# Parskatt/RoMa

Hardware: AMD Instinct MI355X
Metric: image-pairs/sec, roma_outdoor 560->864, batch=8 per GPU (higher is better)
Workload: dtype bf16; 1 GPU; roma_outdoor match() 560->864, symmetric, upsample_preds, 8 pairs/GPU/step, seeded synthetic weights + N(0,1) images; precision policy of the reference's bf16 timing script: bfloat16 DINOv2 + float16 autocast for VGG / decoder / refiners (ROMA_MIXED), f32 accumulate; precision_policy=mixed, global_batch=8, streams_per_gpu=2, parallelism=single GPU, outputs_finite=True

## Files before the change

include/roma_hip.h:

```cpp
#ifndef ROMA_HIP_H
#define ROMA_HIP_H
#include <stdint.h>
#ifdef __cplusplus
extern "C" {
#endif

typedef struct roma_model* roma_handle_t;

enum { ROMA_F32 = 0, ROMA_BF16 = 1, ROMA_F16 = 2,
       ROMA_MIXED = 3 };
int roma_h16_format(void);
enum { ROMA_ERR_ARG = -1, ROMA_ERR_HIP = -2, ROMA_ERR_STATE = -3 };

typedef struct {
  int coarse_h, coarse_w;
  int upsample_h, upsample_w;
  int symmetric;
  int upsample_preds;
  int attenuate_cert;
  int precision;
  int max_batch;
  int device;
} roma_config_t;

const char* roma_last_error(void);
const char* roma_version(void);
#define ROMA_ABI_VERSION 5
int roma_abi_stamp(void);
int roma_self_check(void);

typedef struct {
  const float *ln1_w, *ln1_b, *ln2_w, *ln2_b;
  const float *ls1, *ls2;
  const void *qkv_w, *proj_w, *fc1_w, *fc2_w;
  const float *qkv_b, *proj_b, *fc1_b, *fc2_b;
  int qkv_ldw, proj_ldw, fc1_ldw, fc2_ldw;
} roma_vit_block_t;

typedef struct {
  int B, H, W;
  int act;
  int bf16_residual;
  const float *im_a, *im_b;
  const void* patch_w;
  const float* patch_b;
  int patch_ldw;
  const float *cls_tok, *pos_emb;
  const roma_vit_block_t* blocks;
  int nblocks;
  const float *norm_w, *norm_b;
  void *col, *pt, *x, *xs, *ln, *ao, *hid, *q, *k, *vt;
  void* feat_out;
} roma_vit_args_t;
int roma_vit_forward(const roma_vit_args_t* a, void* stream);
int roma_op_convert_from_bf16(const void* in_bf16, void* out_h16, long n, void* stream);

int roma_create(const roma_config_t* cfg, roma_handle_t* out);
int roma_set_tensor(roma_handle_t h, const char* name, int ndim, const int64_t* shape, const void* data, int is_int64);
int roma_finalize(roma_handle_t h);
int roma_set_option(roma_handle_t h, const char* key, int value);
int roma_set_option_f(roma_handle_t h, const char* key, double value);
int roma_match(roma_handle_t h, int B, const float* im_a, const float* im_b, const float* im_a_hr,
               const float* im_b_hr, float* warp_out, float* cert_out, void* stream);
typedef struct {
  int upsample;
  int symmetric;
  double scale_factor;
  const float* seed_flow;
  const float* seed_cert;
  int seed_h, seed_w;
  float* flow[5];
  float* cert[5];
  void* feat[5];
} roma_forward_args_t;
int roma_forward(roma_handle_t h, int B, const float* im_a, const float* im_b, const roma_forward_args_t* a, void* stream);
long roma_debug_fetch(roma_handle_t h, const char* name, void* dst_host, long nbytes);
int roma_debug_inject(roma_handle_t h, const char* name, const void* src_host, long nbytes);
long roma_debug_trace(roma_handle_t h, int slot, unsigned long long* sums_host, long max_entries, char* names_host,
                      long names_bytes);
int roma_destroy(roma_handle_t h);
int roma_tuning(const char* key, int value);
long roma_tuning_describe(char* buf, long nbytes);
long roma_debug_gemm_trace(unsigned int* dst_host, long nbytes);
int roma_profile_enable(int on);
long roma_profile_report(char* buf, long nbytes);


int roma_op_local_corr(const void* feature0, const void* feature1, const float* warp, void* out, int B, int H, int W,
                       int C, int K, int nearest, int dt_in, int dt_out, void* stream);
int roma_op_local_corr_window(const void* feature0, const void* feature1, const float* warp, void* out, int B, int H,
                              int W, int C, int radius, float scale, long ldo, int dt_in, int dt_out, void* stream);
long roma_op_local_corr_window_workspace(int B, int H, int W, int radius);
int roma_op_local_corr_window_ws(const void* feature0, const void* feature1, const float* warp, void* out, int B, int H,
                                 int W, int C, int radius, float scale, long ldo, int dt_in, int dt_out, void* ws,
                                 long ws_bytes, void* stream);

int roma_op_gemm(const void* A, long lda, const void* W, long ldw, void* C, long ldc, int M, int N, int K, int batch,
                 long sA, long sW, long sC, const float* bias, const float* scale, const float* res, long ldr,
                 int act, float alpha, int dt_in, int dt_out, void* stream);
int roma_op_conv3x3(const void* in, const void* w, const float* bias, void* out, int B, int H, int W, int Cin, int Cout,
                    int relu, int dt, void* stream);
int roma_op_conv3x3_slab(const void* in, const void* w, const float* bias, void* out, int B, int H, int W, int Cin, int Cout,
                         int relu, int dt, void* stream);
int roma_op_attention(const void* q, const void* k, const void* vt, void* out, int B, int heads, int N, int npad, int hd,
                      int dt_in, int dt_out, void* stream);
int roma_op_qkv_scatter_gemm(const void* A, const void* W, const float* bias, void* q, void* k, void* vt, int B, int N,
                             int npad, int heads, int hd, int K, int dt_in, int dt_out, void* stream);
int roma_op_layernorm(const float* x, const float* w, const float* b, void* out, long M, int D, float eps, int dt_out,
                      void* stream);
int roma_op_layernorm_dt(const void* x, int dt_in, const float* w, const float* b, void* out, long M, int D, float eps,
                         int dt_out, void* stream);
int roma_op_gemm_res_bf16(const void* A, long lda, const void* W, long ldw, void* C, long ldc, int M, int N, int K,
                          const float* bias, const float* scale, const void* res, long ldr, void* stream);
int roma_op_cholesky_solve_t(float* A, float* Ft, float* LT, float* Linv, float* LinvT, int n, int d, int batch,
                             void* stream);
int roma_op_gp(const void* x, const void* y, const float* pos_w, const float* pos_b, float* mu, int b, int h, int w, int dt,
               void* stream);
int roma_op_cls_to_flow(const float* logits, long ld, float* flow, float* cert, long M, void* stream);
int roma_op_resize_bilinear(const float* in, float* out, int B, int Hin, int Win, int Hout, int Wout, int nc,
                            void* stream);
int roma_op_refiner_input(const void* feat, long ldf, const float* flow, void* d, long ldd, const float* emb_w,
                          const float* emb_b, int B, int H, int W, int C, int E, int Kcorr, int nimg, int shift,
                          float disp_scale, int dt, void* stream);
int roma_op_dwconv5x5(const void* in, void* out, const float* w, const float* bias, int B, int H, int W, int Cp, int dt,
                      void* stream);
int roma_op_refiner_block(const void* in, void* out, const float* dw_w, const float* dw_b, const void* pw,
                          const float* pw_b, int B, int H, int W, int Cp, int dt, void* stream);
int roma_op_refiner_block_final(const void* in, float* delta, const float* dw_w, const float* dw_b, const void* pw_final,
                                const float* bias_final, int B, int H, int W, int Cp, int dt, void* stream);
int roma_op_refiner_apply_delta(const float* delta, float* flow, float* cert, long M, float sx, float sy, void* stream);
int roma_op_kde(const float* x, long n, int down, float std, int half_inputs, float* density, void* stream);
int roma_op_sample_warp_at(const float* warp, const float* cert, int H, int W, const float* xa, long n, float* xa_to_b,
                           float* cert_a, void* stream);
int roma_op_mutual_nn(const float* a, long na, const float* b, long nb, const float* cert_a, float cert_th, float max_dist,
                      int* match_b, void* ws_a, void* ws_b, void* stream);
int roma_op_mutual_nn_count(const float* a, long na, const float* b, long nb, const float* cert_a, float cert_th, float max_dist,
                            void* ws_a, void* ws_b, long long* offsets, void* stream);
int roma_op_mutual_nn_fill(const float* a, long na, const float* b, long nb, const float* cert_a, float cert_th, float max_dist,
                           const void* ws_a, const void* ws_b, long long* offsets, long long* pairs, void* stream);
long roma_op_multinomial_workspace(long n, long k);
int roma_op_multinomial(const float* weights, long n, long k, unsigned long long seed, long long* out_indices, void* workspace,
                        long workspace_bytes, void* stream);
long roma_op_sample_matches_workspace(int B, long n, long num, int balanced);
int roma_op_sample_matches(const float* matches, const float* certainty, const unsigned long long* seeds, int B, long n, long num,
                           int threshold, float thresh, int balanced, float* out_matches, float* out_certainty, int* out_counts,
                           long long* out_idx, long long* out_first_idx, float* out_density, void* workspace, long workspace_bytes,
                           void* stream);
long roma_op_ransac_workspace(int B, int N);
int roma_op_ransac(int model, const float* kpts_a, const float* kpts_b, const int* counts, const unsigned long long* seeds, int B,
                   int N, float threshold, double confidence, int max_iters, int refine, double* out_model, unsigned char* out_mask,
                   unsigned char* out_ok, int* out_info, void* workspace, long workspace_bytes, void* stream);
long roma_op_magsac_workspace(int B, int N);
int roma_op_magsac(int model, const float* kpts_a, const float* kpts_b, const int* counts, const unsigned long long* seeds, int B,
                   int N, float threshold, double confidence, int max_iters, int lo_iters, double* out_model, unsigned char* out_mask,
                   unsigned char* out_ok, int* out_info, double* out_score, void* workspace, long workspace_bytes, void* stream);
long roma_op_essential_workspace(int B, int N);
int roma_op_essential(const float* kpts_a, const float* kpts_b, const int* counts, const unsigned long long* seeds,
                      const double* camera_matrix, int B, int N, float threshold, double prob, int max_iters, double* out_e,
                      unsigned char* out_mask, unsigned char* out_ok, int* out_info, void* workspace, long workspace_bytes,
                      void* stream);
long roma_op_essential_magsac_workspace(int B, int N);
int roma_op_essential_magsac(const float* kpts_a, const float* kpts_b, const int* counts, const unsigned long long* seeds,
                             const double* camera_matrix, int B, int N, float threshold, double prob, int max_iters, int lo_iters,
                             double* out_e, unsigned char* out_mask, unsigned char* out_ok, int* out_info, double* out_score,
                             void* workspace, long workspace_bytes, void* stream);
int roma_op_essential_minimal(const double* x0, const double* x1, int S, double* out_e, int* out_n, void* stream);
long roma_op_recover_pose_workspace(int B, int N);
int roma_op_recover_pose(const double* E, const float* kpts_a, const float* kpts_b, const unsigned char* mask, const int* counts,
                         const double* camera_matrix, int B, int N, double distance_thresh, int* out_n_good, double* out_r,
                         double* out_t, unsigned char* out_mask, void* workspace, long workspace_bytes, void* stream);
long roma_op_refine_pose_workspace(int B, int N);
int roma_op_refine_pose(const double* R, const double* t, const float* kpts_a, const float* kpts_b, const int* counts,
                        const unsigned char* valid, int B, int N, double thr, int max_steps, double* out_r, double* out_t,
                        unsigned char* out_mask, int* out_info, void* workspace, long workspace_bytes, void* stream);
long roma_op_absolute_pose_workspace(int B, int N);
int roma_op_absolute_pose(const float* points3d, const float* kpts, const int* counts, const unsigned long long* seeds,
                          const double* camera_matrix, int B, int N, float threshold, double conf, int max_iters, double* out_r,
                          double* out_t, unsigned char* out_mask, unsigned char* out_ok, int* out_info, void* workspace,
                          long workspace_bytes, void* stream);
int roma_op_absolute_pose_minimal(const double* X, const double* x, int S, double* out_r, double* out_t, int* out_n, void* stream);
int roma_op_refine_absolute_pose(const double* R, const double* t, const float* points3d, const float* kpts, const int* counts,
                                 const unsigned char* valid, const double* camera_matrix, int B, int N, double thr, int max_steps,
                                 double* out_r, double* out_t, unsigned char* out_mask, int* out_info, void* stream);
int roma_op_lift_matches(const float* matches, const float* depth_a, const double* camera_a, int B, int N, int H, int W, int H_b,
                         int W_b, float* out_points, float* out_kpts_b, void* stream);
long roma_op_bundle_adjust_workspace(int B, int V, int N);
int roma_op_bundle_adjust(const double* points, const float* kpts, const double* camera_matrices, const double* R, const double* t,
                          const unsigned char* hold, const int* counts, const unsigned char* valid, int B, int V, int N,
                          double reproj_thresh, int max_steps, double* out_points, double* out_r, double* out_t, unsigned char* out_mask,
                          int* out_info, double* out_cost, void* workspace, long workspace_bytes, void* stream);
long roma_op_build_tracks_workspace(int B, int V, int K, int P, int M);
int roma_op_build_tracks(const int* inds, const int* pair_views, const int* match_counts, const int* num_kpts, const float* x, int B,
                         int V, int K, int P, int M, int max_tracks, int min_views, int* out_tracks, float* out_kpts, int* out_counts,
                         int* out_total, int* out_info, void* workspace, long workspace_bytes, void* stream);
int roma_op_triangulate_views(const float* kpts, const double* camera_matrices, const double* R, const double* t,
                              const unsigned char* view_valid, const int* counts, const unsigned char* valid, int B, int V, int N,
                              double max_reproj, double min_parallax, double max_depth, int min_views, int gn_steps, int trim,
                              double* out_points, float* out_reproj, unsigned char* out_used, float* out_parallax,
                              unsigned char* out_flags, int* out_stats, void* stream);
long roma_op_refine_model_workspace(int B, int N);
int roma_op_refine_model(int model, const double* M, const float* kpts_a, const float* kpts_b, const int* counts,
                         const unsigned char* valid, int B, int N, double thr, int max_steps, double* out_m, unsigned char* out_mask,
                         int* out_info, double* out_cost, void* workspace, long workspace_bytes, void* stream);
int roma_op_triangulate(const float* matches, const float* certainty, const int* counts, const unsigned char* valid, const double* R,
                        const double* t, const double* K_a, const double* K_b, int B, long n, int coords, int W_a, int H_a, int W_b,
                        int H_b, int sym_w, double max_depth, double max_reproj, double min_parallax, double min_certainty,
                        float* out_points, float* out_depth_other, float* out_reproj, float* out_parallax, unsigned char* out_flags,
                        int* out_stats, void* stream);
int roma_op_depth_consistency(const float* points, const unsigned char* flags, const double* R, const double* t, const double* K_a,
                              const double* K_b, int W_a, int H_a, int W_b, int H_b, int B, int H, int W, double rel_thresh,
                              unsigned char* out_consistent, float* out_err, void* stream);
int roma_op_warp_kpts(const void* kpts, int kpts_f64, int grid_h, int grid_w, const float* depth0, const float* depth1, const double* T,
                      int t_rows, const double* K0, const double* K1, int B, long L, int H0, int W0, int H1, int W1, double rel_thresh,
                      unsigned char* out_valid, float* out_prob, double* out_rel, double* out_warped, void* stream);
long roma_op_dense_metrics_workspace(int B, int h, int w);
int roma_op_dense_metrics(const float* matches, long batch_stride, long row_stride, const float* depth1, const float* depth2,
                          const double* T, int t_rows, const double* K1, const double* K2, int B, int h, int w, int H1, int W1, int H2,
                          int W2, double rel_thresh, double thr0, double thr1, double thr2, long long* out_n_valid,
                          long long* out_n_below, double* out_gd_sum, double* out_epe, double* out_pck, float* out_prob, double* out_gd,
                          void* workspace, long workspace_bytes, void* stream);
int roma_op_pose_error(const double* R, const double* t, const unsigned char* ok, const double* T_gt, int t_rows, int B, double* out_err,
                       double* log, long capacity, long long* state, void* stream);
int roma_op_corner_error(const double* H_pred, const unsigned char* ok, const double* H_gt, const double* sizes, int B, double* out_err,
                         double* log, long capacity, long long* state, void* stream);
int roma_op_error_log_append(const double* values, int B, double* log, long capacity, long long* state, void* stream);
int roma_op_error_summary(const double* errors, long n, const long long* state, long capacity, const double* thresholds, int T,
                          long long* out_n, long long* out_below, double* out_acc, double* out_auc, void* stream);
int roma_op_render_morph_frame_chunk(void);
long roma_op_render_morph_workspace(int B, int im_h, int im_w, long T);
int roma_op_render_morph(const float* warp, long warp_batch_stride, long warp_row_stride, const void* image, int image_u8, const double* ts,
                         const float* certainty, long cert_batch_stride, long cert_row_stride, float background, int B, long T, int H,
                         int W, int im_h, int im_w, void* out, int out_f32, void* workspace, long workspace_bytes, void* stream);
long roma_op_match_keypoints_workspace(int B, long NA, long NB);
int roma_op_match_keypoints(const float* x_a, const float* x_b, const int* counts_a, const int* counts_b, const float* warp,
                            long warp_batch_stride, long warp_row_stride, const float* certainty, long cert_batch_stride,
                            long cert_row_stride, const float* sizes, long sizes_batch_stride, int B, long NA, long NB, int H, int W,
                            float max_dist, float cert_th, long M, int* inds, float* kpts_a, float* kpts_b, int* counts,
                            long long* total, void* workspace, long workspace_bytes, void* stream);
long roma_op_preprocess_workspace(const long long* desc_host, int n_images, const int* targets_hw, int n_targets);
int roma_op_preprocess(const unsigned char* src, long long src_bytes, const long long* desc_host, const long long* desc_dev,
                       int n_images, const int* targets_hw, int n_targets, int normalize, float* out0, float* out1, void* workspace,
                       void* stream);
int roma_op_nchw_to_nhwc(const float* in, float* out, int B, int C, int H, int W, void* stream);
int roma_op_tiny_pos_embed(const float* corr_volume, float* out, int B, int H1, int W1, int H0, int W0, int exact_softmax,
                           void* stream);
int roma_op_gray_instnorm(const float* in, float* out, int B, int H, int W, int C, float eps, void* stream);
int roma_op_conv2d_nhwc(const float* in, const float* w, const float* bias, const float* res, float* out, int B, int H, int W,
                        int Cin, int Cout, int K, int stride, int pad, int relu, void* stream);
int roma_op_avgpool_nhwc(const float* in, float* out, int B, int H, int W, int C, int k, void* stream);
int roma_op_add3(const float* a, const float* b, const float* c, float* out, long n, void* stream);
int roma_op_tiny_matcher_input(const float* f0, const float* f1, const float* warp, int warp_channels, float* d, int B, int H,
                               int W, int H1, int W1, int C, int Cp, void* stream);
int roma_op_tiny_update(const float* base, int base_channels, const float* delta, long ldd, float sx, float sy, float* out,
                        long npix, void* stream);
int roma_op_tiny_final(const float* matches, float* warp, float* certainty, int B, int H, int W, void* stream);
int roma_op_visualize_warp(const float* warp, const float* certainty, const float* im_a, const float* im_b, int H, int W,
                           int symmetric, int im_h, int im_w, float* out, void* stream);
int roma_op_fb_consistency(const float* flow_fwd, const float* flow_bwd, int B, int H, int W, float th_n, float* out,
                           void* stream);
int roma_op_maxpool2x2(const void* in, void* out, int B, int H, int W, int C, int dt, void* stream);
int roma_op_pool_proj(const void* in, void* pooled, void* pf, const void* pw, long ldw, const float* pb, int N, int ldf, int B, int H,
                      int W, int C, int dt, void* stream);
int roma_op_refiner_out(const void* d, long ldd, int dt, const float* w, const float* b, float* flow, float* cert, long M,
                        int Cp, float sx, float sy, void* stream);
int roma_op_conv3x3_c3(const float* img, const float* w, const float* bias, void* out, int B, int H, int W, int dt_out,
                       void* stream);
int roma_op_conv3x3_c3_bf16(const float* img, const void* w, const float* bias, void* out, int B, int H, int W, void* stream);

#ifdef __cplusplus
}
#endif
#endif
```

roma_amd/_lib.py:

```python
from __future__ import annotations

import ctypes as C
import os

_HERE = os.path.dirname(os.path.abspath(__file__))
_HERE = os.environ.get("ROMA_LIB_DIR", _HERE)
LIB_PATH = os.path.join(_HERE, "libroma_hip.so")
LIB_PATHS = {"bf16": LIB_PATH, "f16": os.path.join(_HERE, "libroma_hip_f16.so")}

ROMA_F32, ROMA_BF16, ROMA_F16, ROMA_MIXED = 0, 1, 2, 3
H16_CODE = {"bf16": ROMA_BF16, "f16": ROMA_F16}


class RomaConfig(C.Structure):
    _fields_ = [("coarse_h", C.c_int), ("coarse_w", C.c_int), ("upsample_h", C.c_int), ("upsample_w", C.c_int),
                ("symmetric", C.c_int), ("upsample_preds", C.c_int), ("attenuate_cert", C.c_int),
                ("precision", C.c_int), ("max_batch", C.c_int), ("device", C.c_int)]


class RomaForwardArgs(C.Structure):
    _fields_ = [("upsample", C.c_int), ("symmetric", C.c_int), ("scale_factor", C.c_double),
                ("seed_flow", C.c_void_p), ("seed_cert", C.c_void_p), ("seed_h", C.c_int), ("seed_w", C.c_int),
                ("flow", C.c_void_p * 5), ("cert", C.c_void_p * 5), ("feat", C.c_void_p * 5)]


_vp, _i, _l, _f = C.c_void_p, C.c_int, C.c_long, C.c_float

SIGNATURES = {
    "roma_last_error": (C.c_char_p, []),
    "roma_version": (C.c_char_p, []),
    "roma_h16_format": (_i, []),
    "roma_abi_stamp": (_i, []),
    "roma_self_check": (_i, []),
    "roma_create": (_i, [C.POINTER(RomaConfig), C.POINTER(_vp)]),
    "roma_set_tensor": (_i, [_vp, C.c_char_p, _i, C.POINTER(C.c_int64), _vp, _i]),
    "roma_finalize": (_i, [_vp]),
    "roma_set_option": (_i, [_vp, C.c_char_p, _i]),
    "roma_set_option_f": (_i, [_vp, C.c_char_p, C.c_double]),
    "roma_match": (_i, [_vp, _i, _vp, _vp, _vp, _vp, _vp, _vp, _vp]),
    "roma_forward": (_i, [_vp, _i, _vp, _vp, C.POINTER(RomaForwardArgs), _vp]),
    "roma_debug_fetch": (_l, [_vp, C.c_char_p, _vp, _l]),
    "roma_debug_trace": (_l, [_vp, _i, _vp, _l, C.c_char_p, _l]),
    "roma_debug_inject": (_i, [_vp, C.c_char_p, _vp, _l]),
    "roma_destroy": (_i, [_vp]),
    "roma_tuning": (_i, [C.c_char_p, _i]),
    "roma_tuning_describe": (_l, [C.c_char_p, _l]),
    "roma_debug_gemm_trace": (_l, [_vp, _l]),
    "roma_vit_forward": (_i, [_vp, _vp]),
    "roma_op_convert_from_bf16": (_i, [_vp, _vp, _l, _vp]),
    "roma_profile_enable": (_i, [_i]),
    "roma_profile_report": (_l, [C.c_char_p, _l]),
    "roma_op_local_corr": (_i, [_vp, _vp, _vp, _vp, _i, _i, _i, _i, _i, _i, _i, _i, _vp]),
    "roma_op_local_corr_window": (_i, [_vp, _vp, _vp, _vp, _i, _i, _i, _i, _i, _f, _l, _i, _i, _vp]),
    "roma_op_local_corr_window_workspace": (_l, [_i, _i, _i, _i]),
    "roma_op_local_corr_window_ws": (_i, [_vp, _vp, _vp, _vp, _i, _i, _i, _i, _i, _f, _l, _i, _i, _vp, _l, _vp]),
    "roma_op_gemm": (_i, [_vp, _l, _vp, _l, _vp, _l, _i, _i, _i, _i, _l, _l, _l, _vp, _vp, _vp, _l, _i, _f, _i, _i, _vp]),
    "roma_op_conv3x3": (_i, [_vp, _vp, _vp, _vp, _i, _i, _i, _i, _i, _i, _i, _vp]),
    "roma_op_conv3x3_slab": (_i, [_vp, _vp, _vp, _vp, _i, _i, _i, _i, _i, _i, _i, _vp]),
    "roma_op_attention": (_i, [_vp, _vp, _vp, _vp, _i, _i, _i, _i, _i, _i, _i, _vp]),
    "roma_op_qkv_scatter_gemm": (_i, [_vp, _vp, _vp, _vp, _vp, _vp, _i, _i, _i, _i, _i, _i, _i, _i, _vp]),
    "roma_op_layernorm": (_i, [_vp, _vp, _vp, _vp, _l, _i, _f, _i, _vp]),
    "roma_op_layernorm_dt": (_i, [_vp, _i, _vp, _vp, _vp, _l, _i, _f, _i, _vp]),
    "roma_op_gemm_res_bf16": (_i, [_vp, _l, _vp, _l, _vp, _l, _i, _i, _i, _vp, _vp, _vp, _l, _vp]),
    "roma_op_cholesky_solve_t": (_i, [_vp, _vp, _vp, _vp, _vp, _i, _i, _i, _vp]),
    "roma_op_gp": (_i, [_vp, _vp, _vp, _vp, _vp, _i, _i, _i, _i, _vp]),
    "roma_op_cls_to_flow": (_i, [_vp, _l, _vp, _vp, _l, _vp]),
    "roma_op_resize_bilinear": (_i, [_vp, _vp, _i, _i, _i, _i, _i, _i, _vp]),
    "roma_op_refiner_input": (_i, [_vp, _l, _vp, _vp, _l, _vp, _vp, _i, _i, _i, _i, _i, _i, _i, _i, _f, _i, _vp]),
    "roma_op_dwconv5x5": (_i, [_vp, _vp, _vp, _vp, _i, _i, _i, _i, _i, _vp]),
    "roma_op_refiner_block": (_i, [_vp, _vp, _vp, _vp, _vp, _vp, _i, _i, _i, _i, _i, _vp]),
    "roma_op_refiner_block_final": (_i, [_vp, _vp, _vp, _vp, _vp, _vp, _i, _i, _i, _i, _i, _vp]),
    "roma_op_refiner_apply_delta": (_i, [_vp, _vp, _vp, _l, _f, _f, _vp]),
    "roma_op_kde": (_i, [_vp, _l, _i, _f, _i, _vp, _vp]),
    "roma_op_sample_warp_at": (_i, [_vp, _vp, _i, _i, _vp, _l, _vp, _vp, _vp]),
    "roma_op_mutual_nn": (_i, [_vp, _l, _vp, _l, _vp, _f, _f, _vp, _vp, _vp, _vp]),
    "roma_op_mutual_nn_count": (_i, [_vp, _l, _vp, _l, _vp, _f, _f, _vp, _vp, _vp, _vp]),
    "roma_op_mutual_nn_fill": (_i, [_vp, _l, _vp, _l, _vp, _f, _f, _vp, _vp, _vp, _vp, _vp]),
    "roma_op_fb_consistency": (_i, [_vp, _vp, _i, _i, _i, _f, _vp, _vp]),
    "roma_op_visualize_warp": (_i, [_vp, _vp, _vp, _vp, _i, _i, _i, _i, _i, _vp, _vp]),
    "roma_op_multinomial_workspace": (_l, [_l, _l]),
    "roma_op_multinomial": (_i, [_vp, _l, _l, C.c_ulonglong, _vp, _vp, _l, _vp]),
    "roma_op_sample_matches_workspace": (_l, [_i, _l, _l, _i]),
    "roma_op_sample_matches": (_i, [_vp, _vp, _vp, _i, _l, _l, _i, _f, _i, _vp, _vp, _vp, _vp, _vp, _vp, _vp, _l, _vp]),
    "roma_op_ransac_workspace": (_l, [_i, _i]),
    "roma_op_ransac": (_i, [_i, _vp, _vp, _vp, _vp, _i, _i, _f, C.c_double, _i, _i, _vp, _vp, _vp, _vp, _vp, _l, _vp]),
    "roma_op_magsac_workspace": (_l, [_i, _i]),
    "roma_op_magsac": (_i, [_i, _vp, _vp, _vp, _vp, _i, _i, _f, C.c_double, _i, _i, _vp, _vp, _vp, _vp, _vp, _vp, _l, _vp]),
    "roma_op_essential_workspace": (_l, [_i, _i]),
    "roma_op_essential": (_i, [_vp, _vp, _vp, _vp, _vp, _i, _i, _f, C.c_double, _i, _vp, _vp, _vp, _vp, _vp, _l, _vp]),
    "roma_op_essential_magsac_workspace": (_l, [_i, _i]),
    "roma_op_essential_magsac": (_i, [_vp, _vp, _vp, _vp, _vp, _i, _i, _f, C.c_double, _i, _i, _vp, _vp, _vp, _vp, _vp, _vp, _l, _vp]),
    "roma_op_essential_minimal": (_i, [_vp, _vp, _i, _vp, _vp, _vp]),
    "roma_op_recover_pose_workspace": (_l, [_i, _i]),
    "roma_op_recover_pose": (_i, [_vp, _vp, _vp, _vp, _vp, _vp, _i, _i, C.c_double, _vp, _vp, _vp, _vp, _vp, _l, _vp]),
    "roma_op_refine_pose_workspace": (_l, [_i, _i]),
    "roma_op_refine_pose": (_i, [_vp, _vp, _vp, _vp, _vp, _vp, _i, _i, C.c_double, _i, _vp, _vp, _vp, _vp, _vp, _l, _vp]),
    "roma_op_absolute_pose_workspace": (_l, [_i, _i]),
    "roma_op_absolute_pose": (_i, [_vp, _vp, _vp, _vp, _vp, _i, _i, _f, C.c_double, _i, _vp, _vp, _vp, _vp, _vp, _vp, _l, _vp]),
    "roma_op_absolute_pose_minimal": (_i, [_vp, _vp, _i, _vp, _vp, _vp, _vp]),
    "roma_op_refine_absolute_pose": (_i, [_vp, _vp, _vp, _vp, _vp, _vp, _vp, _i, _i, C.c_double, _i, _vp, _vp, _vp, _vp, _vp]),
    "roma_op_lift_matches": (_i, [_vp, _vp, _vp, _i, _i, _i, _i, _i, _i, _vp, _vp, _vp]),
    "roma_op_bundle_adjust_workspace": (_l, [_i, _i, _i]),
    "roma_op_bundle_adjust": (_i, [_vp, _vp, _vp, _vp, _vp, _vp, _vp, _vp, _i, _i, _i, C.c_double, _i, _vp, _vp, _vp, _vp, _vp, _vp,
                                  _vp, _l, _vp]),
    "roma_op_build_tracks_workspace": (_l, [_i, _i, _i, _i, _i]),
    "roma_op_build_tracks": (_i, [_vp, _vp, _vp, _vp, _vp, _i, _i, _i, _i, _i, _i, _i, _vp, _vp, _vp, _vp, _vp, _vp, _l, _vp]),
    "roma_op_triangulate_views": (_i, [_vp, _vp, _vp, _vp, _vp, _vp, _vp, _i, _i, _i, C.c_double, C.c_double, C.c_double, _i, _i, _i,
                                      _vp, _vp, _vp, _vp, _vp, _vp, _vp]),
    "roma_op_refine_model_workspace": (_l, [_i, _i]),
    "roma_op_refine_model": (_i, [_i, _vp, _vp, _vp, _vp, _vp, _i, _i, C.c_double, _i, _vp, _vp, _vp, _vp, _vp, _l, _vp]),
    "roma_op_triangulate": (_i, [_vp, _vp, _vp, _vp, _vp, _vp, _vp, _vp, _i, _l, _i, _i, _i, _i, _i, _i, C.c_double, C.c_double,
                                C.c_double, C.c_double, _vp, _vp, _vp, _vp, _vp, _vp, _vp]),
    "roma_op_depth_consistency": (_i, [_vp, _vp, _vp, _vp, _vp, _vp, _i, _i, _i, _i, _i, _i, _i, C.c_double, _vp, _vp, _vp]),
    "roma_op_warp_kpts": (_i, [_vp, _i, _i, _i, _vp, _vp, _vp, _i, _vp, _vp, _i, _l, _i, _i, _i, _i, C.c_double, _vp, _vp, _vp, _vp, _vp]),
    "roma_op_dense_metrics_workspace": (_l, [_i, _i, _i]),
    "roma_op_dense_metrics": (_i, [_vp, _l, _l, _vp, _vp, _vp, _i, _vp, _vp, _i, _i, _i, _i, _i, _i, _i, C.c_double, C.c_double, C.c_double,
                                  C.c_double, _vp, _vp, _vp, _vp, _vp, _vp, _vp, _vp, _l, _vp]),
    "roma_op_pose_error": (_i, [_vp, _vp, _vp, _vp, _i, _i, _vp, _vp, _l, _vp, _vp]),
    "roma_op_corner_error": (_i, [_vp, _vp, _vp, _vp, _i, _vp, _vp, _l, _vp, _vp]),
    "roma_op_error_log_append": (_i, [_vp, _i, _vp, _l, _vp, _vp]),
    "roma_op_error_summary": (_i, [_vp, _l, _vp, _l, C.POINTER(C.c_double), _i, _vp, _vp, _vp, _vp, _vp]),
    "roma_op_render_morph_frame_chunk": (_i, []),
    "roma_op_render_morph_workspace": (_l, [_i, _i, _i, _l]),
    "roma_op_render_morph": (_i, [_vp, _l, _l, _vp, _i, _vp, _vp, _l, _l, _f, _i, _l, _i, _i, _i, _i, _vp, _i, _vp, _l, _vp]),
    "roma_op_match_keypoints_workspace": (_l, [_i, _l, _l]),
    "roma_op_match_keypoints": (_i, [_vp, _vp, _vp, _vp, _vp, _l, _l, _vp, _l, _l, _vp, _l, _i, _l, _l, _i, _i, _f, _f, _l, _vp, _vp, _vp,
                                    _vp, _vp, _vp, _l, _vp]),
    "roma_op_preprocess_workspace": (_l, [_vp, _i, _vp, _i]),
    "roma_op_preprocess": (_i, [_vp, C.c_longlong, _vp, _vp, _i, _vp, _i, _i, _vp, _vp, _vp, _vp]),
    "roma_op_nchw_to_nhwc": (_i, [_vp, _vp, _i, _i, _i, _i, _vp]),
    "roma_op_tiny_pos_embed": (_i, [_vp, _vp, _i, _i, _i, _i, _i, _i, _vp]),
    "roma_op_gray_instnorm": (_i, [_vp, _vp, _i, _i, _i, _i, _f, _vp]),
    "roma_op_conv2d_nhwc": (_i, [_vp, _vp, _vp, _vp, _vp, _i, _i, _i, _i, _i, _i, _i, _i, _i, _vp]),
    "roma_op_avgpool_nhwc": (_i, [_vp, _vp, _i, _i, _i, _i, _i, _vp]),
    "roma_op_add3": (_i, [_vp, _vp, _vp, _vp, _l, _vp]),
    "roma_op_tiny_matcher_input": (_i, [_vp, _vp, _vp, _i, _vp, _i, _i, _i, _i, _i, _i, _i, _vp]),
    "roma_op_tiny_update": (_i, [_vp, _i, _vp, _l, _f, _f, _vp, _l, _vp]),
    "roma_op_tiny_final": (_i, [_vp, _vp, _vp, _i, _i, _i, _vp]),
    "roma_op_maxpool2x2": (_i, [_vp, _vp, _i, _i, _i, _i, _i, _vp]),
    "roma_op_pool_proj": (_i, [_vp, _vp, _vp, _vp, _l, _vp, _i, _i, _i, _i, _i, _i, _i, _vp]),
    "roma_op_conv3x3_c3": (_i, [_vp, _vp, _vp, _vp, _i, _i, _i, _i, _vp]),
    "roma_op_conv3x3_c3_bf16": (_i, [_vp, _vp, _vp, _vp, _i, _i, _i, _vp]),
    "roma_op_refiner_out": (_i, [_vp, _l, _i, _vp, _vp, _vp, _vp, _l, _i, _f, _f, _vp]),
}

_libs = {}


class RomaHipError(RuntimeError):
    pass


def load(fmt: str = "bf16"):
    if fmt in _libs:
        return _libs[fmt]
    path = LIB_PATHS[fmt]
    if not os.path.exists(path):
        raise ImportError(f"{path} not found - build it with `python -c 'import __graft_entry__ as g; g.build()'` "
                          "(roma_amd has no CPU fallback)")
    lib = C.CDLL(path)
    for name, (res, args) in SIGNATURES.items():
        fn = getattr(lib, name)
        fn.restype = res
        fn.argtypes = args
    if lib.roma_h16_format() != H16_CODE[fmt]:
        raise ImportError(f"{path} does not store {fmt} (roma_h16_format() = {lib.roma_h16_format()})")
    lib.h16 = fmt
    _libs[fmt] = lib
    return lib


def fmt_of(dtype) -> str:
    return "f16" if str(dtype) == "torch.float16" else "bf16"


def last_error(lib=None) -> str:
    return (lib or load()).roma_last_error().decode("utf-8", "replace")


def check(rc: int, exc=RomaHipError, lib=None):
    if rc != 0:
        raise exc(last_error(lib))
    return rc
```

roma_amd/csrc/api.hip:

```cpp
#include <algorithm>
#include <mutex>
#include <map>
#include <vector>
#include <dlfcn.h>
#include <string.h>

#include "../../include/roma_hip.h"
#include "attention.h"
#include "conv64.h"
#include "conv_patch.h"
#include "elementwise.h"
#include "gemm.h"
#include "local_corr.h"
#include "pool_proj.h"
#include "gp.h"
#include "model.h"
#include "refiner_block.h"
#include "kde.h"
#include "keypoints.h"
#include "keypoints_batched.h"
#include "tiny.h"
#include "tuning.h"
#include "vit.h"
#include "sampling.h"
#include "sample_batched.h"
#include "absolute_pose.h"
#include "bundle.h"
#include "essential.h"
#include "model_refine.h"
#include "pose_refine.h"
#include "geometry.h"
#include "triangulate.h"
#include "tracks.h"
#include "gt_warp.h"
#include "metrics.h"
#include "morph.h"
#include "preprocess.h"

namespace roma {
static thread_local std::string g_err;
void set_error(const std::string& msg) { g_err = msg; }
}

namespace roma {
struct ProfRec { std::string name, unit; double work; hipEvent_t e0, e1; };
static bool g_prof_on = false;
static std::vector<ProfRec> g_prof;
bool prof_enabled() { return g_prof_on; }
void prof_begin(const char* kernel, double work, const char* unit, hipStream_t s) {
  ProfRec r;
  r.name = kernel; r.unit = unit; r.work = work;
  (void)hipEventCreate(&r.e0);
  (void)hipEventCreate(&r.e1);
  (void)hipEventRecord(r.e0, s);
  g_prof.push_back(r);
}
void prof_end(hipStream_t s) { (void)hipEventRecord(g_prof.back().e1, s); }
}

struct roma_model {
  roma::Model m;
};

namespace roma {
void* g_peer_lib = nullptr;
int g_mixed_handles = 0;
template <typename F> static F peer_sym(const char* name) {
  return g_peer_lib ? reinterpret_cast<F>(dlsym(g_peer_lib, name)) : nullptr;
}
}

using namespace roma;

static inline hipStream_t S(void* s) { return static_cast<hipStream_t>(s); }
#ifdef ROMA_H16_F16
static constexpr int ROMA_H16_CODE = ROMA_F16, ROMA_OTHER16_CODE = ROMA_BF16;
#else
static constexpr int ROMA_H16_CODE = ROMA_BF16, ROMA_OTHER16_CODE = ROMA_F16;
#endif
static inline int dt_code(int dt) {
  if (dt == ROMA_F32) return DT_F32;
  if (dt == ROMA_H16_CODE) return DT_BF16;
  set_error(dt == ROMA_OTHER16_CODE
                ? std::string("this library stores ") + ROMA_H16_NAME + ": load " +
                      (ROMA_H16_CODE == ROMA_BF16 ? "libroma_hip_f16.so for ROMA_F16" : "libroma_hip.so for ROMA_BF16")
                : std::string("bad dtype code"));
  return -1;
}
#define DT(dt)                           \
  ({                                     \
    const int _d = dt_code(dt);          \
    if (_d < 0) return ROMA_ERR_ARG;     \
    _d;                                  \
  })

extern "C" {

const char* roma_last_error(void) { return g_err.c_str(); }
const char* roma_version(void) { return "roma_hip 0.3 (gfx950, 16-bit storage = " ROMA_H16_NAME ")"; }
int roma_h16_format(void) { return ROMA_H16_CODE; }
int roma_abi_stamp(void) { return ROMA_ABI_VERSION * 100000 + (int)sizeof(roma_vit_args_t); }
int roma_self_check(void) { return roma::internal_h16_code(); }

int roma_create(const roma_config_t* cfg, roma_handle_t* out) {
  ROMA_REQUIRE(cfg && out, "roma_create: null argument");
  ROMA_REQUIRE(cfg->coarse_h > 0 && cfg->coarse_w > 0 && cfg->coarse_h % 14 == 0 && cfg->coarse_w % 14 == 0,
               "Needs to be multiple of 14 for backbone");
  ROMA_REQUIRE(cfg->coarse_h >= 16 && cfg->coarse_w >= 16, "roma_create: coarse resolution too small for the stride-16 pyramid");
  ROMA_REQUIRE(cfg->upsample_h >= 0 && cfg->upsample_w >= 0 && (cfg->upsample_h == 0 || (cfg->upsample_h >= 16 && cfg->upsample_w >= 16)),
               "roma_create: bad upsample resolution");
  ROMA_REQUIRE(cfg->max_batch >= 1, "roma_create: max_batch must be >= 1");
  if (cfg->precision == ROMA_MIXED) {
    ROMA_REQUIRE(ROMA_H16_CODE == ROMA_F16, "ROMA_MIXED: load libroma_hip_f16.so (it runs DINOv2 through libroma_hip.so)");
  } else if (dt_code(cfg->precision) < 0) {
    return ROMA_ERR_ARG;
  }
  int ndev = 0;
  ROMA_CHECK_HIP(hipGetDeviceCount(&ndev));
  ROMA_REQUIRE(cfg->device >= 0 && cfg->device < ndev, "roma_create: no such HIP device (the HIP path has no CPU fallback)");
  roma_model* h = new roma_model();
  h->m.cfg = *cfg;
  *out = h;
  return 0;
}

int roma_set_tensor(roma_handle_t h, const char* name, int ndim, const int64_t* shape, const void* data, int is_int64) {
  ROMA_REQUIRE(h, "roma_set_tensor: null handle");
  return h->m.set_tensor(name, ndim, shape, data, is_int64);
}

int roma_finalize(roma_handle_t h) {
  ROMA_REQUIRE(h, "roma_finalize: null handle");
  return h->m.finalize();
}

int roma_set_option(roma_handle_t h, const char* key, int value) {
  ROMA_REQUIRE(h && key, "roma_set_option: null argument");
  const std::string k(key);
  if (k == "symmetric") h->m.cfg.symmetric = value ? 1 : 0;
  else if (k == "upsample_preds") {
    ROMA_REQUIRE(!value || h->m.cfg.upsample_h > 0, "roma_set_option: handle was created without an upsample resolution");
    h->m.cfg.upsample_preds = value ? 1 : 0;
  } else if (k == "attenuate_cert") h->m.cfg.attenuate_cert = value ? 1 : 0;
  else if (k == "debug") h->m.debug = value != 0;
  else if (k == "fuse_refiner_blocks") h->m.fuse_refiner_blocks = value != 0;
  else if (k == "compose_out_conv") h->m.compose_out_conv = value != 0;
  else if (k == "vit_bf16_residual") h->m.vit_bf16_residual = value != 0;
  else if (k == "dual_stream") h->m.n_streams = value != 0 ? 2 : 1;
  else if (k == "trace") h->m.trace_on = value != 0;
  else if (k == "streams") {
    ROMA_REQUIRE(value >= 1 && value <= Model::MAX_STREAMS, "roma_set_option: streams must be 1..4");
    h->m.n_streams = value;
  }
  else {
    set_error("roma_set_option: unknown key " + k);
    return ROMA_ERR_ARG;
  }
  return 0;
}

int roma_set_option_f(roma_handle_t h, const char* key, double value) {
  ROMA_REQUIRE(h && key, "roma_set_option_f: null argument");
  const std::string k(key);
  if (k == "coarse_scale_factor") {
    ROMA_REQUIRE(value >= 0.0, "roma_set_option_f: coarse_scale_factor must be >= 0 (0 = derive from the handle's resolution)");
    h->m.coarse_scale_factor = value;
  } else {
    set_error("roma_set_option_f: unknown key " + k);
    return ROMA_ERR_ARG;
  }
  return 0;
}

int roma_match(roma_handle_t h, int B, const float* im_a, const float* im_b, const float* im_a_hr, const float* im_b_hr,
               float* warp_out, float* cert_out, void* stream) {
  ROMA_REQUIRE(h, "roma_match: null handle");
  return h->m.match(B, im_a, im_b, im_a_hr, im_b_hr, warp_out, cert_out, S(stream));
}

int roma_forward(roma_handle_t h, int B, const float* im_a, const float* im_b, const roma_forward_args_t* a, void* stream) {
  ROMA_REQUIRE(h, "roma_forward: null handle");
  return h->m.forward(B, im_a, im_b, a, S(stream));
}

long roma_debug_fetch(roma_handle_t h, const char* name, void* dst_host, long nbytes) {
  if (!h || !name) return ROMA_ERR_ARG;
  auto it = h->m.dbg.find(name);
  if (it == h->m.dbg.end()) {
    set_error(std::string("roma_debug_fetch: no such stage: ") + name);
    return ROMA_ERR_ARG;
  }
  if (!dst_host) return (long)it->second.second;
  if ((size_t)nbytes < it->second.second) {
    set_error("roma_debug_fetch: destination too small");
    return ROMA_ERR_ARG;
  }
  if (hipSetDevice(h->m.cfg.device) != hipSuccess || hipDeviceSynchronize() != hipSuccess) return ROMA_ERR_HIP;
  if (hipMemcpy(dst_host, it->second.first, it->second.second, hipMemcpyDeviceToHost) != hipSuccess) return ROMA_ERR_HIP;
  return (long)it->second.second;
}

int roma_debug_inject(roma_handle_t h, const char* name, const void* src_host, long nbytes) {
  ROMA_REQUIRE(h, "roma_debug_inject: null handle");
  return h->m.debug_inject(name, src_host, nbytes > 0 ? (size_t)nbytes : 0);
}

long roma_debug_trace(roma_handle_t h, int slot, unsigned long long* sums_host, long max_entries, char* names_host,
                      long names_bytes) {
  if (!h || slot < 0 || slot >= Model::MAX_STREAMS_DECL) return ROMA_ERR_ARG;
  const long n = h->m.trace_n[slot];
  if (!sums_host) return n;
  if (max_entries < n || !h->m.trace_dev[slot]) {
    set_error("roma_debug_trace: destination too small or tracing was never enabled");
    return ROMA_ERR_ARG;
  }
  if (hipSetDevice(h->m.cfg.device) != hipSuccess || hipDeviceSynchronize() != hipSuccess) return ROMA_ERR_HIP;
  if (hipMemcpy(sums_host, h->m.trace_dev[slot], (size_t)n * sizeof(unsigned long long), hipMemcpyDeviceToHost) != hipSuccess)
    return ROMA_ERR_HIP;
  if (names_host && names_bytes > 0) {
    std::string all;
    for (long i = 0; i < n; ++i) all += h->m.trace_names[slot][(size_t)i] + "\n";
    const size_t c = std::min<size_t>(all.size(), (size_t)names_bytes - 1);
    memcpy(names_host, all.data(), c);
    names_host[c] = 0;
  }
  return n;
}

int roma_destroy(roma_handle_t h) {
  delete h;
  return 0;
}

int roma_tuning(const char* key, int value) {
  ROMA_REQUIRE(key, "roma_tuning: null key");
  if (g_mixed_handles > 0)
    if (auto f = peer_sym<int (*)(const char*, int)>("roma_tuning"))
      if (int rc = f(key, value)) {
        set_error(std::string("roma_tuning: the bfloat16 sibling library refused key ") + key);
        return rc;
      }
  return tuning_set(key, value);
}

long roma_tuning_describe(char* buf, long nbytes) {
  const std::string js = tuning_describe();
  if (!buf) return (long)js.size() + 1;
  if (nbytes < (long)js.size() + 1) return ROMA_ERR_ARG;
  memcpy(buf, js.c_str(), js.size() + 1);
  return (long)js.size() + 1;
}

int roma_vit_forward(const roma_vit_args_t* a, void* stream) {
  ROMA_REQUIRE(a, "roma_vit_forward: null argument");
  ROMA_REQUIRE(a->act == ROMA_F32 || a->act == ROMA_H16_CODE, "roma_vit_forward: act must be ROMA_F32 or this library's 16-bit code");
  return vit_forward(*a, S(stream));
}

int roma_op_convert_from_bf16(const void* in_bf16, void* out_h16, long n, void* stream) {
  ROMA_REQUIRE(in_bf16 && out_h16, "roma_op_convert_from_bf16: null pointer");
  return convert_from_bf16_launch(in_bf16, out_h16, n, S(stream));
}

long roma_debug_gemm_trace(unsigned int* dst_host, long nbytes) {
  ROMA_REQUIRE(dst_host && nbytes > 0, "roma_debug_gemm_trace: null destination");
  if (hipDeviceSynchronize() != hipSuccess) return ROMA_ERR_HIP;
  const int rc = gemm8p_trace_read(dst_host, nbytes);
  return rc < 0 ? rc : std::min<long>(nbytes, (long)sizeof(unsigned) * 16 * 2 * 256 * 4);
}

int roma_profile_enable(int on) {
  if (g_mixed_handles > 0)
    if (auto f = peer_sym<int (*)(int)>("roma_profile_enable"))
      if (int rc = f(on)) return rc;
  for (auto& r : g_prof) { (void)hipEventDestroy(r.e0); (void)hipEventDestroy(r.e1); }
  g_prof.clear();
  g_prof_on = on != 0;
  return 0;
}

long roma_profile_report(char* buf, long nbytes) {
  if (hipDeviceSynchronize() != hipSuccess) return ROMA_ERR_HIP;
  struct Agg { long calls = 0; double ms = 0, work = 0; std::string unit; };
  std::map<std::string, Agg> agg;
  for (auto& r : g_prof) {
    float ms = 0.f;
    if (hipEventElapsedTime(&ms, r.e0, r.e1) != hipSuccess) continue;
    Agg& a = agg[r.name];
    a.calls++; a.ms += ms; a.work += r.work; a.unit = r.unit;
  }
  std::string js = "{";
  bool first = true;
  for (auto& kv : agg) {
    char tmp[512];
    snprintf(tmp, sizeof tmp, "%s\"%s\": {\"calls\": %ld, \"total_ms\": %.6f, \"work\": %.6e, \"unit\": \"%s\"}", first ? "" : ", ",
             kv.first.c_str(), kv.second.calls, kv.second.ms, kv.second.work, kv.second.unit.c_str());
    js += tmp;
    first = false;
  }
  if (auto f = peer_sym<long (*)(char*, long)>("roma_profile_report")) {
    const long n = f(nullptr, 0);
    if (n > 3) {
      std::string peer((size_t)n, '\0');
      if (f(&peer[0], n) > 0) {
        peer.resize(strlen(peer.c_str()));
        if (peer.size() > 2) js += (first ? "" : ", ") + peer.substr(1, peer.size() - 2);
      }
    }
  }
  js += "}";
  if (!buf) return (long)js.size() + 1;
  if (nbytes < (long)js.size() + 1) return ROMA_ERR_ARG;
  memcpy(buf, js.c_str(), js.size() + 1);
  return (long)js.size() + 1;
}

int roma_op_local_corr(const void* feature0, const void* feature1, const float* warp, void* out, int B, int H, int W,
                       int C, int K, int nearest, int dt_in, int dt_out, void* stream) {
  LocalCorrArgs a;
  a.nearest = nearest ? 1 : 0;
  a.f0 = feature0; a.f1 = feature1; a.warp = warp; a.out = out; a.B = B; a.H = H; a.W = W; a.C = C; a.K = K;
  a.ld0 = C; a.ld1 = C; a.ldo = K; a.nimg = B; a.f1_shift = 0; a.scale = 1.f; a.in_dt = DT(dt_in); a.out_dt = DT(dt_out);
  return local_corr_general_launch(a, S(stream));
}

int roma_op_local_corr_window(const void* feature0, const void* feature1, const float* warp, void* out, int B, int H,
                              int W, int C, int radius, float scale, long ldo, int dt_in, int dt_out, void* stream) {
  LocalCorrArgs a;
  a.f0 = feature0; a.f1 = feature1; a.warp = warp; a.out = out; a.B = B; a.H = H; a.W = W; a.C = C; a.radius = radius;
  a.ld0 = C; a.ld1 = C; a.ldo = ldo; a.nimg = B; a.f1_shift = 0; a.scale = scale; a.in_dt = DT(dt_in); a.out_dt = DT(dt_out);
  ROMA_REQUIRE(ldo >= (2 * radius + 1) * (2 * radius + 1), "local_corr_window: ldo < K");
  return local_corr_window_launch(a, S(stream));
}

long roma_op_local_corr_window_workspace(int B, int H, int W, int radius) {
  if (B <= 0 || H <= 0 || W <= 0) return 0;
  return local_corr_ws_ints(B, H, W, radius) * (long)sizeof(int);
}

int roma_op_local_corr_window_ws(const void* feature0, const void* feature1, const float* warp, void* out, int B, int H,
                                 int W, int C, int radius, float scale, long ldo, int dt_in, int dt_out, void* ws,
                                 long ws_bytes, void* stream) {
  LocalCorrArgs a;
  a.f0 = feature0; a.f1 = feature1; a.warp = warp; a.out = out; a.B = B; a.H = H; a.W = W; a.C = C; a.radius = radius;
  a.ld0 = C; a.ld1 = C; a.ldo = ldo; a.nimg = B; a.f1_shift = 0; a.scale = scale; a.in_dt = DT(dt_in); a.out_dt = DT(dt_out);
  a.ws = static_cast<int*>(ws); a.ws_bytes = ws_bytes;
  ROMA_REQUIRE(ldo >= (2 * radius + 1) * (2 * radius + 1), "local_corr_window: ldo < K");
  if (roma_op_local_corr_window_workspace(B, H, W, radius) == 0) {
    a.ws = nullptr; a.ws_bytes = 0;
  } else {
    ROMA_REQUIRE(ws && (reinterpret_cast<uintptr_t>(ws) & 3) == 0, "local_corr_window_ws: ws must be a 4-byte aligned device pointer");
  }
  return local_corr_window_launch(a, S(stream));
}

int roma_op_gemm(const void* A, long lda, const void* W, long ldw, void* C, long ldc, int M, int N, int K, int batch,
                 long sA, long sW, long sC, const float* bias, const float* scale, const float* res, long ldr, int act,
                 float alpha, int dt_in, int dt_out, void* stream) {
  GemmArgs g;
  g.A = A; g.lda = lda; g.W = W; g.ldw = ldw; g.C = C; g.ldc = ldc; g.M = M; g.N = N; g.K = K; g.batch = batch;
  g.sA = sA; g.sW = sW; g.sC = sC; g.bias = bias; g.scale = scale; g.res = res; g.ldr = ldr; g.sR = sC; g.act = act;
  g.alpha = alpha; g.in_dt = DT(dt_in); g.out_dt = DT(dt_out);
  return gemm_launch(g, S(stream));
}

int roma_op_conv3x3(const void* in, const void* w, const float* bias, void* out, int B, int H, int W, int Cin, int Cout,
                    int relu, int dt, void* stream) {
  GemmArgs g;
  g.A = in; g.W = w; g.ldw = 9 * Cin; g.C = out; g.ldc = Cout; g.M = B * H * W; g.N = Cout; g.K = 9 * Cin;
  g.in_dt = DT(dt); g.out_dt = DT(dt); g.bias = bias; g.act = relu ? ACT_RELU : ACT_NONE;
  g.conv_h = H; g.conv_w = W; g.conv_c = Cin;
  return gemm_launch(g, S(stream));
}

int roma_op_conv3x3_slab(const void* in, const void* w, const float* bias, void* out, int B, int H, int W, int Cin, int Cout,
                         int relu, int dt, void* stream) {
  GemmArgs g;
  g.A = in; g.W = w; g.ldw = 9 * Cin; g.C = out; g.ldc = Cout; g.M = B * H * W; g.N = Cout; g.K = 9 * Cin;
  g.in_dt = DT(dt); g.out_dt = DT(dt); g.bias = bias; g.act = relu ? ACT_RELU : ACT_NONE;
  g.conv_h = H; g.conv_w = W; g.conv_c = Cin; g.conv_korder = 1;
  return gemm_launch(g, S(stream));
}

int roma_op_attention(const void* q, const void* k, const void* vt, void* out, int B, int heads, int N, int npad, int hd,
                      int dt_in, int dt_out, void* stream) {
  AttnArgs a;
  a.q = q; a.k = k; a.vt = vt; a.out = out; a.B = B; a.heads = heads; a.N = N; a.npad = npad; a.hd = hd;
  a.ldo = (long)heads * hd; a.in_dt = DT(dt_in); a.out_dt = DT(dt_out);
  return attention_launch(a, S(stream));
}

int roma_op_qkv_scatter_gemm(const void* A, const void* W, const float* bias, void* q, void* k, void* vt, int B, int N,
                             int npad, int heads, int hd, int K, int dt_in, int dt_out, void* stream) {
  GemmArgs g;
  g.A = A; g.lda = K; g.W = W; g.ldw = K; g.M = B * N; g.N = 3 * heads * hd; g.K = K; g.in_dt = DT(dt_in);
  g.out_dt = DT(dt_out); g.bias = bias; g.mode = EPI_QKV; g.q = q; g.k = k; g.vt = vt; g.heads = heads; g.hd = hd;
  g.ntok = N; g.npad = npad; g.qscale = 1.0f / sqrtf((float)hd);
  return gemm_launch(g, S(stream));
}

int roma_op_layernorm(const float* x, const float* w, const float* b, void* out, long M, int D, float eps, int dt_out,
                      void* stream) {
  return layernorm_launch(x, w, b, out, M, D, eps, DT(dt_out), S(stream));
}

int roma_op_layernorm_dt(const void* x, int dt_in, const float* w, const float* b, void* out, long M, int D, float eps,
                         int dt_out, void* stream) {
  return layernorm_launch_dt(x, DT(dt_in), w, b, out, M, D, eps, DT(dt_out), S(stream));
}

int roma_op_gemm_res_bf16(const void* A, long lda, const void* W, long ldw, void* C, long ldc, int M, int N, int K,
                          const float* bias, const float* scale, const void* res, long ldr, void* stream) {
  GemmArgs g;
  g.A = A; g.lda = lda; g.W = W; g.ldw = ldw; g.C = C; g.ldc = ldc; g.M = M; g.N = N; g.K = K;
  g.bias = bias; g.scale = scale; g.res_bf16 = res; g.ldr = ldr; g.in_dt = DT_BF16; g.out_dt = DT_BF16;
  return gemm_launch(g, S(stream));
}

int roma_op_cholesky_solve_t(float* A, float* Ft, float* LT, float* Linv, float* LinvT, int n, int d, int batch,
                             void* stream) {
  if (batch > 1 && Ft == A + (long)n * n)
    return cholesky_solve_t(A, Ft, LT, Linv, LinvT, n, d, batch, S(stream), (long)(n + d) * n, (long)(n + d) * n);
  return cholesky_solve_t(A, Ft, LT, Linv, LinvT, n, d, batch, S(stream));
}

int roma_op_gp(const void* x, const void* y, const float* pos_w, const float* pos_b, float* mu, int b, int h, int w, int dt,
               void* stream) {
  ROMA_REQUIRE(x && y && pos_w && pos_b && mu && b > 0 && h > 0 && w > 0, "roma_op_gp: bad arguments");
  hipStream_t st = S(stream);
  const int n = h * w;
  const size_t esz = DT(dt) == DT_F32 ? 4 : 2;
  Arena plan;
  plan.alloc((size_t)2 * b * n * 512 * esz);
  if (int rc = gp_posterior(nullptr, 512, DT(dt), b, false, h, w, pos_w, pos_b, mu, 512, plan, st, true)) return rc;
  Arena ar;
  ar.cap = plan.peak + 4096;
  ar.dry = false;
  ROMA_CHECK_HIP(hipMallocAsync(reinterpret_cast<void**>(&ar.base), ar.cap, st));
  char* pf = static_cast<char*>(ar.alloc((size_t)2 * b * n * 512 * esz));
  int rc = 0;
  if (hipMemcpyAsync(pf, x, (size_t)b * n * 512 * esz, hipMemcpyDeviceToDevice, st) != hipSuccess ||
      hipMemcpyAsync(pf + (size_t)b * n * 512 * esz, y, (size_t)b * n * 512 * esz, hipMemcpyDeviceToDevice, st) != hipSuccess) {
    set_error("roma_op_gp: device copy failed");
    rc = ROMA_ERR_HIP;
  }
  if (!rc) rc = gp_posterior(pf, 512, DT(dt), b, false, h, w, pos_w, pos_b, mu, 512, ar, st, false);
  (void)hipFreeAsync(ar.base, st);
  return rc;
}

int roma_op_cls_to_flow(const float* logits, long ld, float* flow, float* cert, long M, void* stream) {
  return cls_to_flow_launch(logits, ld, flow, cert, M, S(stream));
}

int roma_op_resize_bilinear(const float* in, float* out, int B, int Hin, int Win, int Hout, int Wout, int nc,
                            void* stream) {
  return resize_bilinear_launch(in, out, B, Hin, Win, Hout, Wout, nc, S(stream));
}

int roma_op_refiner_input(const void* feat, long ldf, const float* flow, void* d, long ldd, const float* emb_w,
                          const float* emb_b, int B, int H, int W, int C, int E, int Kcorr, int nimg, int shift,
                          float disp_scale, int dt, void* stream) {
  RefinerInputArgs a;
  a.feat = feat; a.ldf = ldf; a.flow = flow; a.d = d; a.ldd = ldd; a.emb_w = emb_w; a.emb_b = emb_b;
  a.B = B; a.H = H; a.W = W; a.C = C; a.E = E; a.Kcorr = Kcorr; a.nimg = nimg; a.shift = shift;
  a.disp_scale = disp_scale; a.dt = DT(dt);
  ROMA_REQUIRE(feat && flow && d && B > 0 && H > 0 && W > 0 && C > 0 && nimg > 0, "roma_op_refiner_input: bad arguments");
  ROMA_REQUIRE(ldd >= 2 * C + E + Kcorr && ldf >= C, "roma_op_refiner_input: row strides too small");
  return refiner_input_launch(a, S(stream));
}

int roma_op_dwconv5x5(const void* in, void* out, const float* w, const float* bias, int B, int H, int W, int Cp, int dt,
                      void* stream) {
  return dwconv5x5_launch(in, out, w, bias, B, H, W, Cp, DT(dt), S(stream));
}

int roma_op_refiner_block(const void* in, void* out, const float* dw_w, const float* dw_b, const void* pw,
                          const float* pw_b, int B, int H, int W, int Cp, int dt, void* stream) {
  return refiner_block_launch(in, out, dw_w, dw_b, pw, Cp, pw_b, B, H, W, Cp, DT(dt), S(stream));
}

int roma_op_refiner_block_final(const void* in, float* delta, const float* dw_w, const float* dw_b, const void* pw_final,
                                const float* bias_final, int B, int H, int W, int Cp, int dt, void* stream) {
  ROMA_REQUIRE(in && delta && dw_w && dw_b && pw_final && bias_final, "roma_op_refiner_block_final: null pointer");
  return refiner_block_final_launch(in, delta, dw_w, dw_b, pw_final, Cp, bias_final, B, H, W, Cp, DT(dt), S(stream));
}

int roma_op_refiner_apply_delta(const float* delta, float* flow, float* cert, long M, float sx, float sy, void* stream) {
  ROMA_REQUIRE(delta && flow && cert && M >= 0, "roma_op_refiner_apply_delta: null pointer");
  return refiner_apply_delta_launch(delta, flow, cert, M, sx, sy, S(stream));
}

int roma_op_kde(const float* x, long n, int down, float std, int half_inputs, float* density, void* stream) {
  return kde_launch(x, n, down, std, half_inputs, density, S(stream));
}

int roma_op_sample_warp_at(const float* warp, const float* cert, int H, int W, const float* xa, long n, float* xa_to_b,
                           float* cert_a, void* stream) {
  return sample_warp_at_launch(warp, cert, H, W, xa, n, xa_to_b, cert_a, S(stream));
}

int roma_op_mutual_nn(const float* a, long na, const float* b, long nb, const float* cert_a, float cert_th, float max_dist,
                      int* match_b, void* ws_a, void* ws_b, void* stream) {
  return mutual_nn_launch(a, na, b, nb, cert_a, cert_th, max_dist, match_b, static_cast<unsigned long long*>(ws_a),
                          static_cast<unsigned long long*>(ws_b), S(stream));
}

int roma_op_mutual_nn_count(const float* a, long na, const float* b, long nb, const float* cert_a, float cert_th, float max_dist,
                            void* ws_a, void* ws_b, long long* offsets, void* stream) {
  return mutual_nn_count_launch(a, na, b, nb, cert_a, cert_th, max_dist, static_cast<unsigned long long*>(ws_a),
                                static_cast<unsigned long long*>(ws_b), offsets, S(stream));
}
int roma_op_mutual_nn_fill(const float* a, long na, const float* b, long nb, const float* cert_a, float cert_th, float max_dist,
                           const void* ws_a, const void* ws_b, long long* offsets, long long* pairs, void* stream) {
  return mutual_nn_fill_launch(a, na, b, nb, cert_a, cert_th, max_dist, static_cast<const unsigned long long*>(ws_a),
                               static_cast<const unsigned long long*>(ws_b), offsets, pairs, S(stream));
}

long roma_op_multinomial_workspace(long n, long k) { return (long)multinomial_workspace_bytes(n, k); }
int roma_op_multinomial(const float* weights, long n, long k, unsigned long long seed, long long* out_indices, void* workspace,
                        long workspace_bytes, void* stream) {
  return multinomial_launch(weights, n, k, seed, out_indices, workspace, (size_t)workspace_bytes, S(stream));
}
long roma_op_sample_matches_workspace(int B, long n, long num, int balanced) {
  return (long)sample_matches_workspace_bytes(B, n, num, balanced);
}
int roma_op_sample_matches(const float* matches, const float* certainty, const unsigned long long* seeds, int B, long n, long num,
                           int threshold, float thresh, int balanced, float* out_matches, float* out_certainty, int* out_counts,
                           long long* out_idx, long long* out_first_idx, float* out_density, void* workspace, long workspace_bytes,
                           void* stream) {
  return sample_matches_launch(matches, certainty, seeds, B, n, num, threshold, thresh, balanced, out_matches, out_certainty, out_counts,
                               out_idx, out_first_idx, out_density, workspace, (size_t)(workspace_bytes > 0 ? workspace_bytes : 0),
                               S(stream));
}
long roma_op_ransac_workspace(int B, int N) { return (long)ransac_workspace_bytes(B, N); }
int roma_op_ransac(int model, const float* kpts_a, const float* kpts_b, const int* counts, const unsigned long long* seeds, int B,
                   int N, float threshold, double confidence, int max_iters, int refine, double* out_model, unsigned char* out_mask,
                   unsigned char* out_ok, int* out_info, void* workspace, long workspace_bytes, void* stream) {
  return ransac_launch(model, kpts_a, kpts_b, counts, seeds, B, N, threshold, confidence, max_iters, refine, out_model, out_mask,
                       out_ok, out_info, workspace, (size_t)(workspace_bytes > 0 ? workspace_bytes : 0), S(stream));
}
long roma_op_magsac_workspace(int B, int N) { return (long)magsac_workspace_bytes(B, N); }
int roma_op_magsac(int model, const float* kpts_a, const float* kpts_b, const int* counts, const unsigned long long* seeds, int B,
                   int N, float threshold, double confidence, int max_iters, int lo_iters, double* out_model, unsigned char* out_mask,
                   unsigned char* out_ok, int* out_info, double* out_score, void* workspace, long workspace_bytes, void* stream) {
  return magsac_launch(model, kpts_a, kpts_b, counts, seeds, B, N, threshold, confidence, max_iters, lo_iters, out_model, out_mask,
                       out_ok, out_info, out_score, workspace, (size_t)(workspace_bytes > 0 ? workspace_bytes : 0), S(stream));
}
long roma_op_essential_workspace(int B, int N) { return (long)essential_workspace_bytes(B, N); }
int roma_op_essential(const float* kpts_a, const float* kpts_b, const int* counts, const unsigned long long* seeds,
                      const double* camera_matrix, int B, int N, float threshold, double prob, int max_iters, double* out_e,
                      unsigned char* out_mask, unsigned char* out_ok, int* out_info, void* workspace, long workspace_bytes,
                      void* stream) {
  return essential_launch(kpts_a, kpts_b, counts, seeds, camera_matrix, B, N, threshold, prob, max_iters, out_e, out_mask, out_ok,
                          out_info, workspace, (size_t)(workspace_bytes > 0 ? workspace_bytes : 0), S(stream));
}
long roma_op_essential_magsac_workspace(int B, int N) { return (long)essential_magsac_workspace_bytes(B, N); }
int roma_op_essential_magsac(const float* kpts_a, const float* kpts_b, const int* counts, const unsigned long long* seeds,
                             const double* camera_matrix, int B, int N, float threshold, double prob, int max_iters, int lo_iters,
                             double* out_e, unsigned char* out_mask, unsigned char* out_ok, int* out_info, double* out_score,
                             void* workspace, long workspace_bytes, void* stream) {
  return essential_magsac_launch(kpts_a, kpts_b, counts, seeds, camera_matrix, B, N, threshold, prob, max_iters, lo_iters, out_e,
                                 out_mask, out_ok, out_info, out_score, workspace,
                                 (size_t)(workspace_bytes > 0 ? workspace_bytes : 0), S(stream));
}
int roma_op_essential_minimal(const double* x0, const double* x1, int S_, double* out_e, int* out_n, void* stream) {
  return essential_minimal_launch(x0, x1, S_, out_e, out_n, S(stream));
}
long roma_op_recover_pose_workspace(int B, int N) { return (long)recover_pose_workspace_bytes(B, N); }
int roma_op_recover_pose(const double* E, const float* kpts_a, const float* kpts_b, const unsigned char* mask, const int* counts,
                         const double* camera_matrix, int B, int N, double distance_thresh, int* out_n_good, double* out_r,
                         double* out_t, unsigned char* out_mask, void* workspace, long workspace_bytes, void* stream) {
  return recover_pose_launch(E, kpts_a, kpts_b, mask, counts, camera_matrix, B, N, distance_thresh, out_n_good, out_r, out_t,
                             out_mask, workspace, (size_t)(workspace_bytes > 0 ? workspace_bytes : 0), S(stream));
}
long roma_op_refine_pose_workspace(int B, int N) { return (long)refine_pose_workspace_bytes(B, N); }
int roma_op_refine_pose(const double* R, const double* t, const float* kpts_a, const float* kpts_b, const int* counts,
                        const unsigned char* valid, int B, int N, double thr, int max_steps, double* out_r, double* out_t,
                        unsigned char* out_mask, int* out_info, void* workspace, long workspace_bytes, void* stream) {
  return refine_pose_launch(R, t, kpts_a, kpts_b, counts, valid, B, N, thr, max_steps, out_r, out_t, out_mask, out_info, workspace,
                            (size_t)(workspace_bytes > 0 ? workspace_bytes : 0), S(stream));
}
long roma_op_absolute_pose_workspace(int B, int N) { return (long)absolute_pose_workspace_bytes(B, N); }
int roma_op_absolute_pose(const float* points3d, const float* kpts, const int* counts, const unsigned long long* seeds,
                          const double* camera_matrix, int B, int N, float threshold, double conf, int max_iters, double* out_r,
                          double* out_t, unsigned char* out_mask, unsigned char* out_ok, int* out_info, void* workspace,
                          long workspace_bytes, void* stream) {
  return absolute_pose_launch(points3d, kpts, counts, seeds, camera_matrix, B, N, threshold, conf, max_iters, out_r, out_t, out_mask,
                              out_ok, out_info, workspace, (size_t)(workspace_bytes > 0 ? workspace_bytes : 0), S(stream));
}
int roma_op_absolute_pose_minimal(const double* X, const double* x, int S_, double* out_r, double* out_t, int* out_n, void* stream) {
  return absolute_pose_minimal_launch(X, x, S_, out_r, out_t, out_n, S(stream));
}
int roma_op_refine_absolute_pose(const double* R, const double* t, const float* points3d, const float* kpts, const int* counts,
                                 const unsigned char* valid, const double* camera_matrix, int B, int N, double thr, int max_steps,
                                 double* out_r, double* out_t, unsigned char* out_mask, int* out_info, void* stream) {
  return refine_absolute_pose_launch(R, t, points3d, kpts, counts, valid, camera_matrix, B, N, thr, max_steps, out_r, out_t, out_mask,
                                     out_info, S(stream));
}
int roma_op_lift_matches(const float* matches, const float* depth_a, const double* camera_a, int B, int N, int H, int W, int H_b,
                         int W_b, float* out_points, float* out_kpts_b, void* stream) {
  return lift_matches_launch(matches, depth_a, camera_a, B, N, H, W, H_b, W_b, out_points, out_kpts_b, S(stream));
}
long roma_op_bundle_adjust_workspace(int B, int V, int N) { return (long)bundle_adjust_workspace_bytes(B, V, N); }
int roma_op_bundle_adjust(const double* points, const float* kpts, const double* camera_matrices, const double* R, const double* t,
                          const unsigned char* hold, const int* counts, const unsigned char* valid, int B, int V, int N,
                          double reproj_thresh, int max_steps, double* out_points, double* out_r, double* out_t, unsigned char* out_mask,
                          int* out_info, double* out_cost, void* workspace, long workspace_bytes, void* stream) {
  return bundle_adjust_launch(points, kpts, camera_matrices, R, t, hold, counts, valid, B, V, N, reproj_thresh, max_steps, out_points,
                              out_r, out_t, out_mask, out_info, out_cost, workspace, (size_t)(workspace_bytes > 0 ? workspace_bytes : 0),
                              S(stream));
}
long roma_op_build_tracks_workspace(int B, int V, int K, int P, int M) { return (long)build_tracks_workspace_bytes(B, V, K, P, M); }
int roma_op_build_tracks(const int* inds, const int* pair_views, const int* match_counts, const int* num_kpts, const float* x, int B,
                         int V, int K, int P, int M, int max_tracks, int min_views, int* out_tracks, float* out_kpts, int* out_counts,
                         int* out_total, int* out_info, void* workspace, long workspace_bytes, void* stream) {
  return build_tracks_launch(inds, pair_views, match_counts, num_kpts, x, B, V, K, P, M, max_tracks, min_views, out_tracks, out_kpts,
                             out_counts, out_total, out_info, workspace, (size_t)(workspace_bytes > 0 ? workspace_bytes : 0), S(stream));
}
int roma_op_triangulate_views(const float* kpts, const double* camera_matrices, const double* R, const double* t,
                              const unsigned char* view_valid, const int* counts, const unsigned char* valid, int B, int V, int N,
                              double max_reproj, double min_parallax, double max_depth, int min_views, int gn_steps, int trim,
                              double* out_points, float* out_reproj, unsigned char* out_used, float* out_parallax,
                              unsigned char* out_flags, int* out_stats, void* stream) {
  return triangulate_views_launch(kpts, camera_matrices, R, t, view_valid, counts, valid, B, V, N, max_reproj, min_parallax, max_depth,
                                  min_views, gn_steps, trim, out_points, out_reproj, out_used, out_parallax, out_flags, out_stats,
                                  S(stream));
}
long roma_op_refine_model_workspace(int B, int N) { return (long)refine_model_workspace_bytes(B, N); }
int roma_op_refine_model(int model, const double* M, const float* kpts_a, const float* kpts_b, const int* counts,
                         const unsigned char* valid, int B, int N, double thr, int max_steps, double* out_m, unsigned char* out_mask,
                         int* out_info, double* out_cost, void* workspace, long workspace_bytes, void* stream) {
  return refine_model_launch(model, M, kpts_a, kpts_b, counts, valid, B, N, thr, max_steps, out_m, out_mask, out_info, out_cost,
                             workspace, (size_t)(workspace_bytes > 0 ? workspace_bytes : 0), S(stream));
}
int roma_op_triangulate(const float* matches, const float* certainty, const int* counts, const unsigned char* valid, const double* R,
                        const double* t, const double* K_a, const double* K_b, int B, long n, int coords, int W_a, int H_a, int W_b,
                        int H_b, int sym_w, double max_depth, double max_reproj, double min_parallax, double min_certainty,
                        float* out_points, float* out_depth_other, float* out_reproj, float* out_parallax, unsigned char* out_flags,
                        int* out_stats, void* stream) {
  return triangulate_launch(matches, certainty, counts, valid, R, t, K_a, K_b, B, n, coords, W_a, H_a, W_b, H_b, sym_w, max_depth,
                            max_reproj, min_parallax, min_certainty, out_points, out_depth_other, out_reproj, out_parallax, out_flags,
                            out_stats, S(stream));
}
int roma_op_depth_consistency(const float* points, const unsigned char* flags, const double* R, const double* t, const double* K_a,
                              const double* K_b, int W_a, int H_a, int W_b, int H_b, int B, int H, int W, double rel_thresh,
                              unsigned char* out_consistent, float* out_err, void* stream) {
  return depth_consistency_launch(points, flags, R, t, K_a, K_b, W_a, H_a, W_b, H_b, B, H, W, rel_thresh, out_consistent, out_err,
                                  S(stream));
}
int roma_op_warp_kpts(const void* kpts, int kpts_f64, int grid_h, int grid_w, const float* depth0, const float* depth1, const double* T,
                      int t_rows, const double* K0, const double* K1, int B, long L, int H0, int W0, int H1, int W1, double rel_thresh,
                      unsigned char* out_valid, float* out_prob, double* out_rel, double* out_warped, void* stream) {
  return warp_kpts_launch(kpts, kpts_f64, grid_h, grid_w, depth0, depth1, T, t_rows, K0, K1, B, L, H0, W0, H1, W1, rel_thresh, out_valid,
                          out_prob, out_rel, out_warped, S(stream));
}
long roma_op_dense_metrics_workspace(int B, int h, int w) { return dense_metrics_workspace_bytes(B, h, w); }
int roma_op_dense_metrics(const float* matches, long batch_stride, long row_stride, const float* depth1, const float* depth2,
                          const double* T, int t_rows, const double* K1, const double* K2, int B, int h, int w, int H1, int W1, int H2,
                          int W2, double rel_thresh, double thr0, double thr1, double thr2, long long* out_n_valid,
                          long long* out_n_below, double* out_gd_sum, double* out_epe, double* out_pck, float* out_prob, double* out_gd,
                          void* workspace, long workspace_bytes, void* stream) {
  return dense_metrics_launch(matches, batch_stride, row_stride, depth1, depth2, T, t_rows, K1, K2, B, h, w, H1, W1, H2, W2, rel_thresh,
                              thr0, thr1, thr2, out_n_valid, out_n_below, out_gd_sum, out_epe, out_pck, out_prob, out_gd, workspace,
                              workspace_bytes, S(stream));
}
int roma_op_pose_error(const double* R, const double* t, const unsigned char* ok, const double* T_gt, int t_rows, int B, double* out_err,
                       double* log, long capacity, long long* state, void* stream) {
  return pose_error_launch(R, t, ok, T_gt, t_rows, B, out_err, log, capacity, state, S(stream));
}
int roma_op_corner_error(const double* H_pred, const unsigned char* ok, const double* H_gt, const double* sizes, int B, double* out_err,
                         double* log, long capacity, long long* state, void* stream) {
  return corner_error_launch(H_pred, ok, H_gt, sizes, B, out_err, log, capacity, state, S(stream));
}
int roma_op_error_log_append(const double* values, int B, double* log, long capacity, long long* state, void* stream) {
  return error_log_append_launch(values, B, log, capacity, state, S(stream));
}
int roma_op_error_summary(const double* errors, long n, const long long* state, long capacity, const double* thresholds, int T,
                          long long* out_n, long long* out_below, double* out_acc, double* out_auc, void* stream) {
  return error_summary_launch(errors, n, state, capacity, thresholds, T, out_n, out_below, out_acc, out_auc, S(stream));
}
int roma_op_render_morph_frame_chunk(void) { return render_morph_frame_chunk(); }
long roma_op_render_morph_workspace(int B, int im_h, int im_w, long T) { return render_morph_workspace_bytes(B, im_h, im_w, T); }
int roma_op_render_morph(const float* warp, long warp_batch_stride, long warp_row_stride, const void* image, int image_u8, const double* ts,
                         const float* certainty, long cert_batch_stride, long cert_row_stride, float background, int B, long T, int H,
                         int W, int im_h, int im_w, void* out, int out_f32, void* workspace, long workspace_bytes, void* stream) {
  return render_morph_launch(warp, warp_batch_stride, warp_row_stride, image, image_u8, ts, certainty, cert_batch_stride, cert_row_stride,
                             background, B, T, H, W, im_h, im_w, out, out_f32, workspace, workspace_bytes, S(stream));
}
long roma_op_match_keypoints_workspace(int B, long NA, long NB) { return match_keypoints_workspace_bytes(B, NA, NB); }
int roma_op_match_keypoints(const float* x_a, const float* x_b, const int* counts_a, const int* counts_b, const float* warp,
                            long warp_batch_stride, long warp_row_stride, const float* certainty, long cert_batch_stride,
                            long cert_row_stride, const float* sizes, long sizes_batch_stride, int B, long NA, long NB, int H, int W,
                            float max_dist, float cert_th, long M, int* inds, float* kpts_a, float* kpts_b, int* counts,
                            long long* total, void* workspace, long workspace_bytes, void* stream) {
  return match_keypoints_launch(x_a, x_b, counts_a, counts_b, warp, warp_batch_stride, warp_row_stride, certainty, cert_batch_stride,
                                cert_row_stride, sizes, sizes_batch_stride, B, NA, NB, H, W, max_dist, cert_th, M, inds, kpts_a, kpts_b,
                                counts, total, workspace, workspace_bytes, S(stream));
}
long roma_op_preprocess_workspace(const long long* desc_host, int n_images, const int* targets_hw, int n_targets) {
  return preprocess_workspace_bytes(desc_host, n_images, targets_hw, n_targets);
}
int roma_op_preprocess(const unsigned char* src, long long src_bytes, const long long* desc_host, const long long* desc_dev,
                       int n_images, const int* targets_hw, int n_targets, int normalize, float* out0, float* out1, void* workspace,
                       void* stream) {
  return preprocess_launch(src, src_bytes, desc_host, desc_dev, n_images, targets_hw, n_targets, normalize, out0, out1, workspace,
                           S(stream));
}
int roma_op_nchw_to_nhwc(const float* in, float* out, int B, int C, int H, int W, void* stream) {
  return nchw_to_nhwc_launch(in, out, B, C, H, W, S(stream));
}
int roma_op_tiny_pos_embed(const float* corr_volume, float* out, int B, int H1, int W1, int H0, int W0, int exact_softmax,
                           void* stream) {
  return tiny_pos_embed_launch(corr_volume, out, B, H1, W1, H0, W0, exact_softmax, S(stream));
}
int roma_op_gray_instnorm(const float* in, float* out, int B, int H, int W, int C, float eps, void* stream) {
  return gray_instnorm_launch(in, out, B, H, W, C, eps, S(stream));
}
int roma_op_conv2d_nhwc(const float* in, const float* w, const float* bias, const float* res, float* out, int B, int H, int W,
                        int Cin, int Cout, int K, int stride, int pad, int relu, void* stream) {
  return conv2d_nhwc_launch(in, w, bias, res, out, B, H, W, Cin, Cout, K, stride, pad, relu, S(stream));
}
int roma_op_avgpool_nhwc(const float* in, float* out, int B, int H, int W, int C, int k, void* stream) {
  return avgpool_nhwc_launch(in, out, B, H, W, C, k, S(stream));
}
int roma_op_add3(const float* a, const float* b, const float* c, float* out, long n, void* stream) {
  return add3_launch(a, b, c, out, n, S(stream));
}
int roma_op_tiny_matcher_input(const float* f0, const float* f1, const float* warp, int warp_channels, float* d, int B, int H,
                               int W, int H1, int W1, int C, int Cp, void* stream) {
  return tiny_matcher_input_launch(f0, f1, warp, warp_channels, d, B, H, W, H1, W1, C, Cp, S(stream));
}
int roma_op_tiny_update(const float* base, int base_channels, const float* delta, long ldd, float sx, float sy, float* out,
                        long npix, void* stream) {
  return tiny_update_launch(base, base_channels, delta, ldd, sx, sy, out, npix, S(stream));
}
int roma_op_tiny_final(const float* matches, float* warp, float* certainty, int B, int H, int W, void* stream) {
  return tiny_final_launch(matches, warp, certainty, B, H, W, S(stream));
}
int roma_op_visualize_warp(const float* warp, const float* certainty, const float* im_a, const float* im_b, int H, int W,
                           int symmetric, int im_h, int im_w, float* out, void* stream) {
  return visualize_warp_launch(warp, certainty, im_a, im_b, H, W, symmetric, im_h, im_w, out, S(stream));
}
int roma_op_fb_consistency(const float* flow_fwd, const float* flow_bwd, int B, int H, int W, float th_n, float* out,
                           void* stream) {
  return fb_consistency_launch(flow_fwd, flow_bwd, B, H, W, th_n, out, S(stream));
}

int roma_op_maxpool2x2(const void* in, void* out, int B, int H, int W, int C, int dt, void* stream) {
  return maxpool2x2_launch(in, out, B, H, W, C, DT(dt), S(stream));
}

int roma_op_pool_proj(const void* in, void* pooled, void* pf, const void* pw, long ldw, const float* pb, int N, int ldf, int B, int H,
                      int W, int C, int dt, void* stream) {
  return pool_proj_launch(in, pooled, pf, pw, ldw, pb, N, ldf, B, H, W, C, DT(dt), S(stream));
}

int roma_op_refiner_out(const void* d, long ldd, int dt, const float* w, const float* b, float* flow, float* cert, long M,
                        int Cp, float sx, float sy, void* stream) {
  ROMA_REQUIRE(d && w && b && flow && cert && M > 0 && Cp > 0 && ldd >= Cp, "roma_op_refiner_out: bad arguments");
  return refiner_out_launch(d, ldd, DT(dt), w, b, flow, cert, M, Cp, sx, sy, S(stream));
}

int roma_op_conv3x3_c3_bf16(const float* img, const void* w, const float* bias, void* out, int B, int H, int W, void* stream) {
  return conv3x3_c3_bf16_launch(img, w, bias, out, B, H, W, S(stream));
}

int roma_op_conv3x3_c3(const float* img, const float* w, const float* bias, void* out, int B, int H, int W, int dt_out,
                       void* stream) {
  return conv3x3_c3_launch(img, w, bias, out, B, H, W, DT(dt_out), S(stream));
}

}
```

roma_amd/csrc/conv64.h:

```cpp
#pragma once
#include "gemm.h"

namespace roma {
int conv64_try_launch(const GemmArgs& a, hipStream_t stream);
int conv3x3_c3_bf16_launch(const float* img, const void* w, const float* bias, void* out, int B, int H, int W, hipStream_t stream);
}
```

roma_amd/csrc/conv64.hip:

```cpp
#include "conv64.h"

#include <stdio.h>
#include <stdlib.h>

#include <algorithm>

#include "gemm_device.h"
#include "tuning.h"

namespace roma {

static __device__ __attribute__((aligned(256))) unsigned int g_c64_dump[256];

#define C64_WAIT_VM(N) asm volatile("s_waitcnt vmcnt(%0)" ::"n"(N) : "memory")

template <int COUT>
__global__ __launch_bounds__(256, 2) void conv3x3_c64_kernel(const bf16_t* __restrict__ in, const bf16_t* __restrict__ w,
                                                             const float* __restrict__ bias, bf16_t* __restrict__ out, int B,
                                                             int H, int W, int SY, int nxt, int nblocks) {
  constexpr int NCG = COUT / 32;
  constexpr int NPG = 4 / NCG;
  constexpr int TW = 64 * NPG;
  constexpr int NPIECE = ((TW + 2) * 128 + 1023) / 1024;
  constexpr int RSTRIDE = NPIECE * 1024;
  constexpr int KW = (NPIECE + 3) / 4;
  extern __shared__ __attribute__((aligned(1024))) unsigned char ring[];

  if ((int)blockIdx.x >= nblocks) return;
  const int tid = threadIdx.x, lane = tid & 63;
  const int wave = __builtin_amdgcn_readfirstlane(tid >> 6);
  const int cg = wave % NCG, pg = wave / NCG;
  const int l31 = lane & 31, h = lane >> 5;
  typedef unsigned u32x4 __attribute__((ext_vector_type(4)));
  const unsigned ring0 = (unsigned)(size_t)((__attribute__((address_space(3))) unsigned char*)ring);

  u32x4 wreg[36];
  {
    const bf16_t* wp = w + (long)(32 * cg + l31) * 576 + 8 * h;
#pragma unroll
    for (int ks = 0; ks < 36; ++ks) wreg[ks] = *reinterpret_cast<const u32x4*>(wp + 16 * ks);
  }
  float* bias_s = reinterpret_cast<float*>(ring + 4 * RSTRIDE);
  if (tid < COUT) bias_s[tid] = bias[tid];

  unsigned rdo[3];
#pragma unroll
  for (int dx = 0; dx < 3; ++dx) {
    const int p = 64 * pg + l31 + dx;
    rdo[dx] = ring0 + (unsigned)(p * 128 + ((h ^ ((p >> 1) & 7)) << 4));
  }

  for (int lb = blockIdx.x; lb < nblocks; lb += gridDim.x) {
  const int xt = lb % nxt;
  const int r = lb / nxt;
  const int yt = (H + SY - 1) / SY;
  const int ys = (r % yt) * SY;
  const int b = r / yt;
  const int x0 = xt * TW;
  const int sy = min(SY, H - ys);
  if (lb != (int)blockIdx.x) __builtin_amdgcn_s_barrier();

  const bf16_t* inb = in + (long)b * H * W * 64;
  const __amdgpu_buffer_rsrc_t rs_in = __builtin_amdgcn_make_buffer_rsrc(const_cast<bf16_t*>(inb), 0, (int)((long)H * W * 128), 0x00020000);
  unsigned voff[KW];
  bool okx[KW];
  {
    const int dl_p = lane >> 3, dl_slot = lane & 7;
    const u32x4 z4 = {0u, 0u, 0u, 0u};
#pragma unroll
    for (int j = 0; j < KW; ++j) {
      const int q = wave + 4 * j;
      const int p = q * 8 + dl_p;
      const int x = x0 - 1 + p;
      const int c = dl_slot ^ ((p >> 1) & 7);
      okx[j] = q < NPIECE && p < TW + 2 && x >= 0 && x < W;
      voff[j] = okx[j] ? (unsigned)(x * 128 + c * 16) : 0u;
      if (q < NPIECE && !okx[j]) {
        int ln = lane;
        asm volatile("" : "+v"(ln));
#pragma unroll
        for (int sl = 0; sl < 4; ++sl)
          asm volatile("ds_write_b128 %0, %1" ::"v"(ring0 + sl * RSTRIDE + q * 1024 + ln * 16), "v"(z4) : "memory");
      }
    }
  }
  asm volatile("s_waitcnt vmcnt(0) lgkmcnt(0)" ::: "memory");

#define C64_ISSUE_ROW(YY, SLOT)                                                                                \
  {                                                                                                            \
    const int yy_ = (YY);                                                                                      \
    if (yy_ >= 0 && yy_ < H) {                                                                                 \
      const int so_ = yy_ * W * 128;                                                                           \
      _Pragma("unroll") for (int j = 0; j < KW; ++j) {                                                         \
        const int q_ = wave + 4 * j;                                                                           \
        if (q_ < NPIECE) {                                                                                     \
          if (okx[j])                                                                                          \
            __builtin_amdgcn_raw_ptr_buffer_load_lds(rs_in, (__attribute__((address_space(3))) void*)(ring + (SLOT) * RSTRIDE + q_ * 1024), \
                                                     16, (int)voff[j], so_, 0, 0);                             \
        }                                                                                                      \
      }                                                                                                        \
    } else {                                     \
      const u32x4 z4_ = {0u, 0u, 0u, 0u};                                                                      \
      int ln_ = lane;                                                                                          \
      asm volatile("" : "+v"(ln_));                                                                            \
      _Pragma("unroll") for (int j = 0; j < KW; ++j) {                                                         \
        const int q_ = wave + 4 * j;                                                                           \
        if (q_ < NPIECE)                                                                                       \
          asm volatile("ds_write_b128 %0, %1" ::"v"(ring0 + (SLOT) * RSTRIDE + q_ * 1024 + ln_ * 16), "v"(z4_) : "memory"); \
      }                                                                                                        \
    }                                                                                                          \
  }

  u32x4 fa[2][4];
#define C64_READ_G(SLOTOFF, DX, G)                                                                            \
  {                                                                                                           \
    const unsigned ad_ = (rdo[DX] + (SLOTOFF)) ^ (unsigned)((G) << 5);                                         \
    asm volatile("ds_read_b128 %0, %1" : "=v"(fa[0][G]) : "v"(ad_));                                           \
    asm volatile("ds_read_b128 %0, %1 offset:4096" : "=v"(fa[1][G]) : "v"(ad_));                              \
  }
#define C64_WAIT_G(G, N) asm volatile("s_waitcnt lgkmcnt(%2)" : "+v"(fa[0][G]), "+v"(fa[1][G]) : "n"(N) : "memory")

  C64_ISSUE_ROW(ys - 1, 0)
  C64_ISSUE_ROW(ys, 1)
  C64_ISSUE_ROW(ys + 1, 2)

  bf16_t* outb = out + (long)b * H * W * COUT;
  for (int o = 0; o < sy; ++o) {
    if (o == 0) {
      asm volatile("s_waitcnt vmcnt(0) lgkmcnt(0)" ::: "memory");
    } else {
      C64_WAIT_VM(0);
    }
    __builtin_amdgcn_s_barrier();
    C64_ISSUE_ROW(ys + o + 2, (o + 3) & 3)
    if (o == 0) {
      C64_READ_G(0, 0, 0)
      C64_READ_G(0, 0, 1)
    }
    C64_READ_G((o & 3) * RSTRIDE, 0, 2)
    C64_READ_G((o & 3) * RSTRIDE, 0, 3)

    f32x16 acc[2];
#pragma unroll
    for (int tm = 0; tm < 2; ++tm)
#pragma unroll
      for (int e = 0; e < 16; ++e) acc[tm][e] = 0.f;
#pragma unroll
    for (int t = 0; t < 9; ++t) {
#pragma unroll
      for (int g = 0; g < 4; ++g) {
        if (t == 8 && g == 3) {
          C64_WAIT_G(g, 4);
        } else {
          C64_WAIT_G(g, 6);
        }
#pragma unroll
        for (int tm = 0; tm < 2; ++tm)
          acc[tm] = mfma_h16_32x32x16(wreg[t * 4 + g],
                                                            fa[tm][g], acc[tm]);
        __builtin_amdgcn_sched_barrier(0);
        if (t + 1 < 9) {
          C64_READ_G(((o + (t + 1) / 3) & 3) * RSTRIDE, (t + 1) % 3, g)
        } else if (g < 2) {
          C64_READ_G(((o + 1) & 3) * RSTRIDE, 0, g)
        }
        __builtin_amdgcn_sched_barrier(0);
      }
    }

    const int y = ys + o;
#pragma unroll
    for (int P = 0; P < 2; ++P) {
      f32x4 bv0, bv1;
      {
        const unsigned ba = ring0 + 4 * RSTRIDE + (32 * cg + 16 * P + 4 * h) * 4;
        asm volatile("ds_read_b128 %0, %2\n\tds_read_b128 %1, %2 offset:32\n\ts_waitcnt lgkmcnt(0)"
                     : "=&v"(bv0), "=&v"(bv1)
                     : "v"(ba)
                     : "memory");
      }
#pragma unroll
      for (int tm = 0; tm < 2; ++tm) {
        const int x = x0 + 64 * pg + 32 * tm + l31;
        const unsigned a0 = pack_bf16x2(fmaxf(acc[tm][8 * P + 0] + bv0[0], 0.f), fmaxf(acc[tm][8 * P + 1] + bv0[1], 0.f));
        const unsigned a1 = pack_bf16x2(fmaxf(acc[tm][8 * P + 2] + bv0[2], 0.f), fmaxf(acc[tm][8 * P + 3] + bv0[3], 0.f));
        const unsigned b0 = pack_bf16x2(fmaxf(acc[tm][8 * P + 4] + bv1[0], 0.f), fmaxf(acc[tm][8 * P + 5] + bv1[1], 0.f));
        const unsigned b1 = pack_bf16x2(fmaxf(acc[tm][8 * P + 6] + bv1[2], 0.f), fmaxf(acc[tm][8 * P + 7] + bv1[3], 0.f));
        const auto s0 = __builtin_amdgcn_permlane32_swap(a0, b0, false, false);
        const auto s1 = __builtin_amdgcn_permlane32_swap(a1, b1, false, false);
        const u32x4 st = {s0[0], s1[0], s0[1], s1[1]};
        bf16_t* op = outb + ((long)y * W + x) * COUT + 32 * cg + 16 * P + 8 * h;
        u32x4* dst = x < W ? reinterpret_cast<u32x4*>(op) : reinterpret_cast<u32x4*>(g_c64_dump) + lane;
        *dst = st;
      }
    }
  }
  C64_WAIT_VM(0);
  }
#undef C64_WAIT_G
#undef C64_READ_G
#undef C64_ISSUE_ROW
}

template <int DUMMY>
__global__ __launch_bounds__(512, 1) void conv3x3_c128_kernel(const bf16_t* __restrict__ in, const bf16_t* __restrict__ w,
                                                              const float* __restrict__ bias, bf16_t* __restrict__ out, int B,
                                                              int H, int W, int SY, int nxt, int nblocks) {
  constexpr int COUT = 128, TW = 64;
  constexpr int NPIECE = ((TW + 2) * 256 + 1023) / 1024;
  constexpr int RSTRIDE = NPIECE * 1024;
  constexpr int KW = (NPIECE + 7) / 8;
  constexpr int XCH = 4 * RSTRIDE;
  constexpr int BIAS = XCH + 2 * 8 * 4096;
  extern __shared__ __attribute__((aligned(1024))) unsigned char ring[];
  if ((int)blockIdx.x >= nblocks) return;

  const int tid = threadIdx.x, lane = tid & 63;
  const int wave = __builtin_amdgcn_readfirstlane(tid >> 6);
  const int cg = wave & 3, kh = wave >> 2;
  const int l31 = lane & 31, h = lane >> 5;
  typedef unsigned u32x4 __attribute__((ext_vector_type(4)));
  const unsigned ring0 = (unsigned)(size_t)((__attribute__((address_space(3))) unsigned char*)ring);

  u32x4 wreg[36];
  {
    const bf16_t* wp = w + (long)(32 * cg + l31) * 1152 + 64 * kh + 8 * h;
#pragma unroll
    for (int t = 0; t < 9; ++t)
#pragma unroll
      for (int g = 0; g < 4; ++g) wreg[t * 4 + g] = *reinterpret_cast<const u32x4*>(wp + 128 * t + 16 * g);
  }
  float* bias_s = reinterpret_cast<float*>(ring + BIAS);
  if (tid < COUT) bias_s[tid] = bias[tid];

  unsigned rdo[3];
#pragma unroll
  for (int dx = 0; dx < 3; ++dx) {
    const int p = l31 + dx;
    rdo[dx] = ring0 + (unsigned)(p * 256 + (((8 * kh + h) ^ (p & 15)) << 4));
  }
  const unsigned xw = ring0 + XCH + (unsigned)((cg + 4 * (1 - kh)) * 4096 + lane * 16);
  const unsigned xr = ring0 + XCH + (unsigned)((cg + 4 * kh) * 4096 + lane * 16);

  for (int lb = blockIdx.x; lb < nblocks; lb += gridDim.x) {
  const int xt = lb % nxt;
  const int r = lb / nxt;
  const int yt = (H + SY - 1) / SY;
  const int ys = (r % yt) * SY;
  const int b = r / yt;
  const int x0 = xt * TW;
  const int sy = min(SY, H - ys);
  if (lb != (int)blockIdx.x) __builtin_amdgcn_s_barrier();

  const bf16_t* inb = in + (long)b * H * W * 128;
  const __amdgpu_buffer_rsrc_t rs_in = __builtin_amdgcn_make_buffer_rsrc(const_cast<bf16_t*>(inb), 0, (int)((long)H * W * 256), 0x00020000);
  unsigned voff[KW];
  bool okx[KW];
  {
    const int dl_p = lane >> 4, dl_slot = lane & 15;
    const u32x4 z4 = {0u, 0u, 0u, 0u};
#pragma unroll
    for (int j = 0; j < KW; ++j) {
      const int q = wave + 8 * j;
      const int p = q * 4 + dl_p;
      const int x = x0 - 1 + p;
      const int c = dl_slot ^ (p & 15);
      okx[j] = q < NPIECE && p < TW + 2 && x >= 0 && x < W;
      voff[j] = okx[j] ? (unsigned)(x * 256 + c * 16) : 0u;
      if (q < NPIECE && !okx[j]) {
        int ln = lane;
        asm volatile("" : "+v"(ln));
#pragma unroll
        for (int sl = 0; sl < 4; ++sl)
          asm volatile("ds_write_b128 %0, %1" ::"v"(ring0 + sl * RSTRIDE + q * 1024 + ln * 16), "v"(z4) : "memory");
      }
    }
  }
  asm volatile("s_waitcnt vmcnt(0) lgkmcnt(0)" ::: "memory");

#define C128_ISSUE_ROW(YY, SLOT)                                                                               \
  {                                                                                                            \
    const int yy_ = (YY);                                                                                      \
    if (yy_ >= 0 && yy_ < H) {                                                                                 \
      const int so_ = yy_ * W * 256;                                                                           \
      _Pragma("unroll") for (int j = 0; j < KW; ++j) {                                                         \
        const int q_ = wave + 8 * j;                                                                           \
        if (q_ < NPIECE) {                                                                                     \
          if (okx[j])                                                                                          \
            __builtin_amdgcn_raw_ptr_buffer_load_lds(rs_in, (__attribute__((address_space(3))) void*)(ring + (SLOT) * RSTRIDE + q_ * 1024), \
                                                     16, (int)voff[j], so_, 0, 0);                             \
        }                                                                                                      \
      }                                                                                                        \
    } else {                                                                                                   \
      const u32x4 z4_ = {0u, 0u, 0u, 0u};                                                                      \
      int ln_ = lane;                                                                                          \
      asm volatile("" : "+v"(ln_));                                                                            \
      _Pragma("unroll") for (int j = 0; j < KW; ++j) {                                                         \
        const int q_ = wave + 8 * j;                                                                           \
        if (q_ < NPIECE)                                                                                       \
          asm volatile("ds_write_b128 %0, %1" ::"v"(ring0 + (SLOT) * RSTRIDE + q_ * 1024 + ln_ * 16), "v"(z4_) : "memory"); \
      }                                                                                                        \
    }                                                                                                          \
  }

  u32x4 fa[2][4];
#define C128_READ_G(SLOTOFF, DX, G)                                                                           \
  {                                                                                                           \
    const unsigned ad_ = (rdo[DX] + (SLOTOFF)) ^ (unsigned)((G) << 5);                                         \
    asm volatile("ds_read_b128 %0, %1" : "=v"(fa[0][G]) : "v"(ad_));                                           \
    asm volatile("ds_read_b128 %0, %1 offset:8192" : "=v"(fa[1][G]) : "v"(ad_));                              \
  }
#define C128_WAIT_G(G, N) asm volatile("s_waitcnt lgkmcnt(%2)" : "+v"(fa[0][G]), "+v"(fa[1][G]) : "n"(N) : "memory")

  bf16_t* outb = out + (long)b * H * W * COUT;
#define C128_EPILOGUE(ACC, Y, PAR)                                                                            \
  {                                                                                                           \
    f32x4 pp_[4];                                                                                             \
    asm volatile("ds_read_b128 %0, %4\n\tds_read_b128 %1, %4 offset:1024\n\tds_read_b128 %2, %4 offset:2048\n\t" \
                 "ds_read_b128 %3, %4 offset:3072\n\ts_waitcnt lgkmcnt(0)"                                    \
                 : "=&v"(pp_[0]), "=&v"(pp_[1]), "=&v"(pp_[2]), "=&v"(pp_[3])                                 \
                 : "v"(xr + (unsigned)(PAR) * 32768u)                                                         \
                 : "memory");                                                                                 \
    const int x_ = x0 + 32 * kh + l31;                                                                        \
    _Pragma("unroll") for (int P = 0; P < 2; ++P) {                                                           \
      f32x4 bv0_, bv1_;                                                                                       \
      asm volatile("ds_read_b128 %0, %2\n\tds_read_b128 %1, %2 offset:32\n\ts_waitcnt lgkmcnt(0)"            \
                   : "=&v"(bv0_), "=&v"(bv1_)                                                                 \
                   : "v"(ring0 + BIAS + (32 * cg + 16 * P + 4 * h) * 4)                                       \
                   : "memory");                                                                               \
      const f32x4 p0_ = pp_[2 * P], p1_ = pp_[2 * P + 1];                                                     \
      const unsigned a0_ = pack_bf16x2(fmaxf(ACC[8 * P + 0] + p0_[0] + bv0_[0], 0.f), fmaxf(ACC[8 * P + 1] + p0_[1] + bv0_[1], 0.f)); \
      const unsigned a1_ = pack_bf16x2(fmaxf(ACC[8 * P + 2] + p0_[2] + bv0_[2], 0.f), fmaxf(ACC[8 * P + 3] + p0_[3] + bv0_[3], 0.f)); \
      const unsigned b0_ = pack_bf16x2(fmaxf(ACC[8 * P + 4] + p1_[0] + bv1_[0], 0.f), fmaxf(ACC[8 * P + 5] + p1_[1] + bv1_[1], 0.f)); \
      const unsigned b1_ = pack_bf16x2(fmaxf(ACC[8 * P + 6] + p1_[2] + bv1_[2], 0.f), fmaxf(ACC[8 * P + 7] + p1_[3] + bv1_[3], 0.f)); \
      const auto s0_ = __builtin_amdgcn_permlane32_swap(a0_, b0_, false, false);                              \
      const auto s1_ = __builtin_amdgcn_permlane32_swap(a1_, b1_, false, false);                              \
      const u32x4 st_ = {s0_[0], s1_[0], s0_[1], s1_[1]};                                                     \
      bf16_t* op_ = outb + ((long)(Y) * W + x_) * COUT + 32 * cg + 16 * P + 8 * h;                            \
      u32x4* dst_ = x_ < W ? reinterpret_cast<u32x4*>(op_) : reinterpret_cast<u32x4*>(g_c64_dump) + lane;     \
      *dst_ = st_;                                                                                            \
    }                                                                                                         \
  }
#define C128_PUBLISH(ACC, PAR)                                                                                \
  _Pragma("unroll") for (int j = 0; j < 4; ++j) {                                                             \
    const f32x4 v_ = {ACC[4 * j + 0], ACC[4 * j + 1], ACC[4 * j + 2], ACC[4 * j + 3]};                        \
    asm volatile("ds_write_b128 %0, %1" ::"v"(xw + (unsigned)(PAR) * 32768u + j * 1024), "v"(v_) : "memory"); \
  }

  C128_ISSUE_ROW(ys - 1, 0)
  C128_ISSUE_ROW(ys, 1)
  C128_ISSUE_ROW(ys + 1, 2)

  f32x16 acc[2];
  for (int o = 0; o < sy; ++o) {
    asm volatile("s_waitcnt vmcnt(0) lgkmcnt(0)" ::: "memory");
    __builtin_amdgcn_s_barrier();
    if (o > 0) {
      if (kh == 0) C128_EPILOGUE(acc[0], ys + o - 1, (o - 1) & 1)
      else C128_EPILOGUE(acc[1], ys + o - 1, (o - 1) & 1)
    }
    C128_ISSUE_ROW(ys + o + 2, (o + 3) & 3)
    if (o == 0) {
      C128_READ_G(0, 0, 0)
      C128_READ_G(0, 0, 1)
    }
    C128_READ_G((o & 3) * RSTRIDE, 0, 2)
    C128_READ_G((o & 3) * RSTRIDE, 0, 3)

#pragma unroll
    for (int tm = 0; tm < 2; ++tm)
#pragma unroll
      for (int e = 0; e < 16; ++e) acc[tm][e] = 0.f;
#pragma unroll
    for (int t = 0; t < 9; ++t) {
#pragma unroll
      for (int g = 0; g < 4; ++g) {
        if (t == 8 && g == 3) {
          C128_WAIT_G(g, 4);
        } else {
          C128_WAIT_G(g, 6);
        }
#pragma unroll
        for (int tm = 0; tm < 2; ++tm)
          acc[tm] = mfma_h16_32x32x16(wreg[t * 4 + g],
                                                            fa[tm][g], acc[tm]);
        __builtin_amdgcn_sched_barrier(0);
        if (t + 1 < 9) {
          C128_READ_G(((o + (t + 1) / 3) & 3) * RSTRIDE, (t + 1) % 3, g)
        } else if (g < 2) {
          C128_READ_G(((o + 1) & 3) * RSTRIDE, 0, g)
        }
        __builtin_amdgcn_sched_barrier(0);
      }
    }
    if (kh == 0) C128_PUBLISH(acc[1], o & 1)
    else C128_PUBLISH(acc[0], o & 1)
  }
  asm volatile("s_waitcnt vmcnt(0) lgkmcnt(0)" ::: "memory");
  __builtin_amdgcn_s_barrier();
  if (kh == 0) C128_EPILOGUE(acc[0], ys + sy - 1, (sy - 1) & 1)
  else C128_EPILOGUE(acc[1], ys + sy - 1, (sy - 1) & 1)
  C64_WAIT_VM(0);
  }
#undef C128_PUBLISH
#undef C128_EPILOGUE
#undef C128_WAIT_G
#undef C128_READ_G
#undef C128_ISSUE_ROW
}

__global__ __launch_bounds__(256, 4) void conv3x3_c3_bf16_kernel(const float* __restrict__ img, const bf16_t* __restrict__ w,
                                                                 const float* __restrict__ bias, bf16_t* __restrict__ out, int B,
                                                                 int H, int W, int RY, int nxt, long ntiles) {
  __shared__ __attribute__((aligned(16))) float bias_s[64];
  __shared__ __attribute__((aligned(1024))) unsigned char stage[4][4096];
  if (threadIdx.x < 64) bias_s[threadIdx.x] = bias[threadIdx.x];
  __syncthreads();
  const int lane = threadIdx.x & 63;
  const int wave = __builtin_amdgcn_readfirstlane(threadIdx.x >> 6);
  const long t = (long)blockIdx.x * 4 + wave;
  if (t >= ntiles) return;
  const int xt = (int)(t % nxt);
  const long r = t / nxt;
  const int nyb = (H + RY - 1) / RY;
  const int y0 = (int)(r % nyb) * RY;
  const int b = (int)(r / nyb);
  const int l31 = lane & 31, h = lane >> 5;
  const int x = xt * 32 + l31;
  const int HW = H * W;
  typedef unsigned u32x4 __attribute__((ext_vector_type(4)));

  u32x4 wf[2][2];
#pragma unroll
  for (int cb = 0; cb < 2; ++cb)
#pragma unroll
    for (int ks = 0; ks < 2; ++ks) wf[cb][ks] = *reinterpret_cast<const u32x4*>(w + (32 * cb + l31) * 32 + 16 * h + 8 * ks);

  int toff[16], tsel[16];
#pragma unroll
  for (int s_ = 0; s_ < 16; ++s_) {
    const int k0 = s_, k1 = 16 + s_;
    const int o0 = (k0 / 9) * HW + ((k0 % 9) / 3 - 1) * W + (k0 % 3 - 1);
    const int o1 = k1 < 27 ? (k1 / 9) * HW + ((k1 % 9) / 3 - 1) * W + (k1 % 3 - 1) : 0;
    const int m0 = (1 << ((k0 % 9) / 3)) | (8 << (k0 % 3));
    const int m1 = k1 < 27 ? ((1 << ((k1 % 9) / 3)) | (8 << (k1 % 3))) : 64;
    toff[s_] = h ? o1 : o0;
    tsel[s_] = h ? m1 : m0;
  }
  const int colbits = ((x >= 1 && x - 1 < W) ? 8 : 0) | (x < W ? 16 : 0) | (x + 1 < W ? 32 : 0);
  const bool cols_in = xt * 32 >= 1 && xt * 32 + 33 <= W;
  const float* p0 = img + (long)b * 3 * HW;
  bf16_t* outb = out + (long)b * HW * 64;
  const unsigned st0 = (unsigned)(size_t)((__attribute__((address_space(3))) unsigned char*)stage[wave]);
  const int ny = min(RY, H - y0);
  for (int o = 0; o < ny; ++o) {
    const int y = y0 + o;
    const int base = y * W + x;
    float v[16];
    if (cols_in && y >= 1 && y + 1 < H) {
#pragma unroll
      for (int s_ = 0; s_ < 16; ++s_) v[s_] = p0[base + toff[s_]];
      if (h) {
#pragma unroll
        for (int s_ = 11; s_ < 16; ++s_) v[s_] = 0.f;
      }
    } else {
      const int okbits = colbits | (y >= 1 ? 1 : 0) | 2 | (y + 1 < H ? 4 : 0);
#pragma unroll
      for (int s_ = 0; s_ < 16; ++s_) {
        const bool ok = (okbits & tsel[s_]) == tsel[s_];
        const float ld = p0[ok ? base + toff[s_] : 0];
        v[s_] = ok ? ld : 0.f;
      }
    }
    u32x4 fr[2];
#pragma unroll
    for (int ks = 0; ks < 2; ++ks)
#pragma unroll
      for (int j = 0; j < 4; ++j) fr[ks][j] = pack_bf16x2(v[8 * ks + 2 * j], v[8 * ks + 2 * j + 1]);
    f32x16 acc[2];
#pragma unroll
    for (int cb = 0; cb < 2; ++cb) {
#pragma unroll
      for (int e = 0; e < 16; ++e) acc[cb][e] = 0.f;
#pragma unroll
      for (int ks = 0; ks < 2; ++ks)
        acc[cb] = mfma_h16_32x32x16(wf[cb][ks],
                                                          fr[ks], acc[cb]);
    }
#pragma unroll
    for (int cb = 0; cb < 2; ++cb)
#pragma unroll
      for (int P = 0; P < 2; ++P) {
        const f32x4 b0 = *reinterpret_cast<const f32x4*>(bias_s + 32 * cb + 16 * P + 4 * h);
        const f32x4 b1 = *reinterpret_cast<const f32x4*>(bias_s + 32 * cb + 16 * P + 8 + 4 * h);
        const unsigned a0 = pack_bf16x2(fmaxf(acc[cb][8 * P + 0] + b0[0], 0.f), fmaxf(acc[cb][8 * P + 1] + b0[1], 0.f));
        const unsigned a1 = pack_bf16x2(fmaxf(acc[cb][8 * P + 2] + b0[2], 0.f), fmaxf(acc[cb][8 * P + 3] + b0[3], 0.f));
        const unsigned c0 = pack_bf16x2(fmaxf(acc[cb][8 * P + 4] + b1[0], 0.f), fmaxf(acc[cb][8 * P + 5] + b1[1], 0.f));
        const unsigned c1 = pack_bf16x2(fmaxf(acc[cb][8 * P + 6] + b1[2], 0.f), fmaxf(acc[cb][8 * P + 7] + b1[3], 0.f));
        const auto s0 = __builtin_amdgcn_permlane32_swap(a0, c0, false, false);
        const auto s1 = __builtin_amdgcn_permlane32_swap(a1, c1, false, false);
        const u32x4 st = {s0[0], s1[0], s0[1], s1[1]};
        const int c = 4 * cb + 2 * P + h;
        *reinterpret_cast<__attribute__((address_space(3))) u32x4*>(st0 + l31 * 128 + ((c ^ (l31 & 7)) << 4)) = st;
      }
#pragma unroll
    for (int i = 0; i < 4; ++i) {
      const u32x4 st = *reinterpret_cast<__attribute__((address_space(3))) const u32x4*>(st0 + i * 1024 + lane * 16);
      const int px = i * 8 + (lane >> 3);
      const int c = (lane & 7) ^ (px & 7);
      if (xt * 32 + px < W) *reinterpret_cast<u32x4*>(outb + ((long)y * W + xt * 32 + px) * 64 + c * 8) = st;
    }
  }
}

int conv3x3_c3_bf16_launch(const float* img, const void* w, const float* bias, void* out, int B, int H, int W, hipStream_t stream) {
  ROMA_REQUIRE(img && w && bias && out && B > 0 && H > 0 && W > 0, "conv3x3_c3_bf16: bad arguments");
  ROMA_REQUIRE((long)3 * H * W < (1l << 23), "conv3x3_c3_bf16: image too large for the packed tap offsets");
  const int RY = 8;
  const int nxt = (W + 31) / 32;
  const long ntiles = (long)B * ((H + RY - 1) / RY) * nxt;
  ProfScope ps("conv3x3_c3_bf16_kernel", (double)B * H * W * (12.0 + 128.0), "byte", stream);
  hipLaunchKernelGGL(conv3x3_c3_bf16_kernel, dim3((unsigned)((ntiles + 3) / 4)), dim3(256), 0, stream, img,
                     reinterpret_cast<const bf16_t*>(w), bias, reinterpret_cast<bf16_t*>(out), B, H, W, RY, nxt, ntiles);
  ROMA_LAUNCH_CHECK();
  return 0;
}

int conv64_try_launch(const GemmArgs& a, hipStream_t stream) {
  const int use = tuning(SW_CONV64);
  const bool c128 = a.conv_c == 128;
  if (!(use & (c128 ? 2 : 1))) return 1;
  if ((a.conv_c != 64 && !c128) || a.in_dt != DT_BF16 || a.out_dt != DT_BF16 || a.act != ACT_RELU || !a.bias) return 1;
  if (c128 ? a.N != 128 : (a.N != 64 && a.N != 128)) return 1;
  if (a.ldc != a.N || a.ldw != 9 * a.conv_c || a.batch != 1 || a.mode != EPI_STD || a.scale || a.res || a.res_bf16 || a.alpha != 1.0f)
    return 1;
  const int H = a.conv_h, W = a.conv_w;
  const long hw = (long)H * W;
  if (hw <= 0 || a.M % hw != 0) return 1;
  if ((long)hw * a.conv_c * 2 >= (1l << 31)) return 1;
  const int B = (int)(a.M / hw);
  const int TW = (!c128 && a.N == 64) ? 128 : 64;
  const int slots = c128 ? 256 : 512;
  const int sy_env = tuning(SW_CONV64_SY);
  const int nxt = (W + TW - 1) / TW;
  int SY = sy_env;
  if (SY <= 0) {
    long best = -1;
    for (int yt = 1; yt <= std::max(1, H / 12); ++yt) {
      const int sy = (H + yt - 1) / yt;
      const long n = (long)B * nxt * ((H + sy - 1) / sy);
      const long cost = ((n + slots - 1) / slots) * (sy + 3);
      if (best < 0 || cost < best) {
        best = cost;
        SY = sy;
      }
    }
  }
  const long nb = (long)B * ((H + SY - 1) / SY) * nxt;
  if (nb <= 0 || nb >= (1l << 30)) return 1;
  char pname[64];
  snprintf(pname, sizeof pname, c128 ? "conv3x3_c128_kernel<%d>" : "conv3x3_c64_kernel<%d>", a.N);
  ProfScope ps(pname, 2.0 * (double)a.M * a.N * 9.0 * a.conv_c, "flop", stream);
  const bf16_t* in = reinterpret_cast<const bf16_t*>(a.A);
  const bf16_t* w = reinterpret_cast<const bf16_t*>(a.W);
  bf16_t* out = reinterpret_cast<bf16_t*>(a.C);
  constexpr int LDS64 = 4 * 17 * 1024 + 512, LDS64N128 = 4 * 9 * 1024 + 512;
  constexpr int LDS128 = 4 * 17 * 1024 + 2 * 8 * 4096 + 512;
  static bool attr_set[64] = {false};
  int dev = 0;
  ROMA_CHECK_HIP(hipGetDevice(&dev));
  if (dev < 0 || dev >= 64 || !attr_set[dev]) {
    ROMA_CHECK_HIP(hipFuncSetAttribute(reinterpret_cast<const void*>(&conv3x3_c64_kernel<64>), hipFuncAttributeMaxDynamicSharedMemorySize, LDS64));
    ROMA_CHECK_HIP(hipFuncSetAttribute(reinterpret_cast<const void*>(&conv3x3_c64_kernel<128>), hipFuncAttributeMaxDynamicSharedMemorySize, LDS64N128));
    ROMA_CHECK_HIP(hipFuncSetAttribute(reinterpret_cast<const void*>(&conv3x3_c128_kernel<0>), hipFuncAttributeMaxDynamicSharedMemorySize, LDS128));
    if (dev >= 0 && dev < 64) attr_set[dev] = true;
  }
  const long gx = std::min<long>(nb, slots);
  if (c128) {
    hipLaunchKernelGGL(conv3x3_c128_kernel<0>, dim3((unsigned)gx), dim3(512), LDS128, stream, in, w, a.bias, out, B, H, W, SY, nxt, (int)nb);
  } else if (a.N == 64) {
    hipLaunchKernelGGL(conv3x3_c64_kernel<64>, dim3((unsigned)gx), dim3(256), LDS64, stream, in, w, a.bias, out, B, H, W, SY, nxt, (int)nb);
  } else {
    hipLaunchKernelGGL(conv3x3_c64_kernel<128>, dim3((unsigned)gx), dim3(256), LDS64N128, stream, in, w, a.bias, out, B, H, W, SY, nxt, (int)nb);
  }
  ROMA_LAUNCH_CHECK();
  return 0;
}

}
```

roma_amd/csrc/model.hip:

```cpp
#include "model.h"

#include <dlfcn.h>
#include <math.h>
#include <stdlib.h>

#include <algorithm>

#include "arch.h"
#include "attention.h"
#include "conv64.h"
#include "dry_run.h"
#include "pool_proj.h"
#include "elementwise.h"
#include "gemm.h"
#include "gp.h"
#include "local_corr.h"
#include "refiner_block.h"
#include "vit.h"

namespace roma {

std::mutex g_peer_mutex;
extern void* g_peer_lib;
extern int g_mixed_handles;

Model::~Model() {
  for (int i = 0; i < MAX_STREAMS - 1; ++i) {
    if (side[i]) (void)hipStreamDestroy(side[i]);
    if (ev_join[i]) (void)hipEventDestroy(ev_join[i]);
  }
  if (ev_fork) (void)hipEventDestroy(ev_fork);
  for (void* p : owned) (void)hipFree(p);
  for (auto& kv : dbg) (void)hipFree(kv.second.first);
  for (auto& kv : inject) (void)hipFree(kv.second.first);
  if (peer_lib) {
    std::lock_guard<std::mutex> lk(g_peer_mutex);
    --g_mixed_handles;
  }
}


int Model::load_peer() {
  static void* lib = nullptr;
  static int (*fwd)(const roma_vit_args_t*, void*) = nullptr;
  std::lock_guard<std::mutex> lk(g_peer_mutex);
  if (!lib) {
    ROMA_REQUIRE(roma_h16_format() == ROMA_F16, "ROMA_MIXED is a mode of the binary16 build (libroma_hip_f16.so)");
    Dl_info info;
    ROMA_REQUIRE(dladdr(reinterpret_cast<void*>(&roma_vit_forward), &info) && info.dli_fname, "ROMA_MIXED: cannot locate this library");
    std::string path(info.dli_fname);
    const size_t slash = path.find_last_of('/');
    path = (slash == std::string::npos ? std::string("") : path.substr(0, slash + 1)) + "libroma_hip.so";
    void* l = dlopen(path.c_str(), RTLD_NOW | RTLD_LOCAL | RTLD_DEEPBIND);
    if (!l) {
      set_error("ROMA_MIXED: cannot load the bfloat16 library " + path + ": " + (dlerror() ? dlerror() : "?"));
      return ROMA_ERR_STATE;
    }
    auto fmt = reinterpret_cast<int (*)(void)>(dlsym(l, "roma_h16_format"));
    auto self = reinterpret_cast<int (*)(void)>(dlsym(l, "roma_self_check"));
    auto abi = reinterpret_cast<int (*)(void)>(dlsym(l, "roma_abi_stamp"));
    auto f = reinterpret_cast<int (*)(const roma_vit_args_t*, void*)>(dlsym(l, "roma_vit_forward"));
    std::string why;
    if (!fmt || !f || !self || !abi) why = "it does not export roma_h16_format / roma_self_check / roma_abi_stamp / roma_vit_forward (an older build)";
    else if (fmt() != ROMA_BF16) why = "it is not the bfloat16 build";
    else if (abi() != roma_abi_stamp()) why = "its ABI stamp " + std::to_string(abi()) + " differs from this library's " + std::to_string(roma_abi_stamp()) + " (stale build: roma_vit_args_t would be misread)";
    else if (self() != ROMA_BF16) why = "its internal calls resolve into another library (symbol interposition: link both builds with -Wl,-Bsymbolic)";
    if (!why.empty()) {
      dlclose(l);
      set_error("ROMA_MIXED: " + path + " cannot serve as the bfloat16 sibling: " + why);
      return ROMA_ERR_STATE;
    }
    lib = l;
    fwd = f;
    g_peer_lib = l;
  }
  if (!peer_lib) ++g_mixed_handles;
  peer_lib = lib;
  peer_vit_forward = fwd;
  return 0;
}

int Model::debug_inject(const char* name, const void* host, size_t bytes) {
  ROMA_REQUIRE(name, "roma_debug_inject: null name");
  const std::string k(name);
  ROMA_REQUIRE(k == "gm_flow16" || k == "gm_cert16", "roma_debug_inject: unknown stage (gm_flow16, gm_cert16)");
  ROMA_CHECK_HIP(hipSetDevice(cfg.device));
  auto it = inject.find(k);
  if (it != inject.end()) {
    ROMA_CHECK_HIP(hipDeviceSynchronize());
    (void)hipFree(it->second.first);
    inject.erase(it);
  }
  if (!host || bytes == 0) return 0;
  void* p = nullptr;
  ROMA_CHECK_HIP(hipMalloc(&p, bytes));
  ROMA_CHECK_HIP(hipMemcpy(p, host, bytes, hipMemcpyHostToDevice));
  inject[k] = {p, bytes};
  return 0;
}

int Model::finalize() {
  ROMA_REQUIRE(!finalized, "roma_finalize: already finalized");
  ROMA_CHECK_HIP(hipSetDevice(cfg.device));
  if (int rc = check_contract()) return rc;
  act_dt = cfg.precision == ROMA_F32 ? DT_F32 : DT_BF16;
  mixed = cfg.precision == ROMA_MIXED;
  if (mixed)
    if (int rc = load_peer()) return rc;
  if (int rc = pack_weights()) return rc;
  host.clear();
  arena.dry = persist.dry = true;
  arena.peak = persist.peak = 0;
  const int keep_sym = cfg.symmetric, keep_up = cfg.upsample_preds;
  cfg.symmetric = 1;
  cfg.upsample_preds = cfg.upsample_h > 0 ? 1 : 0;
  int rc = match_impl(cfg.max_batch, nullptr, nullptr, nullptr, nullptr, nullptr, nullptr, nullptr, true, arena, persist);
  Arena plan, plan_p;
  if (!rc && cfg.max_batch >= 2)
    rc = match_impl(cfg.max_batch / 2, nullptr, nullptr, nullptr, nullptr, nullptr, nullptr, nullptr, true, plan, plan_p);
  cfg.symmetric = keep_sym;
  cfg.upsample_preds = keep_up;
  if (rc) return rc;
  side_arena_bytes = plan.peak + 4096;
  side_persist_bytes = plan_p.peak + 4096;
  arena.cap = arena.peak + 4096;
  persist.cap = persist.peak + 4096;
  ROMA_CHECK_HIP(hipMalloc((void**)&arena.base, arena.cap));
  owned.push_back(arena.base);
  ROMA_CHECK_HIP(hipMalloc((void**)&persist.base, persist.cap));
  owned.push_back(persist.base);
  ROMA_CHECK_HIP(hipMemset(persist.base, 0, persist.cap));
  ROMA_CHECK_HIP(hipMemset(arena.base, 0, arena.cap));
  arena.dry = persist.dry = false;
  finalized = true;
  return 0;
}

int Model::ensure_side_streams(int n) {
  for (int i = streams_ready - 1; i + 1 < n; ++i) {
    Arena &a = side_arena[i], &p = side_persist[i];
    a.cap = side_arena_bytes;
    p.cap = side_persist_bytes;
    ROMA_CHECK_HIP(hipMalloc((void**)&a.base, a.cap));
    owned.push_back(a.base);
    ROMA_CHECK_HIP(hipMalloc((void**)&p.base, p.cap));
    owned.push_back(p.base);
    ROMA_CHECK_HIP(hipMemset(p.base, 0, p.cap));
    ROMA_CHECK_HIP(hipMemset(a.base, 0, a.cap));
    ROMA_CHECK_HIP(hipDeviceSynchronize());
    a.dry = p.dry = false;
    ROMA_CHECK_HIP(hipStreamCreateWithFlags(&side[i], hipStreamNonBlocking));
    ROMA_CHECK_HIP(hipEventCreateWithFlags(&ev_join[i], hipEventDisableTiming));
    if (!ev_fork) ROMA_CHECK_HIP(hipEventCreateWithFlags(&ev_fork, hipEventDisableTiming));
    streams_ready = i + 2;
  }
  return 0;
}

static int dbg_dual_slot() { return tuning(SW_DEBUG_DUAL_SLOT); }

int Model::dbg_save(const char* name, const void* p, size_t bytes, hipStream_t st) {
  if (!debug) return 0;
  if (dbg_dual_slot() >= 0) {
    static const std::string only = std::string(",") + (getenv("ROMA_DEBUG_ONLY") ? getenv("ROMA_DEBUG_ONLY") : "") + ",";
    if (dbg_cur_slot != dbg_dual_slot() || only.find(std::string(",") + name + ",") == std::string::npos) return 0;
  }
  auto it = dbg.find(name);
  if (it == dbg.end() || it->second.second != bytes) {
    if (it != dbg.end()) (void)hipFree(it->second.first);
    void* q = nullptr;
    ROMA_CHECK_HIP(hipMalloc(&q, bytes));
    dbg[name] = {q, bytes};
    it = dbg.find(name);
  }
  ROMA_CHECK_HIP(hipMemcpyAsync(it->second.first, p, bytes, hipMemcpyDeviceToDevice, st));
  return 0;
}

int Model::match(int B, const float* ima, const float* imb, const float* ima_hr, const float* imb_hr, float* warp,
                 float* cert, hipStream_t st) {
  ROMA_REQUIRE(finalized, "roma_match: call roma_finalize first");
  ROMA_REQUIRE(B >= 1 && B <= cfg.max_batch, "roma_match: batch size out of range (max_batch)");
  ROMA_REQUIRE(ima && imb && warp && cert, "roma_match: null image / output pointer");
  if (cfg.upsample_preds) {
    ROMA_REQUIRE(cfg.upsample_h > 0, "roma_match: upsample_preds set but the handle has no upsample resolution");
    ROMA_REQUIRE(ima_hr && imb_hr, "roma_match: upsample_preds requires im_A_high_res and im_B_high_res");
  }
  ROMA_CHECK_HIP(hipSetDevice(cfg.device));
  return match_streams(B, ima, imb, ima_hr, imb_hr, warp, cert, st);
}

int Model::forward(int B, const float* ima, const float* imb, const roma_forward_args_t* fw, hipStream_t st) {
  ROMA_REQUIRE(finalized, "roma_forward: call roma_finalize first");
  ROMA_REQUIRE(B >= 1 && B <= cfg.max_batch, "roma_forward: batch size out of range (max_batch)");
  ROMA_REQUIRE(ima && imb && fw, "roma_forward: null image / argument pointer");
  if (fw->upsample) {
    ROMA_REQUIRE(cfg.upsample_h > 0, "roma_forward: upsample pass on a handle without an upsample resolution");
    ROMA_REQUIRE(fw->seed_flow && fw->seed_cert && fw->seed_h > 0 && fw->seed_w > 0,
                 "roma_forward: the upsample pass needs batch[\"corresps\"] (seed_flow / seed_cert)");
  }
  ROMA_CHECK_HIP(hipSetDevice(cfg.device));
  return match_impl(B, ima, imb, nullptr, nullptr, nullptr, nullptr, st, false, arena, persist, fw);
}

int Model::match_streams(int B, const float* ima, const float* imb, const float* ima_hr, const float* imb_hr, float* warp,
                         float* cert, hipStream_t st) {
  const int env_streams = tuning(SW_STREAMS);
  const bool serial_env = tuning(SW_STREAMS_SERIAL) != 0;
  const int ns = (debug && dbg_dual_slot() < 0) ? 1 : std::min(std::min(env_streams > 0 ? env_streams : n_streams, (int)MAX_STREAMS), B);
  if (ns <= 1) return match_impl(B, ima, imb, ima_hr, imb_hr, warp, cert, st, false, arena, persist);
  if (int rc = ensure_side_streams(ns)) return rc;
  const size_t im_lo = (size_t)3 * cfg.coarse_h * cfg.coarse_w, im_hi = (size_t)3 * cfg.upsample_h * cfg.upsample_w;
  const int Ho = cfg.upsample_preds ? cfg.upsample_h : cfg.coarse_h, Wo = cfg.upsample_preds ? cfg.upsample_w : cfg.coarse_w;
  const size_t px = (size_t)Ho * Wo * (cfg.symmetric ? 2 : 1);
  ROMA_CHECK_HIP(hipEventRecord(ev_fork, st));
  int rc = 0, b0 = 0;
  for (int i = 0; i < ns; ++i) {
    const int bi = B / ns + (i < B % ns ? 1 : 0);
    hipStream_t si = i == 0 ? st : side[i - 1];
    if (i > 0) ROMA_CHECK_HIP(hipStreamWaitEvent(si, ev_fork, 0));
    if (i > 0 && serial_env) {
      hipStream_t sp = i == 1 ? st : side[i - 2];
      ROMA_CHECK_HIP(hipEventRecord(ev_join[i - 1], sp));
      ROMA_CHECK_HIP(hipStreamWaitEvent(si, ev_join[i - 1], 0));
    }
    if (!rc)
      rc = match_impl(bi, ima + b0 * im_lo, imb + b0 * im_lo, ima_hr ? ima_hr + b0 * im_hi : nullptr,
                      imb_hr ? imb_hr + b0 * im_hi : nullptr, warp + b0 * px * 4, cert + b0 * px, si, false,
                      i == 0 ? arena : side_arena[i - 1], i == 0 ? persist : side_persist[i - 1]);
    b0 += bi;
  }
  for (int i = 1; i < ns; ++i) {
    (void)hipEventRecord(ev_join[i - 1], side[i - 1]);
    (void)hipStreamWaitEvent(st, ev_join[i - 1], 0);
  }
  return rc;
}

struct Model::Call {
  Arena &arena, &persist;
  int B = 0, nimg = 0, ndp = 0;
  int shift = 0;
  bool sym = false;
  size_t esz = 4;
  hipStream_t st = nullptr;
  bool dry = false;
  int tslot = 0;
  bool tracing = false;
  const roma_forward_args_t* fw = nullptr;
  int th = 0, tw = 0, T = 0;
  int Npd = 0, Npt = 0;
  void *qbuf = nullptr, *kbuf = nullptr, *vtbuf = nullptr;
  void *ln = nullptr, *ao = nullptr, *hid = nullptr;
  Call(Arena& a, Arena& p) : arena(a), persist(p) {}
  void* alloc(size_t elems, size_t es) const { return arena.alloc(elems * es); }
  void* at(void* p, long elems) const { return static_cast<char*>(p) + elems * (long)esz; }
};

struct Model::Pass {
  bool up = false;
  int H = 0, W = 0;
  const float *imA = nullptr, *imB = nullptr;
  void* feat[5] = {nullptr};
  void* pf_pre[2] = {nullptr, nullptr};
  bool pp_on[2] = {false, false};
  double scale_factor = 1.0;
  float *flow = nullptr, *cert = nullptr, *flow_alt = nullptr, *cert_alt = nullptr;
  const char* tag() const { return up ? "p2" : "p1"; }
};

struct Model::Scale {
  int si, ins, hs, ws;
  int lvl;
  long hw, M;
  const RefinerW& r;
  int ldf;
  float sx, sy;
  std::string tp;
  size_t pf_bytes, d_bytes, flow_bytes, cert_bytes;
  void* pf = nullptr;
  void *d0 = nullptr, *d1 = nullptr;
  Scale(const Call& c, const Pass& p, int si_, const RefinerW& r_)
      : si(si_), ins(SCALE_INT[si_]), hs(ins == 16 ? c.th : p.H / ins), ws(ins == 16 ? c.tw : p.W / ins),
        lvl(ins == 16 ? 4 : (ins == 8 ? 3 : (ins == 4 ? 2 : (ins == 2 ? 1 : 0)))), hw((long)hs * ws), M((long)c.ndp * hw), r(r_),
        ldf((int)round_up(r_.Cf, 8)), sx((float)ins / (4.0f * (float)p.W)), sy((float)ins / (4.0f * (float)p.H)),
        tp(std::string(p.tag()) + "_s" + SCALES[si_]), pf_bytes((size_t)c.nimg * hw * ldf * c.esz),
        d_bytes((size_t)M * r_.Cp * c.esz), flow_bytes((size_t)M * 2 * 4), cert_bytes((size_t)M * 4) {}
};

int Model::fits(const Call& c) {
  if (c.dry || !(c.arena.overflow || c.persist.overflow)) return 0;
  c.arena.overflow = c.persist.overflow = false;
  set_error("roma_match / roma_forward: the workspace planned by roma_finalize is too small for this call (an option that "
            "changes the buffer plan was switched after roma_finalize); the results of this call are invalid");
  return -5;
}

int Model::observe(const Call& c, const std::string& trace_name, const std::string& dbg_name, const void* p, size_t bytes,
                   long rows, int ld, int c0, int c1) {
  if (c.tracing && !trace_name.empty() && trace_n[c.tslot] < TRACE_MAX) {
    const int k = trace_n[c.tslot]++;
    if ((int)trace_names[c.tslot].size() <= k) trace_names[c.tslot].push_back(trace_name);
    else trace_names[c.tslot][k] = trace_name;
    unsigned long long* out = trace_dev[c.tslot] + k;
    if (int rc = c1 > c0 ? checksum_cols_launch(p, rows, ld, c0, c1, out, c.st) : checksum_launch(p, bytes, out, c.st)) return rc;
  }
  if (debug && !c.dry && !dbg_name.empty()) return dbg_save(dbg_name.c_str(), p, bytes, c.st);
  return 0;
}

int Model::encode_vgg(const Call& c, Pass& p) {
  const bool dry = c.dry; hipStream_t st = c.st;
  const int H = p.H, W = p.W, nimg = c.nimg, B = c.B;
  const size_t esz = c.esz;
  const int fh[4] = {H, H / 2, H / 4, H / 8}, fw_[4] = {W, W / 2, W / 4, W / 8};
  const int fc[4] = {64, 128, 256, 512};
  size_t fbytes[4];
  for (int l = 0; l < 4; ++l) {
    fbytes[l] = (size_t)nimg * fh[l] * fw_[l] * fc[l] * esz;
    p.feat[l] = c.arena.alloc(fbytes[l]);
  }
  const int pp_si[2] = {4, 3};
  for (int l = 0; l < 2; ++l) {
    const RefinerW& rr = ref[pp_si[l]];
    const int ldf_l = (int)round_up(rr.Cf, 8);
    p.pp_on[l] = tuning(SW_POOL_PROJ) != 0 && fh[l] >= 2 && fw_[l] >= 2 &&
                 pool_proj_supported(fc[l], rr.Cf, ldf_l, act_dt) && proj[pp_si[l]].b != nullptr;
    if (p.pp_on[l] || dry) p.pf_pre[l] = c.alloc((size_t)nimg * fh[l] * fw_[l] * ldf_l, esz);
    if (!p.pp_on[l] && !dry) p.pf_pre[l] = nullptr;
  }
  const size_t enc_mark = c.arena.mark();
  void* t0 = c.alloc((size_t)nimg * H * W * 64, esz);
  void* t1 = c.alloc((size_t)nimg * (H / 2) * (W / 2) * 64, esz);
  void* col1 = c.alloc((size_t)nimg * H * W * 32, esz);
  if (int rc = fits(c)) return rc;
  if (act_dt == DT_BF16 && (tuning(SW_CONV64) & 4) && (long)3 * H * W < (1l << 23)) {
    RUN(conv3x3_c3_bf16_launch(p.imA, vgg[0].w, vgg[0].b, t0, B, H, W, st));
    RUN(conv3x3_c3_bf16_launch(p.imB, vgg[0].w, vgg[0].b, c.at(t0, (long)B * H * W * 64), B, H, W, st));
  } else {
    RUN(im2col3x3_c3_launch(p.imA, col1, B, H, W, act_dt, st));
    RUN(im2col3x3_c3_launch(p.imB, c.at(col1, (long)B * H * W * 32), B, H, W, act_dt, st));
    GemmArgs g;
    g.A = col1; g.lda = 32; g.W = vgg[0].w; g.ldw = vgg[0].ldw; g.C = t0; g.ldc = 64;
    g.M = nimg * H * W; g.N = 64; g.K = 32; g.k_alg = 27; g.in_dt = act_dt; g.out_dt = act_dt; g.bias = vgg[0].b; g.act = ACT_RELU;
    RUN(gemm_launch(g, st));
  }
  auto conv = [&](int li, const void* in, void* out, int h, int w) -> int {
    GemmArgs g;
    g.A = in; g.W = vgg[li].w; g.ldw = vgg[li].ldw; g.C = out; g.ldc = vgg_cout[li];
    g.M = nimg * h * w; g.N = vgg_cout[li]; g.K = 9 * vgg_cin[li];
    g.in_dt = act_dt; g.out_dt = act_dt; g.bias = vgg[li].b; g.act = ACT_RELU;
    g.conv_h = h; g.conv_w = w; g.conv_c = vgg_cin[li]; g.conv_korder = vgg_korder[li];
    RUN(gemm_launch(g, st));
    return 0;
  };
  auto pool = [&](int l, const void* in, void* out) -> int {
    if (p.pp_on[l]) {
      const int si_ = pp_si[l];
      RUN(pool_proj_launch(in, out, p.pf_pre[l], proj[si_].w, proj[si_].ldw, proj[si_].b, ref[si_].Cf, (int)round_up(ref[si_].Cf, 8),
                           nimg, fh[l], fw_[l], fc[l], act_dt, st));
    } else {
      RUN(maxpool2x2_launch(in, out, nimg, fh[l], fw_[l], fc[l], act_dt, st));
    }
    return 0;
  };
  if (int rc = conv(1, t0, p.feat[0], H, W)) return rc;
  if (int rc = pool(0, p.feat[0], t1)) return rc;
  if (int rc = conv(2, t1, t0, H / 2, W / 2)) return rc;
  if (int rc = conv(3, t0, p.feat[1], H / 2, W / 2)) return rc;
  if (int rc = pool(1, p.feat[1], t1)) return rc;
  if (int rc = conv(4, t1, t0, H / 4, W / 4)) return rc;
  if (int rc = conv(5, t0, t1, H / 4, W / 4)) return rc;
  if (int rc = conv(6, t1, t0, H / 4, W / 4)) return rc;
  if (int rc = conv(7, t0, p.feat[2], H / 4, W / 4)) return rc;
  RUN(maxpool2x2_launch(p.feat[2], t1, nimg, H / 4, W / 4, 256, act_dt, st));
  if (int rc = conv(8, t1, t0, H / 8, W / 8)) return rc;
  if (int rc = conv(9, t0, t1, H / 8, W / 8)) return rc;
  if (int rc = conv(10, t1, t0, H / 8, W / 8)) return rc;
  if (int rc = conv(11, t0, p.feat[3], H / 8, W / 8)) return rc;
  c.arena.release(enc_mark);
  static const char* const dbg_names[4] = {"feat1", "feat2", "feat4", "feat8"};
  for (int l = 0; l < 4; ++l)
    if (int rc = observe(c, std::string(p.tag()) + "_" + dbg_names[l], p.up ? "" : dbg_names[l], p.feat[l], fbytes[l])) return rc;
  if (c.fw && !dry)
    for (int l = 0; l < 4; ++l)
      if (c.fw->feat[4 - l]) ROMA_CHECK_HIP(hipMemcpyAsync(c.fw->feat[4 - l], p.feat[l], fbytes[l], hipMemcpyDeviceToDevice, st));
  return 0;
}

int Model::encode_dino(Call& c, Pass& p) {
  const bool dry = c.dry; hipStream_t st = c.st;
  const int nimg = c.nimg, T = c.T;
  const size_t esz = c.esz;
  const long rows_d = (long)nimg * (T + 1), rows_t = (long)c.ndp * T;
  const size_t fbytes = (size_t)nimg * T * 1024 * esz;
  p.feat[4] = c.arena.alloc(fbytes);
  const long rmax = std::max(rows_d, rows_t);
  c.ln = c.alloc((size_t)rmax * 1024, esz);
  c.ao = c.alloc((size_t)rmax * 1024, esz);
  c.hid = c.alloc((size_t)rmax * 4096, esz);
  const size_t dmark = c.arena.mark();
  void* col = c.alloc((size_t)nimg * T * patch.ldw, esz);
  float* pt = (float*)c.alloc((size_t)nimg * T * 1024, 4);
  float* x = (float*)c.alloc((size_t)rows_d * 1024, 4);
  const bool res_f32_env = tuning(SW_VIT_RES_F32) != 0;
  void* xs = nullptr;
  if (act_dt == DT_BF16) xs = c.alloc((size_t)rows_d * 1024, 2);
  void* feat_vit = p.feat[4];
  if (mixed) feat_vit = c.alloc((size_t)nimg * T * 1024, 2);
  if (int rc = fits(c)) return rc;
  if (!dry) {
    roma_vit_block_t blk[24];
    for (int i = 0; i < 24; ++i) blk[i] = dino[i].pub();
    roma_vit_args_t va{};
    va.B = c.B; va.H = p.H; va.W = p.W;
    va.act = act_dt == DT_F32 ? ROMA_F32 : (mixed ? ROMA_BF16 : roma_h16_format());
    va.bf16_residual = act_dt == DT_BF16 && vit_bf16_residual && !res_f32_env;
    va.im_a = p.imA; va.im_b = p.imB;
    va.patch_w = patch.w; va.patch_b = patch.b; va.patch_ldw = patch.ldw;
    va.cls_tok = cls_tok; va.pos_emb = pos_emb;
    va.blocks = blk; va.nblocks = 24;
    va.norm_w = dino_nw; va.norm_b = dino_nb;
    va.col = col; va.pt = pt; va.x = x; va.xs = xs; va.ln = c.ln; va.ao = c.ao; va.hid = c.hid;
    va.q = c.qbuf; va.k = c.kbuf; va.vt = c.vtbuf;
    va.feat_out = feat_vit;
    if (mixed) {
      if (int rc = peer_vit_forward(&va, st)) {
        set_error("ROMA_MIXED: roma_vit_forward of the bfloat16 library failed");
        return rc;
      }
      RUN(convert_from_bf16_launch(feat_vit, p.feat[4], (long)nimg * T * 1024, st));
    } else {
      RUN(vit_forward(va, st));
    }
  }
  c.arena.release(dmark);
  if (int rc = observe(c, "feat16", "feat16", p.feat[4], fbytes)) return rc;
  if (c.fw && !dry && c.fw->feat[0]) ROMA_CHECK_HIP(hipMemcpyAsync(c.fw->feat[0], p.feat[4], fbytes, hipMemcpyDeviceToDevice, st));
  return 0;
}

int Model::seed_upsample_pass(const Call& c, const Pass& p, const float* flow_p1, const float* cert_p1) {
  const bool dry = c.dry;
  const roma_forward_args_t* fw = c.fw;
  const int sh = fw ? fw->seed_h : cfg.coarse_h, sw = fw ? fw->seed_w : cfg.coarse_w;
  RUN(resize_bilinear_launch(fw ? fw->seed_flow : flow_p1, p.flow, c.ndp, sh, sw, p.H / 8, p.W / 8, 2, c.st));
  RUN(resize_bilinear_launch(fw ? fw->seed_cert : cert_p1, p.cert, c.ndp, sh, sw, p.H / 8, p.W / 8, 1, c.st));
  return 0;
}

int Model::proj_head(const Call& c, const Pass& p, Scale& s) {
  const bool dry = c.dry;
  const bool pf_ready = s.lvl < 2 && p.pp_on[s.lvl];
  s.pf = pf_ready ? p.pf_pre[s.lvl] : c.arena.alloc(s.pf_bytes);
  if (int rc = fits(c)) return rc;
  if (!pf_ready) {
    GemmArgs g;
    g.A = p.feat[s.lvl]; g.lda = PROJ_CIN[s.si]; g.W = proj[s.si].w; g.ldw = proj[s.si].ldw; g.C = s.pf; g.ldc = s.ldf;
    g.M = (int)(c.nimg * s.hw); g.N = s.r.Cf; g.K = PROJ_CIN[s.si]; g.in_dt = act_dt; g.out_dt = act_dt; g.bias = proj[s.si].b;
    RUN(gemm_launch(g, c.st));
  }
  return observe(c, s.tp + "_proj", s.ins == 16 ? "proj16" : "", s.pf, s.pf_bytes);
}

int Model::coarse_match(const Call& c, const Pass& p, const Scale& s) {
  const bool dry = c.dry; hipStream_t st = c.st;
  const long rows_t = s.M;
  float* tokens = (float*)c.alloc((size_t)rows_t * 1024, 4);
  const size_t gp_mark = c.arena.mark();
  if (int rc = gp_posterior(s.pf, s.ldf, act_dt, c.B, c.sym, c.th, c.tw, gp_w, gp_b, tokens, 1024, c.arena, st, dry))
    return c.arena.overflow ? fits(c) : rc;
  c.arena.release(gp_mark);
  const int ldl = 4104;
  float* logits = (float*)c.alloc((size_t)rows_t * ldl, 4);
  if (int rc = fits(c)) return rc;
  RUN(copy2d_launch(s.pf, s.ldf, act_dt, tokens + 512, 1024, DT_F32, rows_t, 512, st));
  if (int rc = observe(c, "", "tokens16", tokens, (size_t)rows_t * 1024 * 4)) return rc;
  VitScratch sc;
  sc.ln = c.ln; sc.ao = c.ao; sc.hid = c.hid; sc.q = c.qbuf; sc.k = c.kbuf; sc.vt = c.vtbuf;
  for (int i = 0; i < 5; ++i) RUN(vit_block_run(tdec[i].pub(), tokens, DT_F32, rows_t, c.ndp, c.T, c.Npt, 8, 128, 1e-5f, act_dt, sc, st));
  const void* zin = tokens;
  if (act_dt != DT_F32) {
    RUN(copy2d_launch(tokens, 1024, DT_F32, c.ln, 1024, act_dt, rows_t, 1024, st));
    zin = c.ln;
  }
  GemmArgs g;
  g.A = zin; g.lda = 1024; g.W = to_out.w; g.ldw = to_out.ldw; g.C = logits; g.ldc = ldl;
  g.M = (int)rows_t; g.N = to_out.N; g.K = 1024; g.in_dt = act_dt; g.out_dt = DT_F32; g.bias = to_out.b;
  RUN(gemm_launch(g, st));
  if (int rc = observe(c, s.tp + "_tokens_gp", "", tokens, (size_t)rows_t * 1024 * 4)) return rc;
  if (int rc = observe(c, s.tp + "_logits", "logits16", logits, (size_t)rows_t * ldl * 4)) return rc;
  RUN(cls_to_flow_launch(logits, ldl, p.flow, p.cert, rows_t, st));
  if (int rc = observe(c, s.tp + "_gm_flow", "gm_flow16_own", p.flow, s.flow_bytes)) return rc;
  if (!debug || dry) return 0;
  auto inj = [&](const char* nm, float* dst, size_t bytes) -> int {
    auto it = inject.find(nm);
    if (it == inject.end()) return 0;
    ROMA_REQUIRE(it->second.second == bytes, "roma_debug_inject: injected stage has the wrong size for this batch");
    ROMA_CHECK_HIP(hipMemcpyAsync(dst, it->second.first, bytes, hipMemcpyDeviceToDevice, st));
    return 0;
  };
  if (int rc = inj("gm_flow16", p.flow, s.flow_bytes)) return rc;
  if (int rc = inj("gm_cert16", p.cert, s.cert_bytes)) return rc;
  if (int rc = observe(c, "", "gm_flow16", p.flow, s.flow_bytes)) return rc;
  return observe(c, "", "gm_cert16", p.cert, s.cert_bytes);
}

int Model::refiner_input(const Call& c, const Pass& p, Scale& s) {
  const bool dry = c.dry; hipStream_t st = c.st;
  const RefinerW& r = s.r;
  s.d0 = c.arena.alloc(s.d_bytes);
  s.d1 = c.arena.alloc(s.d_bytes);
  LocalCorrArgs lc;
  if (r.radius) {
    const long lc_ints = local_corr_ws_ints(c.ndp, s.hs, s.ws, r.radius);
    lc.ws = (int*)c.alloc((size_t)lc_ints, 4); lc.ws_bytes = lc_ints * 4;
  }
  if (int rc = fits(c)) return rc;
  if (int rc = observe(c, s.tp + "_flow_before", "", p.flow, s.flow_bytes)) return rc;
  RefinerInputArgs ia;
  ia.feat = s.pf; ia.ldf = s.ldf; ia.flow = p.flow; ia.d = s.d0; ia.ldd = r.Cp; ia.emb_w = r.emb_w; ia.emb_b = r.emb_b;
  ia.B = c.ndp; ia.H = s.hs; ia.W = s.ws; ia.C = r.Cf; ia.E = r.E; ia.Kcorr = r.K; ia.nimg = c.nimg; ia.shift = c.shift;
  ia.disp_scale = (float)(40.0 / 32.0 * p.scale_factor); ia.dt = act_dt;
  RUN(refiner_input_launch(ia, st));
  if (r.radius) {
    lc.f0 = s.pf; lc.f1 = s.pf; lc.warp = p.flow; lc.out = c.at(s.d0, 2 * r.Cf + r.E);
    lc.B = c.ndp; lc.H = s.hs; lc.W = s.ws; lc.C = r.Cf; lc.radius = r.radius; lc.ld0 = s.ldf; lc.ld1 = s.ldf; lc.ldo = r.Cp;
    lc.nimg = c.nimg; lc.f1_shift = c.shift; lc.scale = 1.0f / sqrtf((float)r.Cf); lc.in_dt = act_dt; lc.out_dt = act_dt;
    RUN(local_corr_window_launch(lc, st));
  }
  const bool dual = dbg_dual_slot() >= 0;
  const bool din_small = s.d_bytes <= ((size_t)(dual ? 512 : 64) << 20);
  if (int rc = observe(c, s.tp + "_din", din_small ? std::string(p.tag()) + "_din" + SCALES[s.si] : "", s.d0, s.d_bytes)) return rc;
  if (dual && s.ins == 1)
    if (int rc = observe(c, "", std::string(p.tag()) + "_flowin1", p.flow, s.flow_bytes)) return rc;
  if (!c.tracing) return 0;
  if (int rc = observe(c, s.tp + "_proj_again", "", s.pf, s.pf_bytes)) return rc;
  if (int rc = observe(c, s.tp + "_flow_again", "", p.flow, s.flow_bytes)) return rc;
  if (int rc = observe(c, s.tp + "_din_again", "", s.d0, s.d_bytes)) return rc;
  if (c.esz != 2 || r.E <= 0) return 0;
  const int cols[5] = {0, r.Cf, 2 * r.Cf, 2 * r.Cf + r.E, r.Cp};
  static const char* const part[4] = {"_din_x", "_din_xhat", "_din_emb", "_din_rest"};
  for (int i = 0; i < 4; ++i)
    if (int rc = observe(c, s.tp + part[i], "", s.d0, 0, s.M, r.Cp, cols[i], cols[i + 1])) return rc;
  for (int b = 0; b < c.ndp; ++b)
    if (int rc = observe(c, s.tp + "_din_pair" + std::to_string(b), "", c.at(s.d0, (long)b * s.hw * r.Cp), 0, s.hw, r.Cp, 0, r.Cp)) return rc;
  return 0;
}

int Model::refiner_chain(const Call& c, const Pass& p, const Scale& s, const void** d_last, bool* composed) {
  const bool dry = c.dry; hipStream_t st = c.st;
  const RefinerW& r = s.r;
  const bool fused = fuse_refiner_blocks && refiner_block_supported(r.Cp, act_dt);
  float* delta = fused && (dry || compose_out_conv) ? (float*)c.alloc((size_t)s.M * 4, 4) : nullptr;
  if (int rc = fits(c)) return rc;
  void *dcur = s.d0, *dalt = s.d1;
  *composed = compose_out_conv;
  for (int b = 0; b < 9; ++b) {
    const bool last = b == 8 && compose_out_conv;
    if (last && fused) {
      RUN(refiner_block_final_launch(dcur, delta, r.dw_w[b], r.dw_b[b], r.ocf_w, r.Cp, r.ocf_b, c.ndp, s.hs, s.ws, r.Cp, act_dt, st));
      RUN(refiner_apply_delta_launch(delta, p.flow, p.cert, s.M, s.sx, s.sy, st));
      *d_last = nullptr;
      return 0;
    }
    if (fused) {
      RUN(refiner_block_launch(dcur, dalt, r.dw_w[b], r.dw_b[b], r.pw[b].w, r.pw[b].ldw, r.pw[b].b, c.ndp, s.hs, s.ws, r.Cp, act_dt, st));
      std::swap(dcur, dalt);
      if (int rc = observe(c, s.tp + "_blk" + std::to_string(b), "", dcur, s.d_bytes)) return rc;
      continue;
    }
    RUN(dwconv5x5_launch(dcur, dalt, r.dw_w[b], r.dw_b[b], c.ndp, s.hs, s.ws, r.Cp, act_dt, st));
    if (int rc = observe(c, s.tp + "_dw" + std::to_string(b), "", dalt, s.d_bytes)) return rc;
    if (last) {
      std::swap(dcur, dalt);
      break;
    }
    GemmArgs g;
    g.A = dalt; g.lda = r.Cp; g.W = r.pw[b].w; g.ldw = r.pw[b].ldw; g.C = dcur; g.ldc = r.Cp;
    g.M = (int)s.M; g.N = r.Cp; g.K = r.Cp; g.in_dt = act_dt; g.out_dt = act_dt; g.bias = r.pw[b].b;
    g.n_alg = g.k_alg = r.C;
    RUN(gemm_launch(g, st));
    if (int rc = observe(c, s.tp + "_blk" + std::to_string(b), "", dcur, s.d_bytes)) return rc;
  }
  *d_last = dcur;
  return 0;
}

int Model::refiner_out(const Call& c, const Pass& p, const Scale& s, const void* d_last, bool composed) {
  const bool dry = c.dry; hipStream_t st = c.st;
  const RefinerW& r = s.r;
  if (d_last)
    RUN(refiner_out_launch(d_last, r.Cp, act_dt, composed ? r.oc_w : r.out_w, composed ? r.oc_b : r.out_b, p.flow, p.cert, s.M, r.Cp,
                           s.sx, s.sy, st));
  if (int rc = observe(c, s.tp + "_flow", std::string(p.tag()) + "_flow" + SCALES[s.si], p.flow, s.flow_bytes)) return rc;
  if (int rc = observe(c, s.tp + "_cert", std::string(p.tag()) + "_cert" + SCALES[s.si], p.cert, s.cert_bytes)) return rc;
  if (c.fw && !dry) {
    if (c.fw->flow[s.si]) ROMA_CHECK_HIP(hipMemcpyAsync(c.fw->flow[s.si], p.flow, s.flow_bytes, hipMemcpyDeviceToDevice, st));
    if (c.fw->cert[s.si]) ROMA_CHECK_HIP(hipMemcpyAsync(c.fw->cert[s.si], p.cert, s.cert_bytes, hipMemcpyDeviceToDevice, st));
  }
  return 0;
}

int Model::next_scale(const Call& c, Pass& p, const Scale& s, float* cert16_keep) {
  const bool dry = c.dry; hipStream_t st = c.st;
  if (s.ins == 16) {
    if (s.M % 4 == 0) {
      RUN(copy2d_launch(p.cert, s.M, DT_F32, cert16_keep, s.M, DT_F32, 1, (int)s.M, st));
    } else if (!dry) {
      ROMA_CHECK_HIP(hipMemcpyAsync(cert16_keep, p.cert, s.cert_bytes, hipMemcpyDeviceToDevice, st));
    }
  }
  if (s.ins == 1) return 0;
  const int nh = p.H / (s.ins / 2), nw = p.W / (s.ins / 2);
  RUN(resize_bilinear_launch(p.flow, p.flow_alt, c.ndp, s.hs, s.ws, nh, nw, 2, st));
  RUN(resize_bilinear_launch(p.cert, p.cert_alt, c.ndp, s.hs, s.ws, nh, nw, 1, st));
  std::swap(p.flow, p.flow_alt);
  std::swap(p.cert, p.cert_alt);
  return observe(c, s.tp + "_flow_up", "", p.flow, (size_t)c.ndp * nh * nw * 2 * 4);
}

int Model::epilogue(const Call& c, const float* flow, const float* cert, const float* cert16_keep, float* warp_out, float* cert_out) {
  const bool dry = c.dry;
  const int Hfin = cfg.upsample_preds ? cfg.upsample_h : cfg.coarse_h, Wfin = cfg.upsample_preds ? cfg.upsample_w : cfg.coarse_w;
  FinalArgs fa;
  fa.flow = flow;
  fa.cert = cert;
  fa.cert16 = cfg.attenuate_cert ? cert16_keep : nullptr;
  fa.warp = warp_out; fa.certainty = cert_out;
  fa.B = c.B; fa.H = Hfin; fa.W = Wfin; fa.h16 = c.th; fa.w16 = c.tw; fa.symmetric = cfg.symmetric;
  RUN(final_epilogue_launch(fa, c.st));
  const size_t px = (size_t)c.B * Hfin * Wfin * (cfg.symmetric ? 2 : 1);
  if (int rc = observe(c, "final_warp", "", warp_out, px * 4 * 4)) return rc;
  return observe(c, "final_cert", "", cert_out, px * 4);
}

int Model::match_impl(int B, const float* ima, const float* imb, const float* ima_hr, const float* imb_hr,
                      float* warp_out, float* cert_out, hipStream_t st, bool dry, Arena& arena, Arena& persist,
                      const roma_forward_args_t* fw) {
  Call c(arena, persist);
  c.B = B; c.nimg = 2 * B; c.shift = B;
  c.sym = fw ? fw->symmetric != 0 : cfg.symmetric != 0;
  c.ndp = c.sym ? 2 * B : B;
  c.esz = act_dt == DT_F32 ? 4 : 2;
  c.st = st; c.dry = dry; c.fw = fw;
  arena.reset();
  persist.reset();
  c.tslot = (&arena == &this->arena) ? 0 : (int)(&arena - side_arena) + 1;
  dbg_cur_slot = c.tslot;
  c.tracing = trace_on && !dry;
  if (c.tracing) {
    if (!trace_dev[c.tslot]) {
      ROMA_CHECK_HIP(hipMalloc((void**)&trace_dev[c.tslot], TRACE_MAX * sizeof(unsigned long long)));
      owned.push_back(trace_dev[c.tslot]);
    }
    ROMA_CHECK_HIP(hipMemsetAsync(trace_dev[c.tslot], 0, TRACE_MAX * sizeof(unsigned long long), st));
    trace_n[c.tslot] = 0;
  }
  c.th = cfg.coarse_h / 14; c.tw = cfg.coarse_w / 14; c.T = c.th * c.tw;
  c.Npd = (int)round_up(c.T + 1, 128); c.Npt = (int)round_up(c.T, 128);
  const size_t qkv_elems = std::max((size_t)c.nimg * 16 * c.Npd * 64, (size_t)c.ndp * 8 * c.Npt * 128);
  c.qbuf = persist.alloc(qkv_elems * c.esz);
  c.kbuf = persist.alloc(qkv_elems * c.esz);
  c.vtbuf = persist.alloc(qkv_elems * c.esz);

  float* cert16_keep = (float*)c.alloc((size_t)c.ndp * c.T, 4);
  float *pp_flow[2][2] = {{nullptr, nullptr}, {nullptr, nullptr}}, *pp_cert[2][2] = {{nullptr, nullptr}, {nullptr, nullptr}};
  for (int ps = 0; ps < ((cfg.upsample_preds || (fw && fw->upsample)) ? 2 : 1); ++ps) {
    const size_t px = (size_t)c.ndp * (ps ? cfg.upsample_h : cfg.coarse_h) * (ps ? cfg.upsample_w : cfg.coarse_w);
    for (int i = 0; i < 2; ++i) {
      pp_flow[ps][i] = (float*)c.alloc(px * 2, 4);
      pp_cert[ps][i] = (float*)c.alloc(px, 4);
    }
  }
  if (int rc = fits(c)) return rc;
  float *flow_p1 = nullptr, *cert_p1 = nullptr;
  float *flow_fin = nullptr, *cert_fin = nullptr;

  const int pass0 = fw ? (fw->upsample ? 1 : 0) : 0, pass1 = fw ? pass0 + 1 : (cfg.upsample_preds ? 2 : 1);
  for (int pass = pass0; pass < pass1; ++pass) {
    Pass p;
    p.up = pass == 1;
    p.H = p.up ? cfg.upsample_h : cfg.coarse_h; p.W = p.up ? cfg.upsample_w : cfg.coarse_w;
    p.imA = (p.up && !fw) ? ima_hr : ima;
    p.imB = (p.up && !fw) ? imb_hr : imb;
    p.scale_factor = sqrt((double)p.H * (double)p.W / (560.0 * 560.0));
    if (!p.up && coarse_scale_factor > 0.0) p.scale_factor = coarse_scale_factor;
    if (fw && fw->scale_factor > 0.0) p.scale_factor = fw->scale_factor;
    p.flow = pp_flow[pass][0]; p.cert = pp_cert[pass][0]; p.flow_alt = pp_flow[pass][1]; p.cert_alt = pp_cert[pass][1];

    const size_t pass_mark = arena.mark();
    if (int rc = encode_vgg(c, p)) return rc;
    if (!p.up)
      if (int rc = encode_dino(c, p)) return rc;
    if (p.up)
      if (int rc = seed_upsample_pass(c, p, flow_p1, cert_p1)) return rc;
    for (int si = p.up ? 1 : 0; si < 5; ++si) {
      Scale s(c, p, si, ref[si]);
      const size_t scale_mark = arena.mark();
      if (int rc = proj_head(c, p, s)) return rc;
      if (s.ins == 16) {
        const size_t coarse_mark = arena.mark();
        if (int rc = coarse_match(c, p, s)) return rc;
        arena.release(coarse_mark);
      }
      const void* d_last = nullptr;
      bool composed = false;
      if (int rc = refiner_input(c, p, s)) return rc;
      if (int rc = refiner_chain(c, p, s, &d_last, &composed)) return rc;
      if (int rc = refiner_out(c, p, s, d_last, composed)) return rc;
      arena.release(scale_mark);
      if (int rc = next_scale(c, p, s, cert16_keep)) return rc;
    }
    flow_fin = p.flow; cert_fin = p.cert;
    if (!p.up) { flow_p1 = p.flow; cert_p1 = p.cert; }
    arena.release(pass_mark);
  }
  if (fw) return 0;
  return epilogue(c, flow_fin, cert_fin, cert16_keep, warp_out, cert_out);
}

}
```

roma_amd/csrc/tuning.hip:

```cpp
#include "tuning.h"

#include <stdlib.h>
#include <string.h>

#include "../../include/roma_hip.h"

namespace roma {
void set_error(const std::string& msg);
namespace {

struct Row {
  Switch id;
  const char* key;
  const char* env;
  long def;
  int floor;
  const char* doc;
};

constexpr Row ROWS[] = {
    {SW_GEMM8P, "gemm8p", "ROMA_GEMM8P", 1, 0, "large bf16 GEMMs on the 8-phase 256 x 256 kernel (1) or on the one-barrier-per-slab kernel (0)"},
    {SW_GEMM_DBG, "gemm_dbg", "ROMA_GEMM_DBG", 0, 0, "experiment bits of the GEMM kernels (1 skip output stores, 2 skip the K loop, 2048 no streaming stores, ...)"},
    {SW_GEMM8P_WALK, "gemm8p_walk", nullptr, -1, 1, "gemm8p: tile rows per group of the persistent walk (1 = row major); unset = 8 from 24 tile columns on, else 1"},
    {SW_GEMM8P_SCHED, "gemm8p_sched", "ROMA_GEMM8P_SCHED", 1, 0, "gemm8p K-loop schedule: 1 k-half phases, 0 quadrant phases (tools builds only)"},
    {SW_GEMM8P_MAXWG, "gemm8p_maxwg", nullptr, -1, 8, "gemm8p, measurement only: cap the persistent grid at n workgroups (a multiple of 8); unset = one per CU"},
    {SW_WS1X1, "ws1x1", "ROMA_WS1X1", 1, 0, "N = K = 576 refiner 1x1 on the weight-stationary kernel (1) or on the 256 x 192 tile kernel (0)"},
    {SW_LC_MODE, "lc_mode", "ROMA_LC_MODE", 0, 0, "local correlation: 0 tiled form + gather work list, 1 every tile on the gather list (key only), 2 per-pixel kernel"},
    {SW_LC_BIN, "lc_bin", "ROMA_LC_BIN", 1, 0, "local correlation: queries of incoherent tiles sorted by target bin, counters in LDS (1) or device atomics (2), or gathered per query (0)"},
    {SW_CONV64, "conv64", "ROMA_CONV64", 7, 0, "weight-stationary VGG front end, bit mask: 1 the Cin = 64 kernels, 2 the Cin = 128 kernel, 4 the fused first layer"},
    {SW_CONV_PATCH, "conv_patch", "ROMA_CONV_PATCH", 1, 0, "patch-resident 3x3 kernel for slab-major VGG layers (1) or gemm8p (0); environment 0 also packs tap-major weights"},
    {SW_ATTN_XCD, "attn_xcd", "ROMA_ATTN_XCD", 1, 0, "attention work items in per-XCD bands of (batch, head) (1) or in plain order (0)"},
    {SW_ATTN_EXP2, "attn_exp2", nullptr, -1, 0, "tools only: force the 2^x softmax of the 16-bit attention kernel on / off; unset = as the caller says"},
    {SW_DW_RING, "dw_ring", "ROMA_DW_RING", 1, 0, "depthwise 5x5: 0 register-prefetch kernel, 1 ring kernel for the large launches, 2 ring kernel for every shape it takes"},
    {SW_GP_COL, "gp_col", "ROMA_GP_COL", 1, 0, "GP Cholesky left-looking, one launch per block column (1) or the right-looking launch chain (0)"},
    {SW_POOL_PROJ, "pool_proj", "ROMA_POOL_PROJ", 1, 0, "max-pool + proj head of strides 1 / 2 in one pass (1) or as separate kernels (0)"},
    {SW_GP_COL_LEADER, "gp_col_leader", "ROMA_GP_COL_LEADER", 1, 0, "block-column Cholesky: a leader workgroup factorises the diagonal block, its product formed one launch ahead (1) or in its own launch (2), or every workgroup its own copy (0)"},
    {SW_GEMM8P_MINM, nullptr, "ROMA_GEMM8P_MINM", 2048, 0, "gemm8p: smallest M it takes for the wide (N >= 2048) dense launches"},
    {SW_GEMM_NT, nullptr, "ROMA_GEMM_NT", 1, 0, "non-temporal output stores in the 16-bit GEMM row writer"},
    {SW_GEMM_F32_FILL, nullptr, "ROMA_GEMM_F32_FILL", 1, 0, "exact-f32 GEMMs below 192 tiles of 256 x 256 run on 128 x 128 tiles"},
    {SW_GEMM_SMALLM, nullptr, "ROMA_GEMM_SMALLM", 1, 0, "GEMMs below 320 tiles of 128 x 128 run on 128 x 64 tiles"},
    {SW_CONV64_SY, nullptr, "ROMA_CONV64_SY", 0, 0, "conv64 strip height in rows; 0 = the split of H with the fewest rounds"},
    {SW_CONV_KORDER, nullptr, "ROMA_CONV_KORDER", 1, 0, "VGG layers with Cout >= 256 pack slab-major weight rows (read when a handle is created)"},
    {SW_RB_SY, nullptr, "ROMA_RB_SY", 0, 0, "fused refiner block strip height in rows; 0 = the split of H with the fewest rounds"},
    {SW_DWR_MAXSY, nullptr, "ROMA_DWR_MAXSY", 1 << 20, 0, "depthwise ring kernel: cap of the strip height in rows (at least 6)"},
    {SW_DW_RING_MINELEMS, nullptr, "ROMA_DW_RING_MINELEMS", 64l << 20, 0, "dw_ring = 1: smallest launch, in elements, that goes to the ring kernel"},
    {SW_RI_VEC, nullptr, "ROMA_RI_VEC", 1, 0, "refiner_input on the 16-byte vector kernel where alignment allows"},
    {SW_OUT_ROW, nullptr, "ROMA_OUT_ROW", 1, 0, "refiner_out: row kernel for C = 24 in 16-bit storage"},
    {SW_OUT_LPR, nullptr, "ROMA_OUT_LPR", 1, 0, "refiner_out, 16-bit: lanes per row chosen to fill the 16-byte pieces best"},
    {SW_OUT_ROWS_IT, nullptr, "ROMA_OUT_ROWS_IT", 0, 0, "refiner_out: row groups per wave (even, >= 2); otherwise 8"},
    {SW_GP_AUG, nullptr, "ROMA_GP_AUG", 1, 0, "GP Cholesky: right-hand sides stored behind A ride along the factorisation (0 = separate forward loop)"},
    {SW_GP_BWD2, nullptr, "ROMA_GP_BWD2", 1, 0, "GP Cholesky: backward substitution with one launch per step (0 = two)"},
    {SW_COMPOSE_OUT, nullptr, "ROMA_COMPOSE_OUT", 1, 0, "initial value of the handle option compose_out_conv (read when a handle is created)"},
    {SW_VIT_RES_F32, nullptr, "ROMA_VIT_RES_F32", 0, 0, "force DINOv2's f32 residual stream in the 16-bit modes"},
    {SW_STREAMS, nullptr, "ROMA_STREAMS", 0, 0, "number of sub-batch streams of match(); 0 = the handle's option"},
    {SW_STREAMS_SERIAL, nullptr, "ROMA_STREAMS_SERIAL", 0, 0, "diagnostic: sub-batch streams run one after the other"},
    {SW_DEBUG_DUAL_SLOT, nullptr, "ROMA_DEBUG_DUAL_SLOT", -1, 0, "diagnostic: keep the stream split in debug mode, sub-batch k captures the stages of ROMA_DEBUG_ONLY"},
};
constexpr int NROWS = sizeof(ROWS) / sizeof(ROWS[0]);
constexpr bool rows_in_enum_order() {
  for (int i = 0; i < NROWS; ++i)
    if (ROWS[i].id != i) return false;
  return true;
}
static_assert(NROWS == SW_COUNT && rows_in_enum_order(), "one row per Switch, in enum order");
constexpr bool json_plain(const char* s) {
  for (; s && *s; ++s)
    if (*s == '"' || *s == '\\' || *s < ' ') return false;
  return true;
}
constexpr bool rows_json_plain() {
  for (const Row& r : ROWS)
    if (!json_plain(r.key) || !json_plain(r.env) || !json_plain(r.doc)) return false;
  return true;
}
static_assert(rows_json_plain(), "keys, environment names and docs: plain ASCII without quote, backslash or control character");

struct Overrides {
  long v[SW_COUNT];
  constexpr Overrides() : v{} {
    for (long& x : v) x = -1;
  }
};
[[clang::require_constant_initialization]] Overrides g_override;

struct Env {
  long v[SW_COUNT];
  Env() {
    for (int i = 0; i < NROWS; ++i) {
      const char* s = ROWS[i].env ? getenv(ROWS[i].env) : nullptr;
      v[i] = s ? atol(s) : ROWS[i].def;
    }
  }
};
const Env& env() {
  static const Env e;
  return e;
}

}

long tuning_env(Switch id) { return env().v[id]; }
long tuning_override(Switch id) { return g_override.v[id] >= ROWS[id].floor ? g_override.v[id] : -1; }
long tuning(Switch id) { return g_override.v[id] >= ROWS[id].floor ? g_override.v[id] : tuning_env(id); }

int tuning_set(const char* key, long value) {
  for (const Row& r : ROWS)
    if (r.key && !strcmp(r.key, key)) {
      g_override.v[r.id] = value >= r.floor ? value : -1;
      return 0;
    }
  set_error(std::string("roma_tuning: unknown key ") + key);
  return ROMA_ERR_ARG;
}

std::string tuning_describe() {
  std::string js = "[";
  for (const Row& r : ROWS) {
    const auto quoted = [](const char* s) { return s ? "\"" + std::string(s) + "\"" : std::string("null"); };
    const long ov = tuning_override(r.id);
    js += std::string(r.id ? ", " : "") + "{\"key\": " + quoted(r.key) + ", \"env\": " + quoted(r.env) +
          ", \"default\": " + std::to_string(r.def) + ", \"override\": " + (ov >= 0 ? std::to_string(ov) : "null") +
          ", \"value\": " + std::to_string(tuning(r.id)) + ", \"doc\": " + quoted(r.doc) + "}";
  }
  return js + "]";
}

}
```

Measured before the change: 106.8 image-pairs/s.

## Fuse VGG first conv layer into conv1_2 weight-stationary kernel as stem

Result: no change. 107.3 image-pairs/s, median of 6 (+0.5%).

```diff
diff --git a/include/roma_hip.h b/include/roma_hip.h
--- a/include/roma_hip.h
+++ b/include/roma_hip.h
@@ -266,6 +266,8 @@
 int roma_op_conv3x3_c3(const float* img, const float* w, const float* bias, void* out, int B, int H, int W, int dt_out,
                        void* stream);
 int roma_op_conv3x3_c3_bf16(const float* img, const void* w, const float* bias, void* out, int B, int H, int W, void* stream);
+int roma_op_conv_stem(const float* im_a, int n_a, const float* im_b, int n_b, const void* w1, const float* b1, const void* w2,
+                      const float* b2, void* out, int H, int W, void* stream);
 
 #ifdef __cplusplus
 }
diff --git a/roma_amd/_lib.py b/roma_amd/_lib.py
--- a/roma_amd/_lib.py
+++ b/roma_amd/_lib.py
@@ -141,6 +141,7 @@
     "roma_op_pool_proj": (_i, [_vp, _vp, _vp, _vp, _l, _vp, _i, _i, _i, _i, _i, _i, _i, _vp]),
     "roma_op_conv3x3_c3": (_i, [_vp, _vp, _vp, _vp, _i, _i, _i, _i, _vp]),
     "roma_op_conv3x3_c3_bf16": (_i, [_vp, _vp, _vp, _vp, _i, _i, _i, _vp]),
+    "roma_op_conv_stem": (_i, [_vp, _i, _vp, _i, _vp, _vp, _vp, _vp, _vp, _i, _i, _vp]),
     "roma_op_refiner_out": (_i, [_vp, _l, _i, _vp, _vp, _vp, _vp, _l, _i, _f, _f, _vp]),
 }
 
diff --git a/roma_amd/csrc/api.hip b/roma_amd/csrc/api.hip
--- a/roma_amd/csrc/api.hip
+++ b/roma_amd/csrc/api.hip
@@ -766,6 +766,11 @@
   return conv3x3_c3_bf16_launch(img, w, bias, out, B, H, W, S(stream));
 }
 
+int roma_op_conv_stem(const float* im_a, int n_a, const float* im_b, int n_b, const void* w1, const float* b1, const void* w2,
+                      const float* b2, void* out, int H, int W, void* stream) {
+  return conv_stem_launch(im_a, n_a, im_b, n_b, w1, b1, w2, b2, out, H, W, S(stream));
+}
+
 int roma_op_conv3x3_c3(const float* img, const float* w, const float* bias, void* out, int B, int H, int W, int dt_out,
                        void* stream) {
   return conv3x3_c3_launch(img, w, bias, out, B, H, W, DT(dt_out), S(stream));
diff --git a/roma_amd/csrc/conv64.h b/roma_amd/csrc/conv64.h
--- a/roma_amd/csrc/conv64.h
+++ b/roma_amd/csrc/conv64.h
@@ -3,5 +3,9 @@
 
 namespace roma {
 int conv64_try_launch(const GemmArgs& a, hipStream_t stream);
+int conv64_strip_height(int B, int H, int nxt, int slots);
 int conv3x3_c3_bf16_launch(const float* img, const void* w, const float* bias, void* out, int B, int H, int W, hipStream_t stream);
+bool conv_stem_supported(int H, int W);
+int conv_stem_launch(const float* imA, int nA, const float* imB, int nB, const void* w1, const float* b1, const void* w2,
+                     const float* b2, void* out, int H, int W, hipStream_t stream);
 }
diff --git a/roma_amd/csrc/conv64.hip b/roma_amd/csrc/conv64.hip
--- a/roma_amd/csrc/conv64.hip
+++ b/roma_amd/csrc/conv64.hip
@@ -5,202 +5,11 @@
 
 #include <algorithm>
 
+#include "conv64_kernel.h"
 #include "gemm_device.h"
 #include "tuning.h"
 
 namespace roma {
-
-static __device__ __attribute__((aligned(256))) unsigned int g_c64_dump[256];
-
-#define C64_WAIT_VM(N) asm volatile("s_waitcnt vmcnt(%0)" ::"n"(N) : "memory")
-
-template <int COUT>
-__global__ __launch_bounds__(256, 2) void conv3x3_c64_kernel(const bf16_t* __restrict__ in, const bf16_t* __restrict__ w,
-                                                             const float* __restrict__ bias, bf16_t* __restrict__ out, int B,
-                                                             int H, int W, int SY, int nxt, int nblocks) {
-  constexpr int NCG = COUT / 32;
-  constexpr int NPG = 4 / NCG;
-  constexpr int TW = 64 * NPG;
-  constexpr int NPIECE = ((TW + 2) * 128 + 1023) / 1024;
-  constexpr int RSTRIDE = NPIECE * 1024;
-  constexpr int KW = (NPIECE + 3) / 4;
-  extern __shared__ __attribute__((aligned(1024))) unsigned char ring[];
-
-  if ((int)blockIdx.x >= nblocks) return;
-  const int tid = threadIdx.x, lane = tid & 63;
-  const int wave = __builtin_amdgcn_readfirstlane(tid >> 6);
-  const int cg = wave % NCG, pg = wave / NCG;
-  const int l31 = lane & 31, h = lane >> 5;
-  typedef unsigned u32x4 __attribute__((ext_vector_type(4)));
-  const unsigned ring0 = (unsigned)(size_t)((__attribute__((address_space(3))) unsigned char*)ring);
-
-  u32x4 wreg[36];
-  {
-    const bf16_t* wp = w + (long)(32 * cg + l31) * 576 + 8 * h;
-#pragma unroll
-    for (int ks = 0; ks < 36; ++ks) wreg[ks] = *reinterpret_cast<const u32x4*>(wp + 16 * ks);
-  }
-  float* bias_s = reinterpret_cast<float*>(ring + 4 * RSTRIDE);
-  if (tid < COUT) bias_s[tid] = bias[tid];
-
-  unsigned rdo[3];
-#pragma unroll
-  for (int dx = 0; dx < 3; ++dx) {
-    const int p = 64 * pg + l31 + dx;
-    rdo[dx] = ring0 + (unsigned)(p * 128 + ((h ^ ((p >> 1) & 7)) << 4));
-  }
-
-  for (int lb = blockIdx.x; lb < nblocks; lb += gridDim.x) {
-  const int xt = lb % nxt;
-  const int r = lb / nxt;
-  const int yt = (H + SY - 1) / SY;
-  const int ys = (r % yt) * SY;
-  const int b = r / yt;
-  const int x0 = xt * TW;
-  const int sy = min(SY, H - ys);
-  if (lb != (int)blockIdx.x) __builtin_amdgcn_s_barrier();
-
-  const bf16_t* inb = in + (long)b * H * W * 64;
-  const __amdgpu_buffer_rsrc_t rs_in = __builtin_amdgcn_make_buffer_rsrc(const_cast<bf16_t*>(inb), 0, (int)((long)H * W * 128), 0x00020000);
-  unsigned voff[KW];
-  bool okx[KW];
-  {
-    const int dl_p = lane >> 3, dl_slot = lane & 7;
-    const u32x4 z4 = {0u, 0u, 0u, 0u};
-#pragma unroll
-    for (int j = 0; j < KW; ++j) {
-      const int q = wave + 4 * j;
-      const int p = q * 8 + dl_p;
-      const int x = x0 - 1 + p;
-      const int c = dl_slot ^ ((p >> 1) & 7);
-      okx[j] = q < NPIECE && p < TW + 2 && x >= 0 && x < W;
-      voff[j] = okx[j] ? (unsigned)(x * 128 + c * 16) : 0u;
-      if (q < NPIECE && !okx[j]) {
-        int ln = lane;
-        asm volatile("" : "+v"(ln));
-#pragma unroll
-        for (int sl = 0; sl < 4; ++sl)
-          asm volatile("ds_write_b128 %0, %1" ::"v"(ring0 + sl * RSTRIDE + q * 1024 + ln * 16), "v"(z4) : "memory");
-      }
-    }
-  }
-  asm volatile("s_waitcnt vmcnt(0) lgkmcnt(0)" ::: "memory");
-
-#define C64_ISSUE_ROW(YY, SLOT)                                                                                \
-  {                                                                                                            \
-    const int yy_ = (YY);                                                                                      \
-    if (yy_ >= 0 && yy_ < H) {                                                                                 \
-      const int so_ = yy_ * W * 128;                                                                           \
-      _Pragma("unroll") for (int j = 0; j < KW; ++j) {                                                         \
-        const int q_ = wave + 4 * j;                                                                           \
-        if (q_ < NPIECE) {                                                                                     \
-          if (okx[j])                                                                                          \
-            __builtin_amdgcn_raw_ptr_buffer_load_lds(rs_in, (__attribute__((address_space(3))) void*)(ring + (SLOT) * RSTRIDE + q_ * 1024), \
-                                                     16, (int)voff[j], so_, 0, 0);                             \
-        }                                                                                                      \
-      }                                                                                                        \
-    } else {                                     \
-      const u32x4 z4_ = {0u, 0u, 0u, 0u};                                                                      \
-      int ln_ = lane;                                                                                          \
-      asm volatile("" : "+v"(ln_));                                                                            \
-      _Pragma("unroll") for (int j = 0; j < KW; ++j) {                                                         \
-        const int q_ = wave + 4 * j;                                                                           \
-        if (q_ < NPIECE)                                                                                       \
-          asm volatile("ds_write_b128 %0, %1" ::"v"(ring0 + (SLOT) * RSTRIDE + q_ * 1024 + ln_ * 16), "v"(z4_) : "memory"); \
-      }                                                                                                        \
-    }                                                                                                          \
-  }
-
-  u32x4 fa[2][4];
-#define C64_READ_G(SLOTOFF, DX, G)                                                                            \
-  {                                                                                                           \
-    const unsigned ad_ = (rdo[DX] + (SLOTOFF)) ^ (unsigned)((G) << 5);                                         \
-    asm volatile("ds_read_b128 %0, %1" : "=v"(fa[0][G]) : "v"(ad_));                                           \
-    asm volatile("ds_read_b128 %0, %1 offset:4096" : "=v"(fa[1][G]) : "v"(ad_));                              \
-  }
-#define C64_WAIT_G(G, N) asm volatile("s_waitcnt lgkmcnt(%2)" : "+v"(fa[0][G]), "+v"(fa[1][G]) : "n"(N) : "memory")
-
-  C64_ISSUE_ROW(ys - 1, 0)
-  C64_ISSUE_ROW(ys, 1)
-  C64_ISSUE_ROW(ys + 1, 2)
-
-  bf16_t* outb = out + (long)b * H * W * COUT;
-  for (int o = 0; o < sy; ++o) {
-    if (o == 0) {
-      asm volatile("s_waitcnt vmcnt(0) lgkmcnt(0)" ::: "memory");
-    } else {
-      C64_WAIT_VM(0);
-    }
-    __builtin_amdgcn_s_barrier();
-    C64_ISSUE_ROW(ys + o + 2, (o + 3) & 3)
-    if (o == 0) {
-      C64_READ_G(0, 0, 0)
-      C64_READ_G(0, 0, 1)
-    }
-    C64_READ_G((o & 3) * RSTRIDE, 0, 2)
-    C64_READ_G((o & 3) * RSTRIDE, 0, 3)
-
-    f32x16 acc[2];
-#pragma unroll
-    for (int tm = 0; tm < 2; ++tm)
-#pragma unroll
-      for (int e = 0; e < 16; ++e) acc[tm][e] = 0.f;
-#pragma unroll
-    for (int t = 0; t < 9; ++t) {
-#pragma unroll
-      for (int g = 0; g < 4; ++g) {
-        if (t == 8 && g == 3) {
-          C64_WAIT_G(g, 4);
-        } else {
-          C64_WAIT_G(g, 6);
-        }
-#pragma unroll
-        for (int tm = 0; tm < 2; ++tm)
-          acc[tm] = mfma_h16_32x32x16(wreg[t * 4 + g],
-                                                            fa[tm][g], acc[tm]);
-        __builtin_amdgcn_sched_barrier(0);
-        if (t + 1 < 9) {
-          C64_READ_G(((o + (t + 1) / 3) & 3) * RSTRIDE, (t + 1) % 3, g)
-        } else if (g < 2) {
-          C64_READ_G(((o + 1) & 3) * RSTRIDE, 0, g)
-        }
-        __builtin_amdgcn_sched_barrier(0);
-      }
-    }
-
-    const int y = ys + o;
-#pragma unroll
-    for (int P = 0; P < 2; ++P) {
-      f32x4 bv0, bv1;
-      {
-        const unsigned ba = ring0 + 4 * RSTRIDE + (32 * cg + 16 * P + 4 * h) * 4;
-        asm volatile("ds_read_b128 %0, %2\n\tds_read_b128 %1, %2 offset:32\n\ts_waitcnt lgkmcnt(0)"
-                     : "=&v"(bv0), "=&v"(bv1)
-                     : "v"(ba)
-                     : "memory");
-      }
-#pragma unroll
-      for (int tm = 0; tm < 2; ++tm) {
-        const int x = x0 + 64 * pg + 32 * tm + l31;
-        const unsigned a0 = pack_bf16x2(fmaxf(acc[tm][8 * P + 0] + bv0[0], 0.f), fmaxf(acc[tm][8 * P + 1] + bv0[1], 0.f));
-        const unsigned a1 = pack_bf16x2(fmaxf(acc[tm][8 * P + 2] + bv0[2], 0.f), fmaxf(acc[tm][8 * P + 3] + bv0[3], 0.f));
-        const unsigned b0 = pack_bf16x2(fmaxf(acc[tm][8 * P + 4] + bv1[0], 0.f), fmaxf(acc[tm][8 * P + 5] + bv1[1], 0.f));
-        const unsigned b1 = pack_bf16x2(fmaxf(acc[tm][8 * P + 6] + bv1[2], 0.f), fmaxf(acc[tm][8 * P + 7] + bv1[3], 0.f));
-        const auto s0 = __builtin_amdgcn_permlane32_swap(a0, b0, false, false);
-        const auto s1 = __builtin_amdgcn_permlane32_swap(a1, b1, false, false);
-        const u32x4 st = {s0[0], s1[0], s0[1], s1[1]};
-        bf16_t* op = outb + ((long)y * W + x) * COUT + 32 * cg + 16 * P + 8 * h;
-        u32x4* dst = x < W ? reinterpret_cast<u32x4*>(op) : reinterpret_cast<u32x4*>(g_c64_dump) + lane;
-        *dst = st;
-      }
-    }
-  }
-  C64_WAIT_VM(0);
-  }
-#undef C64_WAIT_G
-#undef C64_READ_G
-#undef C64_ISSUE_ROW
-}
 
 template <int DUMMY>
 __global__ __launch_bounds__(512, 1) void conv3x3_c128_kernel(const bf16_t* __restrict__ in, const bf16_t* __restrict__ w,
@@ -527,6 +336,23 @@
   return 0;
 }
 
+int conv64_strip_height(int B, int H, int nxt, int slots) {
+  int SY = tuning(SW_CONV64_SY);
+  if (SY <= 0) {
+    long best = -1;
+    for (int yt = 1; yt <= std::max(1, H / 12); ++yt) {
+      const int sy = (H + yt - 1) / yt;
+      const long n = (long)B * nxt * ((H + sy - 1) / sy);
+      const long cost = ((n + slots - 1) / slots) * (sy + 3);
+      if (best < 0 || cost < best) {
+        best = cost;
+        SY = sy;
+      }
+    }
+  }
+  return SY;
+}
+
 int conv64_try_launch(const GemmArgs& a, hipStream_t stream) {
   const int use = tuning(SW_CONV64);
   const bool c128 = a.conv_c == 128;
@@ -542,21 +368,8 @@
   const int B = (int)(a.M / hw);
   const int TW = (!c128 && a.N == 64) ? 128 : 64;
   const int slots = c128 ? 256 : 512;
-  const int sy_env = tuning(SW_CONV64_SY);
   const int nxt = (W + TW - 1) / TW;
-  int SY = sy_env;
-  if (SY <= 0) {
-    long best = -1;
-    for (int yt = 1; yt <= std::max(1, H / 12); ++yt) {
-      const int sy = (H + yt - 1) / yt;
-      const long n = (long)B * nxt * ((H + sy - 1) / sy);
-      const long cost = ((n + slots - 1) / slots) * (sy + 3);
-      if (best < 0 || cost < best) {
-        best = cost;
-        SY = sy;
-      }
-    }
-  }
+  const int SY = conv64_strip_height(B, H, nxt, slots);
   const long nb = (long)B * ((H + SY - 1) / SY) * nxt;
   if (nb <= 0 || nb >= (1l << 30)) return 1;
   char pname[64];
@@ -580,9 +393,9 @@
   if (c128) {
     hipLaunchKernelGGL(conv3x3_c128_kernel<0>, dim3((unsigned)gx), dim3(512), LDS128, stream, in, w, a.bias, out, B, H, W, SY, nxt, (int)nb);
   } else if (a.N == 64) {
-    hipLaunchKernelGGL(conv3x3_c64_kernel<64>, dim3((unsigned)gx), dim3(256), LDS64, stream, in, w, a.bias, out, B, H, W, SY, nxt, (int)nb);
+    hipLaunchKernelGGL(conv3x3_c64_kernel<64>, dim3((unsigned)gx), dim3(256), LDS64, stream, in, w, a.bias, out, B, H, W, SY, nxt, (int)nb, C64Stem{});
   } else {
-    hipLaunchKernelGGL(conv3x3_c64_kernel<128>, dim3((unsigned)gx), dim3(256), LDS64N128, stream, in, w, a.bias, out, B, H, W, SY, nxt, (int)nb);
+    hipLaunchKernelGGL(conv3x3_c64_kernel<128>, dim3((unsigned)gx), dim3(256), LDS64N128, stream, in, w, a.bias, out, B, H, W, SY, nxt, (int)nb, C64Stem{});
   }
   ROMA_LAUNCH_CHECK();
   return 0;
diff --git a/roma_amd/csrc/conv64_kernel.h b/roma_amd/csrc/conv64_kernel.h
--- /dev/null
+++ b/roma_amd/csrc/conv64_kernel.h
@@ -0,0 +1,343 @@
+#pragma once
+#include "gemm_device.h"
+
+namespace roma {
+
+static __device__ __attribute__((aligned(256))) unsigned int g_c64_dump[256];
+
+#define C64_WAIT_VM(N) asm volatile("s_waitcnt vmcnt(%0)" ::"n"(N) : "memory")
+
+struct C64Stem {
+  const float* imA;
+  const float* imB;
+  const bf16_t* w1;
+  const float* b1;
+  int nA;
+};
+
+constexpr int C64_STEM_NOTAP = 0x40000000;
+__device__ __forceinline__ void c64_stem_table(int* tab, int tid, int H, int W) {
+  if (tid < 32) {
+    const int k = tid;
+    const bool tap = k < 27;
+    tab[k] = tap ? ((k / 9) * H * W + ((k % 9) / 3 - 1) * W + (k % 3 - 1)) * 4 : C64_STEM_NOTAP;
+    tab[32 + k] = tap ? ((1 << ((k % 9) / 3)) | (8 << (k % 3))) : 64;
+  }
+}
+
+__device__ __forceinline__ void c64_stem_load(float (&v)[16], __amdgpu_buffer_rsrc_t rs, const int* tab, int yy, int xb, int H,
+                                              int W, int lane) {
+  typedef int i32x4 __attribute__((ext_vector_type(4)));
+  asm volatile("" : "+v"(lane));
+  const int l31 = lane & 31, h = lane >> 5;
+  const int base4 = (yy * W + xb + l31) * 4;
+  const i32x4* tp = reinterpret_cast<const i32x4*>(tab + 16 * h);
+  if (xb >= 1 && xb + 33 <= W && yy >= 1 && yy + 1 < H) {
+#pragma unroll
+    for (int q = 0; q < 4; ++q) {
+      const i32x4 to = tp[q];
+#pragma unroll
+      for (int j = 0; j < 4; ++j)
+        v[4 * q + j] = __builtin_bit_cast(float, __builtin_amdgcn_raw_buffer_load_b32(rs, base4 + to[j], 0, 0));
+    }
+  } else {
+    const int x = xb + l31;
+    const int okbits = (yy >= 1 ? 1 : 0) | 2 | (yy + 1 < H ? 4 : 0) | (x >= 1 && x - 1 < W ? 8 : 0) | (x >= 0 && x < W ? 16 : 0) |
+                       (x + 1 >= 0 && x + 1 < W ? 32 : 0);
+#pragma unroll
+    for (int q = 0; q < 4; ++q) {
+      const i32x4 to = tp[q], ts = tp[8 + q];
+#pragma unroll
+      for (int j = 0; j < 4; ++j) {
+        const bool ok = (okbits & ts[j]) == ts[j];
+        v[4 * q + j] = __builtin_bit_cast(float, __builtin_amdgcn_raw_buffer_load_b32(rs, ok ? base4 + to[j] : C64_STEM_NOTAP, 0, 0));
+      }
+    }
+  }
+}
+
+__device__ __forceinline__ void c64_stem_store(const float (&v)[16], unsigned row, unsigned w1s, const float* b1s, int p0,
+                                               bool store_ok, int lane) {
+  typedef unsigned u32x4 __attribute__((ext_vector_type(4)));
+  typedef __attribute__((address_space(3))) u32x4 lds_u32x4;
+  asm volatile("" : "+v"(lane));
+  const int l31 = lane & 31, h = lane >> 5;
+  u32x4 fr[2];
+#pragma unroll
+  for (int ks = 0; ks < 2; ++ks)
+#pragma unroll
+    for (int j = 0; j < 4; ++j) fr[ks][j] = pack_bf16x2(v[8 * ks + 2 * j], v[8 * ks + 2 * j + 1]);
+  const int p = p0 + l31;
+  const unsigned px = row + (unsigned)(p * 128);
+  const int sw = (p >> 1) & 7;
+#pragma unroll 1
+  for (int cb = 0; cb < 2; ++cb) {
+    const u32x4 wf0 = *reinterpret_cast<const lds_u32x4*>(w1s + (unsigned)(((cb * 2 + 0) * 64 + lane) * 16));
+    const u32x4 wf1 = *reinterpret_cast<const lds_u32x4*>(w1s + (unsigned)(((cb * 2 + 1) * 64 + lane) * 16));
+    f32x16 acc;
+#pragma unroll
+    for (int e = 0; e < 16; ++e) acc[e] = 0.f;
+    acc = mfma_h16_32x32x16(wf0, fr[0], acc);
+    acc = mfma_h16_32x32x16(wf1, fr[1], acc);
+    u32x4 st[2];
+#pragma unroll
+    for (int P = 0; P < 2; ++P) {
+      const f32x4 b0 = *reinterpret_cast<const f32x4*>(b1s + 32 * cb + 16 * P + 4 * h);
+      const f32x4 b1 = *reinterpret_cast<const f32x4*>(b1s + 32 * cb + 16 * P + 8 + 4 * h);
+      const unsigned a0 = pack_bf16x2(fmaxf(acc[8 * P + 0] + b0[0], 0.f), fmaxf(acc[8 * P + 1] + b0[1], 0.f));
+      const unsigned a1 = pack_bf16x2(fmaxf(acc[8 * P + 2] + b0[2], 0.f), fmaxf(acc[8 * P + 3] + b0[3], 0.f));
+      const unsigned c0 = pack_bf16x2(fmaxf(acc[8 * P + 4] + b1[0], 0.f), fmaxf(acc[8 * P + 5] + b1[1], 0.f));
+      const unsigned c1 = pack_bf16x2(fmaxf(acc[8 * P + 6] + b1[2], 0.f), fmaxf(acc[8 * P + 7] + b1[3], 0.f));
+      const auto s0 = __builtin_amdgcn_permlane32_swap(a0, c0, false, false);
+      const auto s1 = __builtin_amdgcn_permlane32_swap(a1, c1, false, false);
+      st[P] = u32x4{s0[0], s1[0], s0[1], s1[1]};
+    }
+    if (store_ok) {
+#pragma unroll
+      for (int P = 0; P < 2; ++P) *reinterpret_cast<lds_u32x4*>(px + (unsigned)(((4 * cb + 2 * P + h) ^ sw) << 4)) = st[P];
+    }
+  }
+}
+
+template <int COUT, bool STEM = false>
+__global__ __launch_bounds__(256, 2) void conv3x3_c64_kernel(const bf16_t* __restrict__ in, const bf16_t* __restrict__ w,
+                                                             const float* __restrict__ bias, bf16_t* __restrict__ out, int B,
+                                                             int H, int W, int SY, int nxt, int nblocks, C64Stem sa) {
+  static_assert(!STEM || COUT == 64, "the stem form is conv1_2");
+  constexpr int NCG = COUT / 32;
+  constexpr int NPG = 4 / NCG;
+  constexpr int TW = 64 * NPG;
+  constexpr int TWS = STEM ? TW - 2 : TW;
+  constexpr int NPIECE = ((TW + 2) * 128 + 1023) / 1024;
+  constexpr int RSTRIDE = NPIECE * 1024;
+  constexpr int KW = (NPIECE + 3) / 4;
+  extern __shared__ __attribute__((aligned(1024))) unsigned char ring[];
+
+  if ((int)blockIdx.x >= nblocks) return;
+  const int tid = threadIdx.x, lane = tid & 63;
+  const int wave = __builtin_amdgcn_readfirstlane(tid >> 6);
+  const int cg = wave % NCG, pg = wave / NCG;
+  const int l31 = lane & 31, h = lane >> 5;
+  typedef unsigned u32x4 __attribute__((ext_vector_type(4)));
+  const unsigned ring0 = (unsigned)(size_t)((__attribute__((address_space(3))) unsigned char*)ring);
+
+  u32x4 wreg[36];
+  {
+    const bf16_t* wp = w + (long)(32 * cg + l31) * 576 + 8 * h;
+#pragma unroll
+    for (int ks = 0; ks < 36; ++ks) wreg[ks] = *reinterpret_cast<const u32x4*>(wp + 16 * ks);
+  }
+  float* bias_s = reinterpret_cast<float*>(ring + 4 * RSTRIDE);
+  if (tid < COUT) bias_s[tid] = bias[tid];
+  constexpr int W1OFF = 4 * RSTRIDE + 512;
+  int* stem_tab = reinterpret_cast<int*>(ring + W1OFF + 4096);
+  if constexpr (STEM) {
+    if (tid < 64) bias_s[64 + tid] = sa.b1[tid];
+    const int cb = wave >> 1, ks = wave & 1;
+    const u32x4 f = *reinterpret_cast<const u32x4*>(sa.w1 + (32 * cb + l31) * 32 + 16 * h + 8 * ks);
+    *reinterpret_cast<__attribute__((address_space(3))) u32x4*>(ring0 + W1OFF + tid * 16) = f;
+    c64_stem_table(stem_tab, tid, H, W);
+    asm volatile("s_waitcnt vmcnt(0) lgkmcnt(0)" ::: "memory");
+    __builtin_amdgcn_s_barrier();
+  }
+
+  unsigned rdo[3];
+#pragma unroll
+  for (int dx = 0; dx < 3; ++dx) {
+    const int p = 64 * pg + l31 + dx;
+    rdo[dx] = ring0 + (unsigned)(p * 128 + ((h ^ ((p >> 1) & 7)) << 4));
+  }
+
+  for (int lb = blockIdx.x; lb < nblocks; lb += gridDim.x) {
+  const int xt = lb % nxt;
+  const int r = lb / nxt;
+  const int yt = (H + SY - 1) / SY;
+  const int ys = (r % yt) * SY;
+  const int b = r / yt;
+  const int x0 = xt * TWS;
+  const int sy = min(SY, H - ys);
+  if (lb != (int)blockIdx.x) __builtin_amdgcn_s_barrier();
+
+  const bf16_t* inb = STEM ? nullptr : in + (long)b * H * W * 64;
+  const __amdgpu_buffer_rsrc_t rs_in = __builtin_amdgcn_make_buffer_rsrc(const_cast<bf16_t*>(inb), 0, (int)((long)H * W * 128), 0x00020000);
+  __amdgpu_buffer_rsrc_t rs_img = rs_in;
+  if constexpr (STEM)
+    rs_img = __builtin_amdgcn_make_buffer_rsrc(const_cast<float*>(b < sa.nA ? sa.imA + (long)b * 3 * H * W : sa.imB + (long)(b - sa.nA) * 3 * H * W),
+                                               0, 3 * H * W * 4, 0x00020000);
+  unsigned voff[KW];
+  bool okx[KW];
+  {
+    const int dl_p = lane >> 3, dl_slot = lane & 7;
+    const u32x4 z4 = {0u, 0u, 0u, 0u};
+#pragma unroll
+    for (int j = 0; j < KW; ++j) {
+      const int q = wave + 4 * j;
+      const int p = q * 8 + dl_p;
+      const int x = x0 - 1 + p;
+      const int c = dl_slot ^ ((p >> 1) & 7);
+      okx[j] = q < NPIECE && p < TWS + 2 && x >= 0 && x < W;
+      voff[j] = okx[j] ? (unsigned)(x * 128 + c * 16) : 0u;
+      if (q < NPIECE && !okx[j]) {
+        int ln = lane;
+        asm volatile("" : "+v"(ln));
+#pragma unroll
+        for (int sl = 0; sl < 4; ++sl)
+          asm volatile("ds_write_b128 %0, %1" ::"v"(ring0 + sl * RSTRIDE + q * 1024 + ln * 16), "v"(z4) : "memory");
+      }
+    }
+  }
+  asm volatile("s_waitcnt vmcnt(0) lgkmcnt(0)" ::: "memory");
+
+#define C64_ISSUE_ROW(YY, SLOT)                                                                                \
+  {                                                                                                            \
+    const int yy_ = (YY);                                                                                      \
+    if (yy_ >= 0 && yy_ < H) {                                                                                 \
+      if constexpr (!STEM) {                                                                                   \
+        const int so_ = yy_ * W * 128;                                                                         \
+        _Pragma("unroll") for (int j = 0; j < KW; ++j) {                                                       \
+          const int q_ = wave + 4 * j;                                                                         \
+          if (q_ < NPIECE) {                                                                                   \
+            if (okx[j])                                                                                        \
+              __builtin_amdgcn_raw_ptr_buffer_load_lds(rs_in, (__attribute__((address_space(3))) void*)(ring + (SLOT) * RSTRIDE + q_ * 1024), \
+                                                       16, (int)voff[j], so_, 0, 0);                           \
+          }                                                                                                    \
+        }                                                                                                      \
+      }                                                                                                        \
+    } else {                                     \
+      const u32x4 z4_ = {0u, 0u, 0u, 0u};                                                                      \
+      int ln_ = lane;                                                                                          \
+      asm volatile("" : "+v"(ln_));                                                                            \
+      _Pragma("unroll") for (int j = 0; j < KW; ++j) {                                                         \
+        const int q_ = wave + 4 * j;                                                                           \
+        if (q_ < NPIECE)                                                                                       \
+          asm volatile("ds_write_b128 %0, %1" ::"v"(ring0 + (SLOT) * RSTRIDE + q_ * 1024 + ln_ * 16), "v"(z4_) : "memory"); \
+      }                                                                                                        \
+    }                                                                                                          \
+  }
+
+  u32x4 fa[2][4];
+#define C64_READ_G(SLOTOFF, DX, G)                                                                            \
+  {                                                                                                           \
+    const unsigned ad_ = (rdo[DX] + (SLOTOFF)) ^ (unsigned)((G) << 5);                                         \
+    asm volatile("ds_read_b128 %0, %1" : "=v"(fa[0][G]) : "v"(ad_));                                           \
+    asm volatile("ds_read_b128 %0, %1 offset:4096" : "=v"(fa[1][G]) : "v"(ad_));                              \
+  }
+#define C64_WAIT_G(G, N) asm volatile("s_waitcnt lgkmcnt(%2)" : "+v"(fa[0][G]), "+v"(fa[1][G]) : "n"(N) : "memory")
+
+  float sv[16];
+#define C64_STEM_LOAD(YY) \
+  if ((YY) >= 0 && (YY) < H) c64_stem_load(sv, rs_img, stem_tab, (YY), x0 - 1 + 32 * wave, H, W, lane);
+#define C64_STEM_ROW(YY, SLOT)                                                                                 \
+  {                                                                                                            \
+    C64_ISSUE_ROW(YY, SLOT)                                                                                    \
+    if ((YY) >= 0 && (YY) < H) {                                                                               \
+      const int xs_ = x0 - 1 + 32 * wave + l31;                                                                \
+      c64_stem_store(sv, ring0 + (unsigned)((SLOT) * RSTRIDE), ring0 + W1OFF, bias_s + 64, 32 * wave, xs_ >= 0 && xs_ < W, lane); \
+    }                                                                                                          \
+  }
+
+  if constexpr (STEM) {
+#pragma unroll 1
+    for (int r = 0; r < 3; ++r) {
+      C64_STEM_LOAD(ys - 1 + r)
+      C64_STEM_ROW(ys - 1 + r, r)
+    }
+    if (sy > 1) C64_STEM_LOAD(ys + 2)
+  } else {
+    C64_ISSUE_ROW(ys - 1, 0)
+    C64_ISSUE_ROW(ys, 1)
+    C64_ISSUE_ROW(ys + 1, 2)
+  }
+
+  bf16_t* outb = out + (long)b * H * W * COUT;
+  for (int o = 0; o < sy; ++o) {
+    if (o == 0 || STEM) {
+      asm volatile("s_waitcnt vmcnt(0) lgkmcnt(0)" ::: "memory");
+    } else {
+      C64_WAIT_VM(0);
+    }
+    __builtin_amdgcn_s_barrier();
+    if constexpr (STEM) {
+      if (o + 1 < sy) {
+        C64_STEM_ROW(ys + o + 2, (o + 3) & 3)
+        asm volatile("s_waitcnt lgkmcnt(0)" ::: "memory");
+      }
+    } else {
+      C64_ISSUE_ROW(ys + o + 2, (o + 3) & 3)
+    }
+    if (o == 0) {
+      C64_READ_G(0, 0, 0)
+      C64_READ_G(0, 0, 1)
+    }
+    C64_READ_G((o & 3) * RSTRIDE, 0, 2)
+    C64_READ_G((o & 3) * RSTRIDE, 0, 3)
+
+    f32x16 acc[2];
+#pragma unroll
+    for (int tm = 0; tm < 2; ++tm)
+#pragma unroll
+      for (int e = 0; e < 16; ++e) acc[tm][e] = 0.f;
+#pragma unroll
+    for (int t = 0; t < 9; ++t) {
+#pragma unroll
+      for (int g = 0; g < 4; ++g) {
+        if (t == 8 && g == 3) {
+          C64_WAIT_G(g, 4);
+        } else {
+          C64_WAIT_G(g, 6);
+        }
+#pragma unroll
+        for (int tm = 0; tm < 2; ++tm)
+          acc[tm] = mfma_h16_32x32x16(wreg[t * 4 + g],
+                                                            fa[tm][g], acc[tm]);
+        __builtin_amdgcn_sched_barrier(0);
+        if (t + 1 < 9) {
+          C64_READ_G(((o + (t + 1) / 3) & 3) * RSTRIDE, (t + 1) % 3, g)
+        } else if (g < 2) {
+          C64_READ_G(((o + 1) & 3) * RSTRIDE, 0, g)
+        }
+        __builtin_amdgcn_sched_barrier(0);
+      }
+    }
+
+    const int y = ys + o;
+#pragma unroll
+    for (int P = 0; P < 2; ++P) {
+      f32x4 bv0, bv1;
+      {
+        const unsigned ba = ring0 + 4 * RSTRIDE + (32 * cg + 16 * P + 4 * h) * 4;
+        asm volatile("ds_read_b128 %0, %2\n\tds_read_b128 %1, %2 offset:32\n\ts_waitcnt lgkmcnt(0)"
+                     : "=&v"(bv0), "=&v"(bv1)
+                     : "v"(ba)
+                     : "memory");
+      }
+#pragma unroll
+      for (int tm = 0; tm < 2; ++tm) {
+        const int x = x0 + 64 * pg + 32 * tm + l31;
+        const bool keep = x < W && 64 * pg + 32 * tm + l31 < TWS;
+        const unsigned a0 = pack_bf16x2(fmaxf(acc[tm][8 * P + 0] + bv0[0], 0.f), fmaxf(acc[tm][8 * P + 1] + bv0[1], 0.f));
+        const unsigned a1 = pack_bf16x2(fmaxf(acc[tm][8 * P + 2] + bv0[2], 0.f), fmaxf(acc[tm][8 * P + 3] + bv0[3], 0.f));
+        const unsigned b0 = pack_bf16x2(fmaxf(acc[tm][8 * P + 4] + bv1[0], 0.f), fmaxf(acc[tm][8 * P + 5] + bv1[1], 0.f));
+        const unsigned b1 = pack_bf16x2(fmaxf(acc[tm][8 * P + 6] + bv1[2], 0.f), fmaxf(acc[tm][8 * P + 7] + bv1[3], 0.f));
+        const auto s0 = __builtin_amdgcn_permlane32_swap(a0, b0, false, false);
+        const auto s1 = __builtin_amdgcn_permlane32_swap(a1, b1, false, false);
+        const u32x4 st = {s0[0], s1[0], s0[1], s1[1]};
+        bf16_t* op = outb + ((long)y * W + x) * COUT + 32 * cg + 16 * P + 8 * h;
+        u32x4* dst = keep ? reinterpret_cast<u32x4*>(op) : reinterpret_cast<u32x4*>(g_c64_dump) + lane;
+        *dst = st;
+      }
+    }
+    if constexpr (STEM) {
+      if (o + 2 < sy) C64_STEM_LOAD(ys + o + 3)
+    }
+  }
+  C64_WAIT_VM(0);
+  }
+#undef C64_STEM_ROW
+#undef C64_STEM_LOAD
+#undef C64_WAIT_G
+#undef C64_READ_G
+#undef C64_ISSUE_ROW
+}
+
+}
diff --git a/roma_amd/csrc/conv_stem.hip b/roma_amd/csrc/conv_stem.hip
--- /dev/null
+++ b/roma_amd/csrc/conv_stem.hip
@@ -0,0 +1,39 @@
+#include <algorithm>
+
+#include "conv64.h"
+#include "conv64_kernel.h"
+
+namespace roma {
+
+bool conv_stem_supported(int H, int W) {
+  return H > 0 && W > 0 && (long)3 * H * W < (1l << 23);
+}
+
+int conv_stem_launch(const float* imA, int nA, const float* imB, int nB, const void* w1, const float* b1, const void* w2,
+                     const float* b2, void* out, int H, int W, hipStream_t stream) {
+  ROMA_REQUIRE(imA && nA > 0 && nB >= 0 && (imB || nB == 0) && w1 && b1 && w2 && b2 && out, "conv_stem: bad arguments");
+  ROMA_REQUIRE(conv_stem_supported(H, W), "conv_stem: image too large");
+  const int B = nA + nB, TW = 126, slots = 512;
+  const int nxt = (W + TW - 1) / TW;
+  const int SY = conv64_strip_height(B, H, nxt, slots);
+  const long nb = (long)B * ((H + SY - 1) / SY) * nxt;
+  ROMA_REQUIRE(nb > 0 && nb < (1l << 30), "conv_stem: grid too large");
+  constexpr int LDS = 4 * 17 * 1024 + 512 + 4096 + 256;
+  const auto kernel = &conv3x3_c64_kernel<64, true>;
+  static bool attr_set[64] = {false};
+  int dev = 0;
+  ROMA_CHECK_HIP(hipGetDevice(&dev));
+  if (dev < 0 || dev >= 64 || !attr_set[dev]) {
+    ROMA_CHECK_HIP(hipFuncSetAttribute(reinterpret_cast<const void*>(kernel), hipFuncAttributeMaxDynamicSharedMemorySize, LDS));
+    if (dev >= 0 && dev < 64) attr_set[dev] = true;
+  }
+  const double px = (double)B * H * W;
+  ProfScope ps("conv3x3_c64_kernel<64, stem>", 2.0 * px * 64.0 * (576.0 + 27.0), "flop", stream);
+  const C64Stem sa{imA, imB, reinterpret_cast<const bf16_t*>(w1), b1, nA};
+  hipLaunchKernelGGL(kernel, dim3((unsigned)std::min<long>(nb, slots)), dim3(256), LDS, stream, (const bf16_t*)nullptr,
+                     reinterpret_cast<const bf16_t*>(w2), b2, reinterpret_cast<bf16_t*>(out), B, H, W, SY, nxt, (int)nb, sa);
+  ROMA_LAUNCH_CHECK();
+  return 0;
+}
+
+}
diff --git a/roma_amd/csrc/model.hip b/roma_amd/csrc/model.hip
--- a/roma_amd/csrc/model.hip
+++ b/roma_amd/csrc/model.hip
@@ -330,11 +330,16 @@
     if (!p.pp_on[l] && !dry) p.pf_pre[l] = nullptr;
   }
   const size_t enc_mark = c.arena.mark();
-  void* t0 = c.alloc((size_t)nimg * H * W * 64, esz);
+  const int c64 = (int)tuning(SW_CONV64);
+  const bool stem = act_dt == DT_BF16 && (c64 & 13) == 5 && conv_stem_supported(H, W) && vgg[0].ldw == 32 && vgg[1].ldw == 576 &&
+                    vgg[0].b && vgg[1].b;
+  void* t0 = c.alloc((size_t)nimg * H * W * (stem && !dry ? 32 : 64), esz);
   void* t1 = c.alloc((size_t)nimg * (H / 2) * (W / 2) * 64, esz);
   void* col1 = c.alloc((size_t)nimg * H * W * 32, esz);
   if (int rc = fits(c)) return rc;
-  if (act_dt == DT_BF16 && (tuning(SW_CONV64) & 4) && (long)3 * H * W < (1l << 23)) {
+  if (stem) {
+    RUN(conv_stem_launch(p.imA, B, p.imB, B, vgg[0].w, vgg[0].b, vgg[1].w, vgg[1].b, p.feat[0], H, W, st));
+  } else if (act_dt == DT_BF16 && (c64 & 4) && (long)3 * H * W < (1l << 23)) {
     RUN(conv3x3_c3_bf16_launch(p.imA, vgg[0].w, vgg[0].b, t0, B, H, W, st));
     RUN(conv3x3_c3_bf16_launch(p.imB, vgg[0].w, vgg[0].b, c.at(t0, (long)B * H * W * 64), B, H, W, st));
   } else {
@@ -364,7 +369,8 @@
     }
     return 0;
   };
-  if (int rc = conv(1, t0, p.feat[0], H, W)) return rc;
+  if (!stem)
+    if (int rc = conv(1, t0, p.feat[0], H, W)) return rc;
   if (int rc = pool(0, p.feat[0], t1)) return rc;
   if (int rc = conv(2, t1, t0, H / 2, W / 2)) return rc;
   if (int rc = conv(3, t0, p.feat[1], H / 2, W / 2)) return rc;
diff --git a/roma_amd/csrc/tuning.hip b/roma_amd/csrc/tuning.hip
--- a/roma_amd/csrc/tuning.hip
+++ b/roma_amd/csrc/tuning.hip
@@ -27,7 +27,7 @@
     {SW_WS1X1, "ws1x1", "ROMA_WS1X1", 1, 0, "N = K = 576 refiner 1x1 on the weight-stationary kernel (1) or on the 256 x 192 tile kernel (0)"},
     {SW_LC_MODE, "lc_mode", "ROMA_LC_MODE", 0, 0, "local correlation: 0 tiled form + gather work list, 1 every tile on the gather list (key only), 2 per-pixel kernel"},
     {SW_LC_BIN, "lc_bin", "ROMA_LC_BIN", 1, 0, "local correlation: queries of incoherent tiles sorted by target bin, counters in LDS (1) or device atomics (2), or gathered per query (0)"},
-    {SW_CONV64, "conv64", "ROMA_CONV64", 7, 0, "weight-stationary VGG front end, bit mask: 1 the Cin = 64 kernels, 2 the Cin = 128 kernel, 4 the fused first layer"},
+    {SW_CONV64, "conv64", "ROMA_CONV64", 7, 0, "weight-stationary VGG front end, bit mask: 1 the Cin = 64 kernels, 2 the Cin = 128 kernel, 4 the fused first layer, 8 the first layer as a launch of its own (unset: inside conv1_2 where 1 and 4 are set)"},
     {SW_CONV_PATCH, "conv_patch", "ROMA_CONV_PATCH", 1, 0, "patch-resident 3x3 kernel for slab-major VGG layers (1) or gemm8p (0); environment 0 also packs tap-major weights"},
     {SW_ATTN_XCD, "attn_xcd", "ROMA_ATTN_XCD", 1, 0, "attention work items in per-XCD bands of (batch, head) (1) or in plain order (0)"},
     {SW_ATTN_EXP2, "attn_exp2", nullptr, -1, 0, "tools only: force the 2^x softmax of the 16-bit attention kernel on / off; unset = as the caller says"},
```
